# kluonj/HelFEM

Measured on AMD Instinct MI355X. Metric: scf_iteration_wall_time_fock_plus_geneig_nbf4230, lower is better.
Workload: dtype f64; 1 GPU; diatomic Z1=7 Z2=7 R=2.068 PBE, nelem=5 nnodes=15 nquad=75 lmmax=[20,20] (Nbf=4230, Nang=61, Nrad=70), XC grid 92x13, symmetry blocks [1380, 1470, 1380]: J+XC Fock build + eig_gsym_sub + density per step; parallelism=shard1, density=occupied orbitals of the core Hamiltonian

## Files before the change

### helfem_amd/__init__.py

```python
import ctypes
import os

import numpy as np

_HERE = os.path.dirname(os.path.abspath(__file__))
_LIB_PATH = os.environ.get("HELFEM_AMD_LIB") or os.path.join(_HERE, "lib", "libhelfem_amd.so")
_lib = None

c_double_p = ctypes.POINTER(ctypes.c_double)
c_int_p = ctypes.POINTER(ctypes.c_int)
c_i64_p = ctypes.POINTER(ctypes.c_int64)


class hfg_diatomic_desc(ctypes.Structure):
    _fields_ = [("Z1", ctypes.c_int), ("Z2", ctypes.c_int), ("Rhalf", ctypes.c_double), ("primbas", ctypes.c_int),
                ("nnodes", ctypes.c_int), ("nquad", ctypes.c_int), ("bval", c_double_p), ("nbval", ctypes.c_int),
                ("lval", c_int_p), ("mval", c_int_p), ("nang", ctypes.c_int), ("lpad", ctypes.c_int)]


class hfg_model_pot(ctypes.Structure):
    _fields_ = [("kind", ctypes.c_int), ("Z", ctypes.c_int), ("d", ctypes.c_double), ("H", ctypes.c_double)]


class hfg_atomic_desc(ctypes.Structure):
# ... 34 lines not shown
class hfg_scf_atomic_extras(ctypes.Structure):
    _fields_ = [("Rrms", ctypes.c_double), ("conf_N", ctypes.c_int), ("conf_R", ctypes.c_double),
                ("conf_barrier", ctypes.c_double), ("shift_conf", ctypes.c_double), ("add_conf", ctypes.c_int),
                ("Zl", ctypes.c_int), ("Zr", ctypes.c_int), ("Rmid", ctypes.c_double), ("nelem0", ctypes.c_int),
                ("grid0", ctypes.c_int), ("zexp0", ctypes.c_double), ("Econf", ctypes.c_double)]


def lib():
    global _lib
    if _lib is None:
        if not os.path.exists(_LIB_PATH):
            raise RuntimeError("%s is missing: run `python -m helfem_amd.build` (or __graft_entry__.build()) first; "
                               "there is no Python/CPU fallback for the hot path" % _LIB_PATH)
        if os.environ.get("HELFEM_NO_TORCH", "0") != "1":
            try:
                import torch
            except Exception:
                pass
        L = ctypes.CDLL(_LIB_PATH)
        L.hfg_last_error.restype = ctypes.c_char_p
        L.hfg_version.restype = ctypes.c_char_p
        L.hfg_gaunt_coefficient.restype = ctypes.c_double
        L.hfg_gaunt_coefficient.argtypes = [ctypes.c_int] * 6
        L.hfg_modified_gaunt_coefficient.restype = ctypes.c_double
        L.hfg_modified_gaunt_coefficient.argtypes = [ctypes.c_int] * 6
        L.hfg_theta_lm.restype = ctypes.c_double
        L.hfg_theta_lm.argtypes = [ctypes.c_int, ctypes.c_int, ctypes.c_double]
        L.hfg_legendre_PQ.restype = None
        L.hfg_legendre_PQ.argtypes = [ctypes.c_int, ctypes.c_int, ctypes.c_double, c_double_p, c_double_p]
        for nm in ("hfg_bessel_il", "hfg_bessel_kl"):
            getattr(L, nm).restype = ctypes.c_double
            getattr(L, nm).argtypes = [ctypes.c_double, ctypes.c_int]
        L.hfg_erfc_phi.restype = ctypes.c_double
        L.hfg_erfc_phi.argtypes = [ctypes.c_int, ctypes.c_double, ctypes.c_double]
        L.hfg_compute_rs_tei.argtypes = [ctypes.c_void_p, ctypes.c_int, ctypes.c_double]
        L.hfg_compute_rs_tei_dev.argtypes = [ctypes.c_void_p, ctypes.c_void_p, ctypes.c_int, ctypes.c_double]
        L.hfg_rs_special_dev.argtypes = [ctypes.c_void_p, ctypes.c_int, ctypes.c_int, c_double_p, c_double_p, ctypes.c_int64, c_double_p]
        L.hfg_set_erfc_binomial_mode.restype = None
        L.hfg_set_erfc_binomial_mode.argtypes = [ctypes.c_int]
        L.hfg_model_potential.argtypes = [ctypes.c_void_p, ctypes.c_void_p, ctypes.POINTER(hfg_model_pot),
                                          ctypes.POINTER(hfg_model_pot), c_double_p]
        L.hfg_chebyshev_rule.restype = None
        L.hfg_chebyshev_rule.argtypes = [ctypes.c_int, c_double_p, c_double_p]
        L.hfg_lobatto_nodes.restype = None
        L.hfg_lobatto_nodes.argtypes = [ctypes.c_int, c_double_p]
        L.hfg_radial_grid.argtypes = [ctypes.c_double, ctypes.c_int, ctypes.c_int, ctypes.c_double, c_double_p]
        L.hfg_basis_confinement.argtypes = [ctypes.c_void_p, ctypes.c_int, ctypes.c_int, ctypes.c_double, ctypes.c_double,
                                            ctypes.c_double, c_double_p]
        L.hfg_atomic_grid.argtypes = [ctypes.c_int, ctypes.c_double, ctypes.c_int, ctypes.c_double, ctypes.c_int, ctypes.c_double,
                                      ctypes.c_int, ctypes.c_int, ctypes.c_double, ctypes.c_int, ctypes.c_int, ctypes.c_int,
                                      ctypes.c_double, ctypes.c_int, ctypes.c_double, c_double_p, c_int_p]
        L.hfg_scf_options_check_ex.argtypes = [ctypes.POINTER(hfg_scf_options), ctypes.POINTER(hfg_scf_atomic_extras)]
        L.hfg_scf_run_ex.argtypes = [ctypes.c_void_p, ctypes.POINTER(hfg_scf_options), ctypes.POINTER(hfg_scf_atomic_extras),
                                     ctypes.POINTER(hfg_scf_result), c_double_p, c_double_p]
        L.hfg_ctx_create.argtypes = [ctypes.POINTER(ctypes.c_void_p), ctypes.c_int, ctypes.c_void_p]
        L.hfg_xc_fock.argtypes = [ctypes.c_void_p, ctypes.c_void_p, ctypes.c_int, ctypes.c_int, c_double_p, c_double_p,
                                  c_double_p, c_double_p, c_double_p, ctypes.c_double]
        L.hfg_xc_fock_pol.argtypes = [ctypes.c_void_p, ctypes.c_void_p, ctypes.c_int, ctypes.c_int, c_double_p, c_double_p,
                                      c_double_p, c_double_p, c_double_p, c_double_p, c_double_p, ctypes.c_double]
        L.hfg_xc_fock_dev.argtypes = [ctypes.c_void_p, ctypes.c_void_p, ctypes.c_int, ctypes.c_int, ctypes.c_void_p,
                                      ctypes.c_void_p, ctypes.c_void_p, ctypes.c_double]
        L.hfg_coulomb_batch.argtypes = [ctypes.c_void_p, ctypes.c_void_p, ctypes.c_int64, c_double_p, c_double_p]
        L.hfg_coulomb_energy_matrix.argtypes = [ctypes.c_void_p, ctypes.c_void_p, ctypes.c_int64, c_double_p, c_double_p]
        L.hfg_coulomb_batch_devptr.argtypes = [ctypes.c_void_p, ctypes.c_void_p, ctypes.c_int64, ctypes.c_void_p, ctypes.c_void_p]
        for name in ("hfg_exchange_batch", "hfg_rs_exchange_batch"):
            getattr(L, name).argtypes = [ctypes.c_void_p, ctypes.c_void_p, ctypes.c_int64, c_double_p, c_double_p]
        for name in ("hfg_exchange_batch_devptr", "hfg_rs_exchange_batch_devptr"):
            getattr(L, name).argtypes = [ctypes.c_void_p, ctypes.c_void_p, ctypes.c_int64, ctypes.c_void_p, ctypes.c_void_p]
        L.hfg_exchange_occ_batch_devptr.argtypes = [ctypes.c_void_p, ctypes.c_void_p, ctypes.c_int64, ctypes.c_void_p, ctypes.c_void_p,
                                                    c_i64_p, ctypes.c_int64, ctypes.c_void_p]
        L.hfg_exchange_batch_plan.argtypes = [ctypes.c_int64, c_int_p, ctypes.c_int, c_int_p, c_int_p]
        L.hfg_fock_compact_pol_size.restype = ctypes.c_int64
        L.hfg_fock_compact_pol_size.argtypes = [ctypes.c_void_p]
        L.hfg_fock_compact_pol_devptr.argtypes = [ctypes.c_void_p, ctypes.c_void_p, ctypes.c_int, ctypes.c_int, ctypes.c_void_p,
                                                  ctypes.c_void_p, ctypes.c_void_p, ctypes.c_void_p, ctypes.c_double]
        L.hfg_fock_finish_pol_devptr.argtypes = [ctypes.c_void_p] * 7
        L.hfg_eig_gsym_sub_pair_devptr.argtypes = [ctypes.c_void_p, ctypes.c_int64, ctypes.c_void_p, ctypes.c_void_p, ctypes.c_void_p,
                                                   ctypes.c_int, c_i64_p, c_i64_p] + [ctypes.c_void_p] * 4
        L.hfg_profile_get.argtypes = [ctypes.c_void_p, ctypes.c_char_p, c_double_p, c_i64_p]
        L.hfg_measure_kernel.argtypes = [ctypes.c_void_p, ctypes.c_char_p, c_double_p, c_i64_p]
        L.hfg_profile_names.argtypes = [ctypes.c_void_p, ctypes.c_char_p, ctypes.c_size_t]
        L.hfg_diis_create.argtypes = [ctypes.c_void_p, ctypes.c_int64, ctypes.c_int, ctypes.c_int, ctypes.c_double, ctypes.c_double,
                                      ctypes.c_int, ctypes.POINTER(ctypes.c_void_p)]
        L.hfg_diis_destroy.argtypes = [ctypes.c_void_p]
        L.hfg_diis_set_metric_devptr.argtypes = [ctypes.c_void_p, ctypes.c_void_p, ctypes.c_void_p, ctypes.c_int64]
        L.hfg_diis_set_blocks.argtypes = [ctypes.c_void_p, ctypes.c_int, c_i64_p, c_i64_p]
        L.hfg_diis_update_devptr.argtypes = [ctypes.c_void_p, ctypes.c_double, ctypes.c_void_p, ctypes.c_void_p, ctypes.c_void_p,
                                             ctypes.c_int64, ctypes.c_void_p, ctypes.c_void_p, ctypes.c_void_p, ctypes.c_int64,
                                             c_double_p]
        L.hfg_diis_solve_devptr.argtypes = [ctypes.c_void_p, ctypes.c_void_p, ctypes.c_void_p, c_int_p]
        L.hfg_diis_size.argtypes = [ctypes.c_void_p]
        L.hfg_diis_get.argtypes = [ctypes.c_void_p, ctypes.c_int, c_double_p, ctypes.c_int64]
        L.hfg_coulomb_dev.argtypes = [ctypes.c_void_p] * 4
        _lib = L
    return _lib


def _check(rc):
    if rc != 0:
        raise RuntimeError(lib().hfg_last_error().decode())


def _f(a):
    return np.asfortranarray(a, dtype=np.float64)


def _p(a):
    return a.ctypes.data_as(c_double_p)


def device_count():
    return int(lib().hfg_device_count())


class Context(object):

    def __init__(self, device=0, stream=None):
        h = ctypes.c_void_p()
        if stream is None:
            sp = None
        elif int(stream) == 0:
            sp = ctypes.c_void_p(-1)
        else:
            sp = ctypes.c_void_p(int(stream))
        _check(lib().hfg_ctx_create(ctypes.byref(h), int(device), sp))
        self.h = h
        self.device = device

    def close(self):
        if self.h:
            lib().hfg_ctx_destroy(self.h)
            self.h = None

    def __del__(self):
        try:
            self.close()
        except Exception:
            pass

    def synchronize(self):
        _check(lib().hfg_ctx_synchronize(self.h))

    def set_shard(self, rank, nranks):
        _check(lib().hfg_ctx_set_shard(self.h, int(rank), int(nranks)))

    def set_fock_blocks(self, basis, blockid_ptr):
        f = lib().hfg_ctx_set_fock_blocks
        f.argtypes = [ctypes.c_void_p, ctypes.c_void_p, ctypes.c_void_p]
        _check(f(self.h, basis.h, ctypes.c_void_p(blockid_ptr or 0)))

    def fix_sinvh(self, device_ptr):
        _check(lib().hfg_ctx_fix_sinvh(self.h, ctypes.c_void_p(device_ptr or 0)))

    def profile(self, on=True):
        _check(lib().hfg_profile_enable(self.h, 1 if on else 0))

    def profile_reset(self):
        _check(lib().hfg_profile_reset(self.h))

    def measure_kernel(self, name):
        ms = ctypes.c_double()
        n = ctypes.c_int64()
        _check(lib().hfg_measure_kernel(self.h, name.encode(), ctypes.byref(ms), ctypes.byref(n)))
        return ms.value, n.value

    def profile_names(self):
        buf = ctypes.create_string_buffer(1 << 16)
        _check(lib().hfg_profile_names(self.h, buf, len(buf)))
        return [x for x in buf.value.decode().split("\n") if x]

    def profile_get(self, name):
        ms = ctypes.c_double()
        n = ctypes.c_int64()
        _check(lib().hfg_profile_get(self.h, name.encode(), ctypes.byref(ms), ctypes.byref(n)))
        return ms.value, n.value

    def cuhf_update(self, S, Ca, na, Cb, nb, Fa, Fb):
        N = int(round(Fa.numel() ** 0.5))
        na, nb = int(na), int(nb)
        for t, count, what in ((S, N * N, "S"), (Ca, N * na, "Ca"), (Cb, N * nb, "Cb"), (Fa, N * N, "Fa"), (Fb, N * N, "Fb")):
            if t is None or not (t.is_cuda and t.is_contiguous() and str(t.dtype) == "torch.float64" and t.numel() >= count):
                raise ValueError("Context.cuhf_update: %s must be a contiguous float64 tensor on the device with at least %d elements"
                                 % (what, count))
        if N * N != Fa.numel() or Fb.numel() != Fa.numel():
            raise ValueError("Context.cuhf_update: Fa and Fb are N x N")
        f = lib().hfg_cuhf_update_devptr
        f.argtypes = [ctypes.c_void_p, ctypes.c_int64, ctypes.c_void_p, ctypes.c_void_p, ctypes.c_int64, ctypes.c_void_p, ctypes.c_int64,
                      ctypes.c_void_p, ctypes.c_void_p]
        _check(f(self.h, N, S.data_ptr(), Ca.data_ptr(), na, Cb.data_ptr(), nb, Fa.data_ptr(), Fb.data_ptr()))


_default_ctx = None


def default_context():
    global _default_ctx
    if _default_ctx is None:
        _default_ctx = Context(0)
    return _default_ctx


def tuning_table():
    buf = ctypes.create_string_buffer(1 << 16)
    _check(lib().hfg_tuning_table(buf, ctypes.c_size_t(len(buf))))
    keys = ("name", "kind", "default", "value", "read", "meaning")
    return [dict(zip(keys, line.split("\t"))) for line in buf.value.decode().split("\n") if line]


def lm_to_l_m(lmmax):
    lmmax = list(lmmax)
    cap = sum(2 * (l + 1) for l in lmmax) + 4
    lv = (ctypes.c_int * cap)()
    mv = (ctypes.c_int * cap)()
    n = ctypes.c_int(cap)
    arr = (ctypes.c_int * len(lmmax))(*lmmax)
    _check(lib().hfg_lm_list(arr, len(lmmax), lv, mv, ctypes.byref(n)))
    return list(lv[:n.value]), list(mv[:n.value])


def get_grid(mumax, nelem, igrid=4, zexp=1.0):
    b = np.zeros(nelem + 1)
    _check(lib().hfg_radial_grid(float(mumax), int(nelem), int(igrid), float(zexp), _p(b)))
    return b


class TwoDBasis(object):

    def __init__(self, Z1, Z2, Rhalf, nnodes, nquad, bval, lval, mval, lpad=10, ctx=None):
        self._bval = np.ascontiguousarray(bval, dtype=np.float64)
        self._lval = (ctypes.c_int * len(lval))(*lval)
        self._mval = (ctypes.c_int * len(mval))(*mval)
        d = hfg_diatomic_desc(int(Z1), int(Z2), float(Rhalf), 4, int(nnodes), int(nquad), _p(self._bval),
                              len(self._bval), self._lval, self._mval, len(lval), int(lpad))
        h = ctypes.c_void_p()
        _check(lib().hfg_diatomic_basis_create(ctypes.byref(d), ctypes.byref(h)))
        self.h = h
        self.ctx = ctx
        self.lval, self.mval = list(lval), list(mval)
        self._uploaded = None
        dims = [ctypes.c_int64() for _ in range(5)]
        _check(lib().hfg_basis_dims(self.h, *[ctypes.byref(x) for x in dims]))
        self._Nbf, self._Ndummy, self._Nrad, self._Nang, self._Nel = [x.value for x in dims]

    def __del__(self):
        try:
            if self.h:
                lib().hfg_basis_destroy(self.h)
                self.h = None
        except Exception:
            pass

    def Nbf(self):
        return self._Nbf

    def Ndummy(self):
        return self._Ndummy

    def Nrad(self):
        return self._Nrad

    def Nang(self):
        return self._Nang

    def Nel(self):
        return self._Nel

    def _mat(self, fn):
        M = np.zeros((self._Nbf, self._Nbf), order="F")
        _check(fn(self.h, _p(M)))
        return M

    def overlap(self):
        return self._mat(lib().hfg_basis_overlap)

    def kinetic(self):
        return self._mat(lib().hfg_basis_kinetic)

    def nuclear(self):
        return self._mat(lib().hfg_basis_nuclear)

    def get_sym_idx(self, symm):
        n = ctypes.c_int()
        _check(lib().hfg_basis_sym_blocks(self.h, int(symm), ctypes.byref(n), None, None))
        ptr = np.zeros(n.value + 1, dtype=np.int64)
        idx = np.zeros(self._Nbf, dtype=np.int64)
        _check(lib().hfg_basis_sym_blocks(self.h, int(symm), ctypes.byref(n), ptr.ctypes.data_as(c_i64_p),
                                          idx.ctypes.data_as(c_i64_p)))
        return [idx[ptr[i]:ptr[i + 1]].copy() for i in range(n.value)]

    def compute_tei(self, exchange=True, device=False, ctx=None):
        if device:
            ctx = ctx or self.ctx or default_context()
            self.ctx = ctx
            _check(lib().hfg_compute_tei_dev(ctx.h, self.h, 1 if exchange else 0))
        else:
            _check(lib().hfg_compute_tei(self.h, 1 if exchange else 0))
        self._uploaded = None

    def overlap_with(self, other):
        out = np.zeros((self.Nbf(), other.Nbf()), order="F")
        f = lib().hfg_basis_interbasis_overlap
        f.argtypes = [ctypes.c_void_p, ctypes.c_void_p, c_double_p]
        _check(f(self.h, other.h, _p(out)))
        return out

    def lm_map(self):
# ... 139 lines not shown
class AtomicTwoDBasis(TwoDBasis):

    def __init__(self, Z, nnodes, nquad, bval, lval, mval, ctx=None, finitenuc=0, Rrms=0.0, zeroder=False, Zl=0, Zr=0, Rmid=0.0):
        self._bval = np.ascontiguousarray(bval, dtype=np.float64)
        self._lval = (ctypes.c_int * len(lval))(*lval)
        self._mval = (ctypes.c_int * len(mval))(*mval)
        d = hfg_atomic_desc(int(Z), 4, int(nnodes), int(nquad), _p(self._bval), len(self._bval), self._lval,
                            self._mval, len(lval))
        h = ctypes.c_void_p()
        if finitenuc or zeroder or Zl or Zr:
            dx = hfg_atomic_desc_ex(d, int(finitenuc), float(Rrms), 1 if zeroder else 0, int(Zl), int(Zr), float(Rmid))
            _check(lib().hfg_atomic_basis_create_ex(ctypes.byref(dx), ctypes.byref(h)))
        else:
            _check(lib().hfg_atomic_basis_create(ctypes.byref(d), ctypes.byref(h)))
        self.h = h
        self.ctx = ctx
        self.lval, self.mval = list(lval), list(mval)
        self._uploaded = None
        dims = [ctypes.c_int64() for _ in range(5)]
        _check(lib().hfg_basis_dims(self.h, *[ctypes.byref(x) for x in dims]))
        self._Nbf, self._Ndummy, self._Nrad, self._Nang, self._Nel = [x.value for x in dims]

    def confinement(self, iconf, N=0, R=0.0, V=0.0, shift=0.0):
        out = np.zeros((self._Nbf, self._Nbf), order="F")
        _check(lib().hfg_basis_confinement(self.h, int(iconf), int(N), float(R), float(V), float(shift), _p(out)))
        return out

    ATOMIC_TABLES = {"prim_tei": 0, "prim_ktei": 4, "disjoint_L": 8, "disjoint_m1L": 10, "disjoint_iL": 12, "disjoint_kL": 13,
                     "rs_tei": 14, "rs_ktei": 15}

    def atomic_table(self, name, L, iel, kel=None):
        which = self.ATOMIC_TABLES[name]
        idx = int(iel) if kel is None else int(iel) * self._Nel + int(kel)
        r, c = ctypes.c_int64(), ctypes.c_int64()
        ctxh = self.ctx.h if self.ctx is not None else None
        f = lib().hfg_basis_get_prim
        f.argtypes = [ctypes.c_void_p, ctypes.c_void_p, ctypes.c_int, ctypes.c_int, ctypes.c_int, c_double_p,
                      ctypes.POINTER(ctypes.c_int64), ctypes.POINTER(ctypes.c_int64)]
        _check(f(ctxh, self.h, which, int(L), idx, None, ctypes.byref(r), ctypes.byref(c)))
        out = np.zeros((r.value, c.value), order="F")
        _check(f(ctxh, self.h, which, int(L), idx, _p(out), ctypes.byref(r), ctypes.byref(c)))
        return out

    RADIAL_TABLES = {"bf": 0, "df": 1, "lf": 2, "r": 3}

    def radial_table(self, name, iel):
        f = lib().hfg_basis_radial_table
        f.argtypes = [ctypes.c_void_p, ctypes.c_int, ctypes.c_int, c_double_p, ctypes.POINTER(ctypes.c_int64),
                      ctypes.POINTER(ctypes.c_int64)]
        r, c = ctypes.c_int64(), ctypes.c_int64()
        _check(f(self.h, self.RADIAL_TABLES[name], int(iel), None, ctypes.byref(r), ctypes.byref(c)))
        out = np.zeros((r.value, c.value), order="F")
        _check(f(self.h, self.RADIAL_TABLES[name], int(iel), _p(out), ctypes.byref(r), ctypes.byref(c)))
        return out[:, 0] if name == "r" else out

    def _compute_rs(self, kind, omega, device, ctx):
        if device:
            ctx = ctx or self.ctx
            if ctx is None:
                raise ValueError("device=True needs a context (ctx=... here or at construction)")
            self.ctx = ctx
            _check(lib().hfg_compute_rs_tei_dev(ctx.h, self.h, kind, float(omega)))
        else:
            _check(lib().hfg_compute_rs_tei(self.h, kind, float(omega)))
        self._uploaded = None

    def compute_yukawa(self, lam, device=False, ctx=None):
        self._compute_rs(1, lam, device, ctx)

    def compute_erfc(self, mu, device=False, ctx=None):
        self._compute_rs(2, mu, device, ctx)

    def rs_exchange_batch(self, Ps, ctx=None):
        return self.exchange_batch(Ps, ctx=ctx, _entry="hfg_rs_exchange_batch")

    def rs_exchange(self, P):
        ctx = self._ensure()
        P = _f(P)
        K = np.zeros_like(P, order="F")
        _check(lib().hfg_rs_exchange(ctx.h, self.h, _p(P), _p(K)))
        return K

    def mix_exchange_tables(self, alpha, beta, ctx=None):
        if ctx is not None and self._uploaded is None:
            self.upload(ctx=ctx)
        ctx = ctx or self._ensure()
        f = lib().hfg_mix_exchange_tables
        f.argtypes = [ctypes.c_void_p, ctypes.c_void_p, ctypes.c_double, ctypes.c_double]
        rc = f(ctx.h, self.h, float(alpha), float(beta))
        if rc == 4:
            return False
        _check(rc)
        return True

    def mix_exchange(self, P):
        if self.ctx is None:
            raise RuntimeError("The mixed exchange tables have not been built (mix_exchange_tables)!")
        P = _f(P)
        K = np.zeros_like(P, order="F")
        f = lib().hfg_mix_exchange
        f.argtypes = [ctypes.c_void_p, ctypes.c_void_p, c_double_p, c_double_p]
        _check(f(self.ctx.h, self.h, _p(P), _p(K)))
        return K

    def mix_exchange_torch(self, dP, dC=None, nocc=None, out=None, ctx=None):
        import torch
        ctx = ctx or self.ctx
        N = self.Nbf()
        N2 = N * N
        if out is None:
            out = torch.empty_like(dP)
        for t in (dP, out) + ((dC,) if dC is not None else ()):
            if t.dtype != torch.float64 or not t.is_cuda or not t.is_contiguous() or t.numel() % N2 or t.numel() != dP.numel():
                raise ValueError("mix_exchange_torch: contiguous float64 device tensors of nP * Nbf * Nbf elements")
        nP = dP.numel() // N2
        L = lib()
        ptr = lambda t: ctypes.c_void_p(t.data_ptr())
        if dC is not None:
            counts = np.ascontiguousarray(np.atleast_1d(nocc), dtype=np.int64)
            if len(counts) != nP:
                raise ValueError("mix_exchange_torch: one count of occupied orbitals per density")
        if nP == 1 and dC is None:
            L.hfg_mix_exchange_devptr.argtypes = [ctypes.c_void_p] * 4
            _check(L.hfg_mix_exchange_devptr(ctx.h, self.h, ptr(dP), ptr(out)))
        elif nP == 1:
            L.hfg_mix_exchange_occ_devptr.argtypes = [ctypes.c_void_p] * 4 + [ctypes.c_int64, ctypes.c_void_p]
            _check(L.hfg_mix_exchange_occ_devptr(ctx.h, self.h, ptr(dP), ptr(dC), int(counts[0]), ptr(out)))
        else:
            L.hfg_mix_exchange_occ_batch_devptr.argtypes = [ctypes.c_void_p, ctypes.c_void_p, ctypes.c_int64, ctypes.c_void_p, ctypes.c_void_p,
                                                            c_i64_p, ctypes.c_int64, ctypes.c_void_p]
            _check(L.hfg_mix_exchange_occ_batch_devptr(ctx.h, self.h, nP, ptr(dP), ptr(dC) if dC is not None else None,
                                                       counts.ctypes.data_as(c_i64_p) if dC is not None else None, N, ptr(out)))
        return out

    def mixed_table(self, L, iel, kel):
        f = lib().hfg_basis_get_prim
        f.argtypes = [ctypes.c_void_p, ctypes.c_void_p, ctypes.c_int, ctypes.c_int, ctypes.c_int, c_double_p,
                      ctypes.POINTER(ctypes.c_int64), ctypes.POINTER(ctypes.c_int64)]
        r, c = ctypes.c_int64(), ctypes.c_int64()
        ctxh = self.ctx.h if self.ctx is not None else None
        idx = int(iel) * self._Nel + int(kel)
        _check(f(ctxh, self.h, 16, int(L), idx, None, ctypes.byref(r), ctypes.byref(c)))
        out = np.zeros((r.value, c.value), order="F")
        _check(f(ctxh, self.h, 16, int(L), idx, _p(out), ctypes.byref(r), ctypes.byref(c)))
        return out


def exchange_batch_plan(ranks, max_members=0):
    r = np.ascontiguousarray(ranks, dtype=np.int32)
    out = np.full(len(r), -2, dtype=np.int32)
    n = ctypes.c_int(0)
    _check(lib().hfg_exchange_batch_plan(len(r), r.ctypes.data_as(c_int_p), int(max_members), out.ctypes.data_as(c_int_p), ctypes.byref(n)))
    return out.tolist(), n.value


class DFTGrid(object):

    def __init__(self, basis, ldft, mdft):
        self.basis, self.ldft, self.mdft = basis, int(ldft), int(mdft)

    def eval_Fxc(self, x_func, c_func, P, thr=1e-12):
        b = self.basis
        if b._uploaded != (self.ldft, self.mdft):
            b.upload(self.ldft, self.mdft)
        P = _f(P)
        H = np.zeros_like(P, order="F")
        exc, nel, ekin = ctypes.c_double(), ctypes.c_double(), ctypes.c_double()
        _check(lib().hfg_xc_fock(b.ctx.h, b.h, int(x_func), int(c_func), _p(P), _p(H), ctypes.byref(exc),
                                 ctypes.byref(nel), ctypes.byref(ekin), float(thr)))
        return H, exc.value, nel.value, ekin.value

    def eval_Fxc_pol(self, x_func, c_func, Pa, Pb, thr=1e-12):
        b = self.basis
        if b._uploaded != (self.ldft, self.mdft):
            b.upload(self.ldft, self.mdft)
        Pa, Pb = _f(Pa), _f(Pb)
        Ha, Hb = np.zeros_like(Pa, order="F"), np.zeros_like(Pb, order="F")
        exc, nel, ekin = ctypes.c_double(), ctypes.c_double(), ctypes.c_double()
        _check(lib().hfg_xc_fock_pol(b.ctx.h, b.h, int(x_func), int(c_func), _p(Pa), _p(Pb), _p(Ha), _p(Hb),
                                     ctypes.byref(exc), ctypes.byref(nel), ctypes.byref(ekin), float(thr)))
        return Ha, Hb, exc.value, nel.value, ekin.value


    def eval_Fxc_dev(self, x_func, c_func, P, Pb=None, thr=1e-12):
        import torch
        b = self.basis
        if b._uploaded != (self.ldft, self.mdft):
            b.upload(self.ldft, self.mdft)
        dev = torch.device("cuda", b.ctx.device)
        N = b.Nbf()

        def up(M):
            return torch.from_numpy(np.asfortranarray(M, dtype=np.float64).ravel(order="F").copy()).to(dev)

        def ptr(t):
            return ctypes.c_void_p(t.data_ptr())
        scal = torch.zeros(3, dtype=torch.float64, device=dev)
        dP = up(P)
        dH = torch.zeros(N * N, dtype=torch.float64, device=dev)
        torch.cuda.synchronize(dev)
        L = lib()
        if Pb is None:
            L.hfg_xc_fock_dev.argtypes = [ctypes.c_void_p, ctypes.c_void_p, ctypes.c_int, ctypes.c_int, ctypes.c_void_p,
                                          ctypes.c_void_p, ctypes.c_void_p, ctypes.c_double]
            _check(L.hfg_xc_fock_dev(b.ctx.h, b.h, int(x_func), int(c_func), ptr(dP), ptr(dH), ptr(scal), float(thr)))
            b.ctx.synchronize()
            sc = scal.cpu().numpy()
            return dH.cpu().numpy().reshape((N, N), order="F"), sc[0], sc[1], sc[2]
        dPb = up(Pb)
        dHb = torch.zeros(N * N, dtype=torch.float64, device=dev)
        torch.cuda.synchronize(dev)
        L.hfg_xc_fock_pol_dev.argtypes = [ctypes.c_void_p, ctypes.c_void_p, ctypes.c_int, ctypes.c_int, ctypes.c_void_p,
                                          ctypes.c_void_p, ctypes.c_void_p, ctypes.c_void_p, ctypes.c_void_p,
                                          ctypes.c_double]
        _check(L.hfg_xc_fock_pol_dev(b.ctx.h, b.h, int(x_func), int(c_func), ptr(dP), ptr(dPb), ptr(dH), ptr(dHb), ptr(scal),
                                     float(thr)))
        b.ctx.synchronize()
        sc = scal.cpu().numpy()
        return (dH.cpu().numpy().reshape((N, N), order="F"), dHb.cpu().numpy().reshape((N, N), order="F"), sc[0], sc[1],
                sc[2])


class scf(object):

    @staticmethod
    def _blocks(m_idx):
        ptr = np.zeros(len(m_idx) + 1, dtype=np.int64)
        for i, b in enumerate(m_idx):
            ptr[i + 1] = ptr[i] + len(b)
        idx = np.concatenate([np.asarray(b, dtype=np.int64) for b in m_idx]) if len(m_idx) else np.zeros(0, np.int64)
        return ptr, np.ascontiguousarray(idx)

    @staticmethod
    def eig_gsym(F, Sinvh, ctx=None):
        ctx = ctx or default_context()
        F, Sinvh = _f(F), _f(Sinvh)
        N, n = Sinvh.shape
        E = np.zeros(n)
        C = np.zeros((N, n), order="F")
        _check(lib().hfg_eig_gsym(ctx.h, ctypes.c_int64(N), ctypes.c_int64(n), _p(F), _p(Sinvh), _p(E), _p(C)))
        return E, C

    @staticmethod
    def eig_gsym_sub(F, Sinvh, m_idx, ctx=None):
        ctx = ctx or default_context()
        F, Sinvh = _f(F), _f(Sinvh)
        N = F.shape[0]
        ptr, idx = scf._blocks(m_idx)
        E = np.zeros(N)
        C = np.zeros((N, N), order="F")
        _check(lib().hfg_eig_gsym_sub(ctx.h, ctypes.c_int64(N), _p(F), _p(Sinvh), len(m_idx),
                                      ptr.ctypes.data_as(c_i64_p), idx.ctypes.data_as(c_i64_p), _p(E), _p(C)))
        return E, C

    @staticmethod
    def eig_gsym_sub_pair(Fa, Fb, Sinvh, m_idx, ctx=None):
        ctx = ctx or default_context()
        Fa, Fb, Sinvh = _f(Fa), _f(Fb), _f(Sinvh)
        N = Fa.shape[0]
        ptr, idx = scf._blocks(m_idx)
        Ea, Eb = np.zeros(N), np.zeros(N)
        Ca, Cb = np.zeros((N, N), order="F"), np.zeros((N, N), order="F")
        f = lib().hfg_eig_gsym_sub_pair
        f.argtypes = [ctypes.c_void_p, ctypes.c_int64, c_double_p, c_double_p, c_double_p, ctypes.c_int, c_i64_p, c_i64_p, c_double_p,
                      c_double_p, c_double_p, c_double_p]
        _check(f(ctx.h, N, _p(Fa), _p(Fb), _p(Sinvh), len(m_idx), ptr.ctypes.data_as(c_i64_p), idx.ctypes.data_as(c_i64_p), _p(Ea), _p(Ca),
                 _p(Eb), _p(Cb)))
        return Ea, Ca, Eb, Cb

    @staticmethod
    def eig_sym(A, ctx=None):
        ctx = ctx or default_context()
        A = _f(A)
        n = A.shape[0]
        E = np.zeros(n)
        C = np.zeros((n, n), order="F")
        _check(lib().hfg_eig_sym(ctx.h, ctypes.c_int64(n), _p(A), _p(E), _p(C)))
        return E, C

    @staticmethod
    def eig_sel_count(m_idx, nev):
        ptr, _ = scf._blocks(m_idx)
        f = lib().hfg_eig_sel_count
        f.restype = ctypes.c_int64
        f.argtypes = [ctypes.c_int, c_i64_p, ctypes.c_int64]
        return int(f(len(m_idx), ptr.ctypes.data_as(c_i64_p), int(nev)))

    @staticmethod
    def eig_sym_sel(A, nev, ctx=None):
        ctx = ctx or default_context()
        A = _f(A)
        n = A.shape[0]
        K = max(0, min(int(nev), n))
        E = np.zeros(K)
        C = np.zeros((n, K), order="F")
        f = lib().hfg_eig_sym_sel
        f.argtypes = [ctypes.c_void_p, ctypes.c_int64, c_double_p, ctypes.c_int64, c_double_p, c_double_p]
        _check(f(ctx.h, n, _p(A), int(nev), _p(E), _p(C)))
        return E, C

    @staticmethod
    def eig_gsym_sub_sel(F, Sinvh, m_idx, nev, ctx=None):
        ctx = ctx or default_context()
        F, Sinvh = _f(F), _f(Sinvh)
        N = F.shape[0]
        ptr, idx = scf._blocks(m_idx)
# ... 311 lines not shown
            raise ValueError("DeviceDIIS.update: nspin = 1 takes one spin")
        err = ctypes.c_double()
        _check(lib().hfg_diis_update_devptr(self.h, float(E), self._dp(self._mat(Fa, self.N, "Fa")), self._dp(self._mat(Pa, self.N, "Pa")),
                                            self._dp(self._mat(Ca, int(nocca), "Ca")), int(nocca) if Ca is not None else 0,
                                            self._dp(self._mat(Fb, self.N, "Fb")), self._dp(self._mat(Pb, self.N, "Pb")),
                                            self._dp(self._mat(Cb, int(noccb), "Cb")), int(noccb) if Cb is not None else 0,
                                            ctypes.byref(err)))
        return err.value

    def solve(self, Fa, Fb=None):
        if self.nspin == 2 and Fb is None:
            raise ValueError("DeviceDIIS.solve: nspin = 2 needs Fb")
        dropped = ctypes.c_int()
        _check(lib().hfg_diis_solve_devptr(self.h, self._dp(self._mat(Fa, self.N, "Fa")), self._dp(self._mat(Fb, self.N, "Fb")),
                                           ctypes.byref(dropped)))
        return dropped.value

    @property
    def size(self):
        return int(lib().hfg_diis_size(self.h))

    def _get(self, which, count):
        out = np.zeros(max(count, 1))
        _check(lib().hfg_diis_get(self.h, which, _p(out), count))
        return out[:count]

    @property
    def B(self):
        k = self.size
        return self._get(0, k * k).reshape(k, k)

    @property
    def T(self):
        k = self.size
        return self._get(1, k * k).reshape(k, k)

    @property
    def weights(self):
        return self._get(2, self.size)

    @property
    def error(self):
        n = self.n
        return self._get(3, self.nspin * n * n).reshape(self.nspin, n, n).transpose(0, 2, 1)


MIX_BY_DEFAULT = {1: True, 2: True}


def _refuse_out_of_scope(who, rohf, cuhf, readocc, maverage, dampfock):
    bad = [name for name, on in (("ROHF", rohf), ("CUHF", cuhf), ("readocc", readocc is not None and int(readocc) >= 0),
                                 ("maverage", maverage), ("dampfock", float(dampfock) != 1.0)) if on]
    if bad:
        raise NotImplementedError("%s.run: %s not supported by the step objects; use the SCF drivers (scf_diatomic, scf_atomic, "
                                  "scf_run_atomic)" % (who, ", ".join(bad)))


class DeviceSCFStep(object):

    def __init__(self, basis, x_func, c_func, ldft, mdft, nocc, symmetry=1, device=0, rank=0, nranks=1,
                 dens_thr=1e-12, kfrac=0.0, device_tei=False, fock_shard="auto", kshort=0.0, omega=0.0, rs_kind=None):
        self.nocc = int(nocc)
        self._setup(basis, x_func, c_func, ldft, mdft, symmetry, device, rank, nranks, dens_thr, kfrac, device_tei, fock_shard,
                    kshort, omega, rs_kind)
        f64 = dict(dtype=self.torch.float64, device=self.dev)
        L, N = lib(), self.N
        self.Fc = self.torch.zeros(int(L.hfg_fock_compact_size(basis.h)), **f64)
        self.scal = self.torch.zeros(3, **f64)
        self.F = self.torch.zeros(N * N, **f64)
        self.E = self.torch.zeros(N, **f64)
        self.C = self.torch.zeros(N * N, **f64)
        self.P = self.torch.zeros(N * N, **f64)
        nb = int(L.hfg_eig_block_buf_size(len(self.blocks), self.blk_ptr.ctypes.data_as(c_i64_p)))
        self.blockbuf = self.torch.zeros(nb, **f64)
        if self.anyK:
            self.K = self.torch.zeros(N * N, **f64)
            self.Pa = self.torch.zeros(N * N, **f64)

    def _setup(self, basis, x_func, c_func, ldft, mdft, symmetry, device, rank, nranks, dens_thr, kfrac, device_tei, fock_shard,
               kshort=0.0, omega=0.0, rs_kind=None):
        self.kshort, self.omega = float(kshort), float(omega)
        self.rs_kind = 0
        self.mix = False
        self.Krs = None
        if self.kshort != 0.0:
            if not isinstance(basis, AtomicTwoDBasis):
                raise RuntimeError("Range separated functionals are not supported.")
            self.rs_kind = xc_rs_kind(x_func) if rs_kind is None else int(rs_kind)
            if self.rs_kind not in (1, 2) or self.omega == 0.0:
                raise ValueError("kshort != 0 needs a screened kernel (rs_kind 1 Yukawa or 2 erfc, from the exchange functional "
                                 "when None) and its range omega != 0")
        import torch
        self.torch = torch
        self.basis = basis
        self.x_func, self.c_func, self.thr = int(x_func), int(c_func), float(dens_thr)
        self.dev = torch.device("cuda", device)
        torch.cuda.set_device(self.dev)
        self.ctx = Context(device, stream=torch.cuda.current_stream(self.dev).cuda_stream)
        self.ctx.set_shard(rank, nranks)
        self.rank, self.nranks = int(rank), int(nranks)
        self.fock_shard = os.environ.get("HELFEM_FOCK_SHARD", fock_shard)
        if device_tei:
            basis.compute_tei(float(kfrac) != 0.0 or self.kshort != 0.0, device=True, ctx=self.ctx)
        if self.kshort != 0.0:
            switches = {r["name"]: r["value"] for r in tuning_table()}
            on_device = bool(device_tei) or switches["HELFEM_RS_TEI"] == "dev"
            basis._compute_rs(self.rs_kind, self.omega, on_device, self.ctx)
        basis.upload(ldft, mdft, ctx=self.ctx)
        if self.kshort != 0.0:
            want = int(switches["HELFEM_EXL_MIX"])
            if want > 0 or (want < 0 and MIX_BY_DEFAULT[self.rs_kind]):
                self.mix = basis.mix_exchange_tables(float(kfrac), self.kshort, ctx=self.ctx)
        L = lib()
        L.hfg_fock_compact_size.restype = ctypes.c_int64
        L.hfg_eig_block_buf_size.restype = ctypes.c_int64
        L.hfg_fock_compact_dev.argtypes = [ctypes.c_void_p, ctypes.c_void_p, ctypes.c_int, ctypes.c_int, ctypes.c_void_p,
                                           ctypes.c_void_p, ctypes.c_void_p, ctypes.c_double]
        N = basis.Nbf()
        self.N = N
        self.blocks = basis.get_sym_idx(symmetry)
        self.blk_ptr, self.blk_idx = scf._blocks(self.blocks)
        blockid = np.zeros(N, dtype=np.int32)
        for ib, b in enumerate(self.blocks):
            blockid[b] = ib
        self.blockid = torch.from_numpy(blockid).to(self.dev)
        self.ctx.set_fock_blocks(basis, self.blockid.data_ptr())
        self.H0 = None
        self.Sinvh = None
        self.kfrac = float(kfrac)
        self.anyK = self.kfrac != 0.0 or self.kshort != 0.0
        self.kscale = self.kfrac if self.kshort == 0.0 else 1.0
        self.have_C = False
        self.have_density = False
        if self.kshort != 0.0:
            self.Krs = None if self.mix else torch.zeros(N * N, dtype=torch.float64, device=self.dev)
            for name in ("hfg_rs_exchange_dev", "hfg_mix_exchange_devptr"):
                getattr(L, name).argtypes = [ctypes.c_void_p] * 4
            L.hfg_mix_exchange_occ_devptr.argtypes = [ctypes.c_void_p] * 4 + [ctypes.c_int64, ctypes.c_void_p]
            L.hfg_mix_exchange_occ_batch_devptr.argtypes = L.hfg_exchange_occ_batch_devptr.argtypes
        if self.anyK:
            L.hfg_exchange_occ_dev.argtypes = [ctypes.c_void_p, ctypes.c_void_p, ctypes.c_void_p, ctypes.c_void_p, ctypes.c_int64,
                                               ctypes.c_void_p]
            L.hfg_exchange_dev.argtypes = [ctypes.c_void_p, ctypes.c_void_p, ctypes.c_void_p, ctypes.c_void_p]

    def _ptr(self, t):
        return ctypes.c_void_p(t.data_ptr())

    def set_matrices(self, H0, Sinvh):
        t = self.torch
        self.H0 = t.from_numpy(np.asfortranarray(H0).ravel(order="F").copy()).to(self.dev)
        self.ctx.fix_sinvh(None)
        self.Sinvh = t.from_numpy(np.asfortranarray(Sinvh).ravel(order="F").copy()).to(self.dev)
        self.ctx.fix_sinvh(self.Sinvh.data_ptr())

    def set_density(self, P, C=None):
        self.P.copy_(self.torch.from_numpy(np.asfortranarray(P).ravel(order="F").copy()))
        self.have_density = True
        self.have_C = C is not None
        if C is not None:
            self.C[:self.N * self.nocc].copy_(self.torch.from_numpy(np.asfortranarray(C[:, :self.nocc]).ravel(order="F").copy()))

    def exchange(self):
        self.torch.mul(self.P, 0.5, out=self.Pa)
        self._build_K(self.Pa, self.C, self.nocc, self.K)

    def _build_K(self, P, C, nocc, K):
        L, h, b = lib(), self.ctx.h, self.basis.h
        if self.mix:
            if self.have_C:
                _check(L.hfg_mix_exchange_occ_devptr(h, b, self._ptr(P), self._ptr(C), ctypes.c_int64(nocc), self._ptr(K)))
            else:
                _check(L.hfg_mix_exchange_devptr(h, b, self._ptr(P), self._ptr(K)))
            return
        if self.kfrac != 0.0:
            if self.have_C:
                _check(L.hfg_exchange_occ_dev(h, b, self._ptr(P), self._ptr(C), ctypes.c_int64(nocc), self._ptr(K)))
            else:
                _check(L.hfg_exchange_dev(h, b, self._ptr(P), self._ptr(K)))
        if self.kshort != 0.0:
            _check(L.hfg_rs_exchange_dev(h, b, self._ptr(P), self._ptr(self.Krs)))
            if self.kfrac != 0.0:
                K.mul_(self.kfrac).add_(self.Krs, alpha=self.kshort)
            else:
                self.torch.mul(self.Krs, self.kshort, out=K)

    def fock_partial(self):
        _check(lib().hfg_fock_compact_dev(self.ctx.h, self.basis.h, self.x_func, self.c_func, self._ptr(self.P),
                                          self._ptr(self.Fc), self._ptr(self.scal), self.thr))

    def fock_finish(self):
        _check(lib().hfg_fock_finish_dev(self.ctx.h, self.basis.h, self._ptr(self.Fc), self._ptr(self.H0),
                                         self._ptr(self.blockid), self._ptr(self.F)))

    def eig_partial(self):
        _check(lib().hfg_eig_blocks_dev(self.ctx.h, ctypes.c_int64(self.N), self._ptr(self.F), self._ptr(self.Sinvh),
                                        len(self.blocks), self.blk_ptr.ctypes.data_as(c_i64_p),
                                        self.blk_idx.ctypes.data_as(c_i64_p), self._ptr(self.blockbuf)))

    def eig_finish(self):
        _check(lib().hfg_eig_assemble_dev(self.ctx.h, ctypes.c_int64(self.N), len(self.blocks),
                                          self.blk_ptr.ctypes.data_as(c_i64_p), self.blk_idx.ctypes.data_as(c_i64_p),
                                          self._ptr(self.blockbuf), self._ptr(self.E), self._ptr(self.C)))

    def eig_whole(self):
        _check(lib().hfg_eig_gsym_sub_dev(self.ctx.h, ctypes.c_int64(self.N), self._ptr(self.F), self._ptr(self.Sinvh),
                                          len(self.blocks), self.blk_ptr.ctypes.data_as(c_i64_p),
                                          self.blk_idx.ctypes.data_as(c_i64_p), self._ptr(self.E), self._ptr(self.C)))

    def density(self):
        _check(lib().hfg_form_density_dev(self.ctx.h, ctypes.c_int64(self.N), ctypes.c_int64(self.N), self._ptr(self.C),
                                          ctypes.c_int64(self.nocc), self._ptr(self.P)))
        self.have_density = True

    def step(self, allreduce=None, exchange_blocks=None):
        shard_fock = self.nranks > 1 and self.fock_shard == "always"
        if self.nranks > 1 and not shard_fock:
            self.ctx.set_shard(0, 1)
        self.fock_partial()
        if self.nranks > 1 and not shard_fock:
            self.ctx.set_shard(self.rank, self.nranks)
        if allreduce is not None and (shard_fock or self.nranks == 1):
            allreduce(self.Fc)
            allreduce(self.scal)
        self.fock_finish()
        if self.anyK:
            self.exchange()
            if allreduce is not None:
                allreduce(self.K)
            self.F.add_(self.K, alpha=self.kscale)
        self._eig_stage(allreduce, exchange_blocks)
        self.density()
        self.have_C = True

    def _whole_shard(self, fn):
        if self.nranks > 1:
            self.ctx.set_shard(0, 1)
        try:
            fn()
        finally:
            if self.nranks > 1:
                self.ctx.set_shard(self.rank, self.nranks)

    def _fock_stage(self, allreduce):
        shard_fock = self.nranks > 1 and self.fock_shard == "always"
        if shard_fock or self.nranks == 1:
            self.fock_partial()
            if allreduce is not None:
                allreduce(self.Fc)
                allreduce(self.scal)
        else:
            self._whole_shard(self.fock_partial)
        self.fock_finish()
        if self.anyK:
            self.exchange()
            if allreduce is not None:
                allreduce(self.K)
            self._add_exchange()

    def _add_exchange(self):
        self.F.add_(self.K, alpha=self.kscale)

    def _eig_stage(self, allreduce, exchange_blocks):
        if self.nranks == 1 and allreduce is None and exchange_blocks is None:
            self.eig_whole()
            return
        self.eig_partial()
        if exchange_blocks is not None:
            exchange_blocks(self.blockbuf, len(self.blocks))
        elif allreduce is not None:
            allreduce(self.blockbuf)
        self.eig_finish()

    def _coulomb_energy_matrix(self, P):
        if getattr(self, "J", None) is None:
            self.J = self.torch.zeros(self.N * self.N, dtype=self.torch.float64, device=self.dev)
        self._whole_shard(lambda: _check(lib().hfg_coulomb_dev(self.ctx.h, self.basis.h, self._ptr(P), self._ptr(self.J))))
        return self.J

    def _energy_terms(self):
        t = self.torch
        J = self._coulomb_energy_matrix(self.P)
        terms = [t.dot(self.P, self.H0), t.dot(self.P, J)]
        terms.append(t.dot(self.Pa, self.K) if self.anyK else t.zeros((), dtype=t.float64, device=self.dev))
        return terms

    def energy(self, Enucr=0.0):
        t = self.torch
        v = t.stack(self._energy_terms() + [self.scal[0]]).cpu().numpy()
        r = dict(E1=float(v[0]), Ecoul=0.5 * float(v[1]), Exx=self._exx_factor() * float(v[2]), Exc=float(v[3]), Enucr=float(Enucr))
        r["Etot"] = r["E1"] + r["Ecoul"] + r["Exx"] + r["Exc"] + r["Enucr"]
        return r

    def _exx_factor(self):
        return self.kscale

    def _nspin(self):
        return 1

    def _density_stage(self):
        self.density()
        self.P.mul_(2.0)
        self.have_C = True

    def _core_guess(self, allreduce, exchange_blocks):
        self.F.copy_(self.H0)
        self._eig_stage(allreduce, exchange_blocks)
# ... 288 lines not shown
```

### helfem_amd/csrc/hip/capi.cpp

```cpp
#include "internal.h"
#include "../host/checkpoint.h"
#include "../host/diis.h"
#include "../host/dftfuncs.h"
#include "../host/exchange_batch_plan.h"
#include "../host/fock_need.h"
#include <cstring>
#include <memory>
#include <mutex>

namespace hfg {
static thread_local std::string g_err;
void set_error(const std::string &msg) { g_err = msg; }

}

using namespace hfg;

#define HFG_TRY try {
#define HFG_CATCH                       \
  }                                     \
  catch (const std::logic_error &e) {   \
    hfg::set_error(e.what());           \
    return 1;                           \
  }                                     \
  catch (const std::runtime_error &e) { \
    hfg::set_error(e.what());           \
    return 2;                           \
  }                                     \
  catch (const std::exception &e) {     \
    hfg::set_error(e.what());           \
    return 3;                           \
  }                                     \
  return 0;

hipStream_t hfg_ctx::side() {
  if (!side_stream) {
    HFG_HIP_CHECK(hipStreamCreateWithFlags(&side_stream, hipStreamNonBlocking));
    HFG_HIP_CHECK(hipEventCreateWithFlags(&side_ev[0], hipEventDisableTiming));
    HFG_HIP_CHECK(hipEventCreateWithFlags(&side_ev[1], hipEventDisableTiming));
  }
  return side_stream;
}
void hfg_ctx::drop_side() {
  if (!side_stream) return;
  (void)hipStreamSynchronize(side_stream);
  (void)hipStreamDestroy(side_stream);
  (void)hipEventDestroy(side_ev[0]);
  (void)hipEventDestroy(side_ev[1]);
  side_stream = nullptr;
  side_ev[0] = side_ev[1] = nullptr;
}
void *hfg_ctx::pinned_buf(size_t bytes) {
  if (bytes > pinned_bytes) {
    if (pinned) (void)hipHostFree(pinned);
    pinned = nullptr;
    HFG_HIP_CHECK(hipHostMalloc((void **)&pinned, bytes, hipHostMallocDefault));
    pinned_bytes = bytes;
  }
  return pinned;
}
hipEvent_t hfg_ctx::get_event() {
  if (!event_pool.empty()) {
    hipEvent_t e = event_pool.back();
    event_pool.pop_back();
    return e;
  }
  hipEvent_t e;
  HFG_HIP_CHECK(hipEventCreate(&e));
  return e;
}
void hfg_ctx::prof_begin(const char *name) {
  hipEvent_t a = get_event(), b = get_event();
  HFG_HIP_CHECK(hipEventRecord(a, stream));
  prof[name].pending.push_back(std::make_pair(a, b));
}
void hfg_ctx::prof_end(const char *name) {
  ProfEntry &p = prof[name];
  HFG_HIP_CHECK(hipEventRecord(p.pending.back().second, stream));
  p.launches++;
}
void hfg_ctx::prof_collect() {
  for (auto &kv : prof) {
    for (auto &ev : kv.second.pending) {
      float ms = 0.f;
      HFG_HIP_CHECK(hipEventSynchronize(ev.second));
      HFG_HIP_CHECK(hipEventElapsedTime(&ms, ev.first, ev.second));
      kv.second.ms += ms;
      event_pool.push_back(ev.first);
      event_pool.push_back(ev.second);
    }
    kv.second.pending.clear();
  }
}

namespace {
struct Stage {
  hfg_ctx *ctx;
  std::vector<double *> bufs;
  explicit Stage(hfg_ctx *c) : ctx(c) { HFG_HIP_CHECK(hipSetDevice(c->device)); }
  ~Stage() {
    for (double *p : bufs) (void)hipFree(p);
  }
  double *alloc(size_t n) {
    double *p = nullptr;
    HFG_HIP_CHECK(hipMalloc((void **)&p, std::max<size_t>(n, 1) * sizeof(double)));
    bufs.push_back(p);
    return p;
  }
  double *up(const double *h, size_t n) {
    double *p = alloc(n);
    HFG_HIP_CHECK(hipMemcpyAsync(p, h, n * sizeof(double), hipMemcpyHostToDevice, ctx->stream));
    return p;
  }
  void down(double *h, const double *d, size_t n) {
    HFG_HIP_CHECK(hipMemcpyAsync(h, d, n * sizeof(double), hipMemcpyDeviceToHost, ctx->stream));
  }
  void sync() { HFG_HIP_CHECK(hipStreamSynchronize(ctx->stream)); }
};

void require_gpu() {
  int n = 0;
  hipError_t e = hipGetDeviceCount(&n);
  if (e != hipSuccess || n <= 0)
    throw std::runtime_error("no usable HIP device: the helfem_amd hot path has no CPU fallback");
}
}

extern "C" {

const char *hfg_last_error(void) { return g_err.c_str(); }
const char *hfg_version(void) { return "helfem_amd 0.1 (gfx950)"; }

int hfg_device_count(void) {
  int n = 0;
  if (hipGetDeviceCount(&n) != hipSuccess) return 0;
  return n;
}

int hfg_ctx_create(hfg_ctx **out, int device, void *stream) {
  HFG_TRY
  require_gpu();
  HFG_HIP_CHECK(hipSetDevice(device));
  hfg_ctx *c = new hfg_ctx();
  c->device = device;
  if (stream == HFG_NULL_STREAM) {
    c->stream = nullptr;
    c->own_stream = false;
  } else if (stream) {
    c->stream = (hipStream_t)stream;
    c->own_stream = false;
  } else {
    HFG_HIP_CHECK(hipStreamCreateWithFlags(&c->stream, hipStreamNonBlocking));
    c->own_stream = true;
  }
  *out = c;
  HFG_CATCH
}

int hfg_ctx_destroy(hfg_ctx *c) {
  HFG_TRY
  if (!c) return 0;
  (void)hipSetDevice(c->device);
  (void)hipStreamSynchronize(c->stream);
  c->work.drop_all();
  for (auto &kv : c->prof)
    for (auto &ev : kv.second.pending) {
      (void)hipEventDestroy(ev.first);
      (void)hipEventDestroy(ev.second);
    }
  for (hipEvent_t e : c->event_pool) (void)hipEventDestroy(e);
  if (c->pinned) (void)hipHostFree(c->pinned);
  if (c->side_stream) {
    (void)hipStreamSynchronize(c->side_stream);
    (void)hipStreamDestroy(c->side_stream);
    (void)hipEventDestroy(c->side_ev[0]);
    (void)hipEventDestroy(c->side_ev[1]);
  }
  if (c->own_stream) (void)hipStreamDestroy(c->stream);
  delete c;
  HFG_CATCH
}

int hfg_ctx_synchronize(hfg_ctx *c) {
  HFG_TRY
  HFG_HIP_CHECK(hipStreamSynchronize(c->stream));
  trdp_check_status(c);
  HFG_CATCH
}

int hfg_ctx_fix_sinvh(hfg_ctx *c, const double *dSinvh) {
  HFG_TRY
  c->fix_sinvh(dSinvh);
  HFG_CATCH
}

int hfg_ctx_set_shard(hfg_ctx *c, int rank, int nranks) {
  HFG_TRY
  if (nranks < 1 || rank < 0 || rank >= nranks) throw std::logic_error("invalid shard");
  c->shard_rank = rank;
  c->shard_n = nranks;
  HFG_CATCH
}

int hfg_diatomic_basis_create(const hfg_diatomic_desc *d, hfg_basis **out) {
  HFG_TRY
  if (d->primbas != 4) throw std::logic_error("Unsupported primitive basis.\n");
  hfg_basis *b = new hfg_basis();
  b->b = helfem::diatomic::TwoDBasis(d->Z1, d->Z2, d->Rhalf, d->nnodes, d->nquad,
                                     helfem::Vec(d->bval, d->bval + d->nbval),
                                     helfem::IVec(d->lval, d->lval + d->nang),
                                     helfem::IVec(d->mval, d->mval + d->nang), d->lpad);
  *out = b;
  HFG_CATCH
}

int hfg_atomic_basis_create(const hfg_atomic_desc *d, hfg_basis **out) {
  HFG_TRY
  if (d->primbas != 4) throw std::logic_error("Unsupported primitive basis.\n");
  hfg_basis *b = new hfg_basis();
  b->kind = 1;
  b->ab = helfem::atomic::TwoDBasis(d->Z, d->nnodes, d->nquad, helfem::Vec(d->bval, d->bval + d->nbval),
                                    helfem::IVec(d->lval, d->lval + d->nang), helfem::IVec(d->mval, d->mval + d->nang));
  *out = b;
  HFG_CATCH
}

static int copy_out(const helfem::Mat &M, double *out);

int hfg_atomic_basis_create_ex(const hfg_atomic_desc_ex *dx, hfg_basis **out) {
  HFG_TRY
  const hfg_atomic_desc *d = &dx->base;
  if (d->primbas != 4) throw std::logic_error("Unsupported primitive basis.\n");
  if (dx->finitenuc != 0 && (dx->Zl != 0 || dx->Zr != 0))
    throw std::logic_error("Off-center nuclei not supported in finite nucleus mode!\n");
  std::unique_ptr<hfg_basis> b(new hfg_basis());
  b->kind = 1;
  b->ab = helfem::atomic::TwoDBasis(d->Z, dx->finitenuc, dx->Rrms, dx->zeroder != 0, d->nnodes, d->nquad,
                                    helfem::Vec(d->bval, d->bval + d->nbval), helfem::IVec(d->lval, d->lval + d->nang),
                                    helfem::IVec(d->mval, d->mval + d->nang), dx->Zl, dx->Zr, dx->Rmid);
  *out = b.release();
  HFG_CATCH
}

int hfg_basis_confinement(const hfg_basis *b, int iconf, int N, double R, double V, double shift, double *out) {
  HFG_TRY
  if (!b->kind) throw std::logic_error("Confinement potentials belong to the atomic program.\n");
  copy_out(b->ab.confinement(N, R, iconf, V, shift), out);
  HFG_CATCH
}

int hfg_atomic_grid(int finitenuc, double Rrms, int nelem, double Rmax, int grid, double zexp, int nelem0, int grid0,
                    double zexp0, int Z, int Zl, int Zr, double Rmid, int add_conf, double shift_conf, double *bval, int *n) {
  HFG_TRY
  helfem::Vec g = helfem::atomic::form_grid(finitenuc, Rrms, nelem, Rmax, grid, zexp, nelem0, grid0, zexp0, Z, Zl, Zr, Rmid,
                                            add_conf != 0, shift_conf, false);
  const int cap = *n;
  *n = (int)g.size();
  if ((int)g.size() > cap) throw std::logic_error("hfg_atomic_grid: output capacity too small");
  for (size_t i = 0; i < g.size(); i++) bval[i] = g[i];
  HFG_CATCH
}

int hfg_angular_basis(int lmax, int mmax, int *lval, int *mval, int *nang) {
  HFG_TRY
  helfem::IVec l, m;
  helfem::atomic::angular_basis(lmax, mmax, l, m);
  if ((int)l.size() > *nang) {
    *nang = (int)l.size();
    throw std::logic_error("hfg_angular_basis: output capacity too small");
  }
  *nang = (int)l.size();
  for (size_t i = 0; i < l.size(); i++) {
    lval[i] = l[i];
    mval[i] = m[i];
  }
  HFG_CATCH
}

int hfg_basis_destroy(hfg_basis *b) {
  HFG_TRY
  if (!b) return 0;
  delete b->dev_mix;
  delete b->dev;
  delete b->dev_rs;
  delete b;
  HFG_CATCH
}

int hfg_basis_dims(const hfg_basis *b, int64_t *Nbf, int64_t *Ndummy, int64_t *Nrad, int64_t *Nang, int64_t *Nel) {
  if (Nbf) *Nbf = b->Nbf();
  if (Ndummy) *Ndummy = b->Ndummy();
  if (Nrad) *Nrad = b->Nrad();
  if (Nang) *Nang = b->Nang();
  if (Nel) *Nel = b->Nel();
  return 0;
}

static int copy_out(const helfem::Mat &M, double *out) {
  memcpy(out, M.memptr(), sizeof(double) * M.n_elem());
  return 0;
}
int hfg_basis_overlap(const hfg_basis *b, double *S) {
  HFG_TRY copy_out(b->kind ? b->ab.overlap() : b->b.overlap(), S);
  HFG_CATCH
}
int hfg_basis_kinetic(const hfg_basis *b, double *T) {
  HFG_TRY copy_out(b->kind ? b->ab.kinetic() : b->b.kinetic(), T);
  HFG_CATCH
}
int hfg_basis_nuclear(const hfg_basis *b, double *V) {
  HFG_TRY copy_out(b->kind ? b->ab.nuclear() : b->b.nuclear(), V);
  HFG_CATCH
}

int hfg_basis_sym_blocks(const hfg_basis *b, int symm, int *nblk, int64_t *blk_ptr, int64_t *blk_idx) {
  HFG_TRY
  auto idx = b->kind ? b->ab.get_sym_idx(symm) : b->b.get_sym_idx(symm);
  *nblk = (int)idx.size();
  if (blk_ptr) {
    int64_t off = 0;
    for (size_t i = 0; i < idx.size(); i++) {
      blk_ptr[i] = off;
      for (size_t k = 0; k < idx[i].size(); k++) blk_idx[off + k] = (int64_t)idx[i][k];
      off += idx[i].size();
    }
    blk_ptr[idx.size()] = off;
  }
  HFG_CATCH
}

int hfg_compute_tei(hfg_basis *b, int exchange) {
  HFG_TRY
  if (b->kind) b->ab.compute_tei(exchange != 0);
  else b->b.compute_tei(exchange != 0);
  HFG_CATCH
}

int hfg_compute_rs_tei(hfg_basis *b, int rs_kind, double omega) {
  HFG_TRY
  if (b->kind == 0) throw std::logic_error("Range separated functionals are not supported.\n");
  if (rs_kind == 1) b->ab.compute_yukawa(omega);
  else if (rs_kind == 2) b->ab.compute_erfc(omega);
  else throw std::logic_error("unknown range-separation kernel (1 = Yukawa, 2 = erfc)\n");
  b->rs_on_device = false;
  drop_mix_tables(b);
// ... 971 lines not shown
```

### helfem_amd/csrc/hip/common.h

```cpp
#pragma once
#include <hip/hip_runtime.h>
#include <cstdint>
#include <cstring>
#include <map>
#include <stdexcept>
#include <string>
#include <vector>

#include "../../../include/helfem_gpu.h"
#include "../host/atomic_basis.h"
#include "../host/diatomic_basis.h"
#include "../host/tuning.h"
#include "workspace_owner.h"

namespace hfg {
using helfem::TrdMode, helfem::tuning;

void set_error(const std::string &msg);

#define HFG_HIP_CHECK(expr)                                                                          \
  do {                                                                                               \
    hipError_t _e = (expr);                                                                          \
    if (_e != hipSuccess)                                                                            \
      throw std::runtime_error(std::string("HIP error: ") + hipGetErrorString(_e) + " in " + #expr + \
                               " (" + __FILE__ + ":" + std::to_string(__LINE__) + ")");              \
  } while (0)

template <typename T>
struct DevBuf {
  T *p = nullptr;
  size_t n = 0;
  DevBuf() {}
  DevBuf(const DevBuf &) = delete;
  DevBuf &operator=(const DevBuf &) = delete;
  ~DevBuf() { release(); }
  void release() {
    if (p) (void)hipFree(p);
    p = nullptr;
    n = 0;
  }
  void resize(size_t count) {
    if (count <= n) return;
    release();
    HFG_HIP_CHECK(hipMalloc((void **)&p, count * sizeof(T)));
    n = count;
  }
  void upload(const std::vector<T> &h, hipStream_t s) {
    resize(h.size() ? h.size() : 1);
    if (h.size()) HFG_HIP_CHECK(hipMemcpyAsync(p, h.data(), h.size() * sizeof(T), hipMemcpyHostToDevice, s));
  }
};

template <typename T>
bool upload_cached(DevBuf<T> &buf, std::vector<T> &cache, const std::vector<T> &h, hipStream_t s) {
  if (buf.p && cache.size() == h.size() && buf.n >= h.size() &&
      (h.empty() || memcmp((const void *)cache.data(), (const void *)h.data(), h.size() * sizeof(T)) == 0))
    return false;
  HFG_HIP_CHECK(hipStreamSynchronize(s));
  cache = h;
  buf.upload(cache, s);
  return true;
}

struct ProfEntry {
  double ms = 0.0;
  int64_t launches = 0;
  std::vector<std::pair<hipEvent_t, hipEvent_t> > pending;
};

}

struct hfg_dev_tables;

struct hfg_ctx {
  int device = 0;
  hipStream_t stream = nullptr;
  bool own_stream = false;
  hipStream_t side_stream = nullptr;
  hipEvent_t side_ev[2] = {nullptr, nullptr};
  hipStream_t side();
  bool avoid_side = false;
  void drop_side();
  int shard_rank = 0, shard_n = 1;
  const double *fixed_sinvh = nullptr;
  unsigned long fixed_gen = 0;
  void fix_sinvh(const double *p) {
    fixed_sinvh = p;
    fixed_gen++;
  }
  hfg::DevBuf<int> fock_need, fock_gneed;
  const hfg_dev_tables *fock_need_tables = nullptr;
  int fock_need_A = 0, fock_need_G = 0;
  bool profiling = false;
  std::map<std::string, hfg::ProfEntry> prof;
  std::vector<hipEvent_t> event_pool;
  hfg::DevBuf<double> ws[8];
  double *pinned = nullptr;
  size_t pinned_bytes = 0;
  hfg::WorkspaceOwner<hfg::WS_CTX_SLOTS> work;

  void *pinned_buf(size_t bytes);
  hipEvent_t get_event();
  void prof_begin(const char *name);
  void prof_end(const char *name);
  void prof_collect();
};

struct hfg_basis {
  int kind = 0;
  helfem::diatomic::TwoDBasis b;
  helfem::atomic::TwoDBasis ab;
  hfg_dev_tables *dev = nullptr;
  hfg_dev_tables *dev_rs = nullptr;
  hfg_dev_tables *dev_mix = nullptr;
  double mix_alpha = 0.0, mix_beta = 0.0, mix_omega = 0.0;
  int mix_kind = 0;
  int dev_device = -1;
  hfg::DevBuf<double> dev_tei;
  bool tei_on_device = false;
  hfg::DevBuf<double> dev_rs_tei, dev_rs_disj;
  bool rs_on_device = false;

  size_t Nbf() const { return kind ? ab.Nbf() : b.Nbf(); }
  size_t Ndummy() const { return kind ? ab.Nbf() : b.Ndummy(); }
  size_t Nrad() const { return kind ? ab.Nrad() : b.Nrad(); }
  size_t Nang() const { return kind ? ab.Nang() : b.Nang(); }
  size_t Nel() const { return kind ? ab.Nel() : b.Nel(); }
  size_t max_Nprim() const { return kind ? ab.max_Nprim() : b.max_Nprim(); }
  bool have_tei() const { return tei_on_device || (kind ? ab.have_tei : b.have_tei); }
};

namespace hfg {
struct GemmTask {
  const double *A;
  const double *B;
  double *C;
  int M, N, K, lda, ldb, ldc;
  int tA = 0, tB = 0;
  double alpha = 1.0, beta = 0.0;
  int sym = 0;
  int over = 0;
  const int *amap = nullptr, *cmap = nullptr;
  const int64_t *rmap = nullptr;
};
static_assert(sizeof(GemmTask) == 104, "GemmTask is compared bytewise: keep it free of padding");

struct ProfScope {
  hfg_ctx *c;
  const char *n;
  ProfScope(hfg_ctx *ctx, const char *name) : c(ctx), n(name) {
    if (c->profiling) c->prof_begin(n);
  }
  ~ProfScope() {
    if (c->profiling) c->prof_end(n);
  }
};
}
```

### helfem_amd/csrc/hip/eig.hip

```cpp
#include "internal.h"
#include "wave.h"
#include "../host/eigsel_count.h"
#include <cstdlib>
#include <cstring>
#include <functional>

namespace hfg {

constexpr int MAXB = 8;
struct EigBatch {
  int nblk;
  int n[MAXB];
  double *A[MAXB];
  double *d[MAXB];
  double *e[MAXB];
  double *tau[MAXB];
  double *v[MAXB];
  double *pp[MAXB];
  double *dots[MAXB];
  double *Z[MAXB];
  int nz[MAXB];
  double *rot[MAXB];
  int *sweeps[MAXB];
  long rotcap[MAXB];
};

constexpr int TRD_NCS = 8;

__global__ void k_gather_block(const double *__restrict__ F, const double *__restrict__ S, int N,
                               const int64_t *__restrict__ rows, const int64_t *__restrict__ cols, int n,
                               double *__restrict__ Fb, double *__restrict__ Xb) {
  int i = blockIdx.x * blockDim.x + threadIdx.x;
  int j = blockIdx.y;
  if (i >= n) return;
  Fb[(size_t)j * n + i] = F[(size_t)rows[j] * N + rows[i]];
  Xb[(size_t)j * n + i] = S[(size_t)cols[j] * N + rows[i]];
}

__global__ void k_gather_f(const double *__restrict__ F, int N, const int64_t *__restrict__ rows, int n, double *__restrict__ Fb) {
  int i = blockIdx.x * blockDim.x + threadIdx.x;
  int j = blockIdx.y;
  if (i >= n) return;
  Fb[(size_t)j * n + i] = F[(size_t)rows[j] * N + rows[i]];
}

__global__ void k_col_support(const double *__restrict__ S, int N, const int64_t *__restrict__ rows, int n,
                              int *__restrict__ flag) {
  int c = blockIdx.x;
  int any = 0;
  for (int i = threadIdx.x; i < n; i += blockDim.x)
    if (S[(size_t)c * N + rows[i]] != 0.0) any = 1;
  any = __syncthreads_or(any);
  if (threadIdx.x == 0) flag[c] = any;
}

__device__ inline void householder_of_column(const double *__restrict__ A, int n, int k, double *vsh, double *red,
                                             double &tau, double &beta) {
  const int m = n - k - 1;
  const double *x = A + (size_t)k * n + k + 1;
  double s = 0.0;
  for (int i = 1 + threadIdx.x; i < m; i += blockDim.x) s += x[i] * x[i];
  s = wave_sum(s);
  int nwave = blockDim.x / 64;
  if ((threadIdx.x & 63) == 0) red[threadIdx.x >> 6] = s;
  __syncthreads();
  double xn2 = 0.0;
  for (int w = 0; w < nwave; w++) xn2 += red[w];
  double alpha = x[0];
  double scale;
  if (xn2 == 0.0) {
    tau = 0.0;
    beta = alpha;
    scale = 0.0;
  } else {
    double nrm = sqrt(alpha * alpha + xn2);
    beta = (alpha >= 0.0) ? -nrm : nrm;
    tau = (beta - alpha) / beta;
    scale = 1.0 / (alpha - beta);
  }
  for (int i = threadIdx.x; i < m; i += blockDim.x) vsh[i] = (i == 0) ? 1.0 : x[i] * scale;
  __syncthreads();
}

__global__ __launch_bounds__(256) void k_trd_gemv(EigBatch b, int k) {
  extern __shared__ double sh[];
  const int blk = blockIdx.y;
  const int n = b.n[blk];
  if (k > n - 3) return;
  const int m = n - k - 1;
  const int nrs = (m + 63) / 64;
  const int rs = blockIdx.x / TRD_NCS, cs = blockIdx.x % TRD_NCS;
  if (rs >= nrs) return;
  double *A = b.A[blk];
  double *vsh = sh;
  double *red = sh + n;
  double tau, beta;
  householder_of_column(A, n, k, vsh, red, tau, beta);
  if (blockIdx.x == 0) {
    for (int i = threadIdx.x; i < m; i += blockDim.x) b.v[blk][i] = vsh[i];
    if (threadIdx.x == 0) {
      b.tau[blk][k] = tau;
      b.e[blk][k] = beta;
      b.d[blk][k] = A[(size_t)k * n + k];
    }
  }
  const int cchunk = (m + TRD_NCS - 1) / TRD_NCS;
  const int c0 = cs * cchunk, c1 = min(m, c0 + cchunk);
  const int wave = threadIdx.x >> 6, lane = threadIdx.x & 63;
  const int row = rs * 64 + lane;
  double acc = 0.0;
  if (row < m) {
    const double *a = A + (size_t)(k + 1) * n + (k + 1) + row;
    for (int c = c0 + wave; c < c1; c += 4) acc += a[(size_t)c * n] * vsh[c];
  }
  __syncthreads();
  red[wave * 64 + lane] = acc;
  __syncthreads();
  if (wave == 0) {
    double p = red[lane] + red[64 + lane] + red[128 + lane] + red[192 + lane];
    if (row < m) b.pp[blk][(size_t)cs * n + row] = p;
    double dv = (row < m) ? p * vsh[row] : 0.0;
    dv = wave_sum(dv);
    if (lane == 0) b.dots[blk][blockIdx.x] = dv;
  }
}

__global__ __launch_bounds__(256) void k_trd_update(EigBatch b, int k) {
  __shared__ double vr[64], vc[64], wr[64], wc[64];
  __shared__ double Ksh;
  const int blk = blockIdx.y;
  const int n = b.n[blk];
  if (k > n - 3) return;
  const int m = n - k - 1;
  const int nt = (m + 63) / 64;
  if ((int)blockIdx.x >= nt * nt) return;
  const int tr = blockIdx.x % nt, tc = blockIdx.x / nt;
  double *A = b.A[blk];
  const double tau = b.tau[blk][k];
  if (threadIdx.x == 0) {
    const int nrs = (m + 63) / 64;
    double s = 0.0;
    for (int i = 0; i < nrs * TRD_NCS; i++) s += b.dots[blk][i];
    Ksh = 0.5 * tau * tau * s;
  }
  __syncthreads();
  if (threadIdx.x < 128) {
    int which = threadIdx.x >> 6, l = threadIdx.x & 63;
    int idx = (which ? tc : tr) * 64 + l;
    double v = 0.0, w = 0.0;
    if (idx < m) {
      v = b.v[blk][idx];
      double p = 0.0;
      for (int cs = 0; cs < TRD_NCS; cs++) p += b.pp[blk][(size_t)cs * n + idx];
      w = tau * p - Ksh * v;
    }
    if (which) {
      vc[l] = v;
      wc[l] = w;
    } else {
      vr[l] = v;
      wr[l] = w;
    }
  }
  __syncthreads();
  const int lane = threadIdx.x & 63, wave = threadIdx.x >> 6;
  const int row = tr * 64 + lane;
  if (row < m) {
    double *a = A + (size_t)(k + 1) * n + (k + 1) + row;
    for (int c = wave; c < 64; c += 4) {
      int col = tc * 64 + c;
      if (col < m) a[(size_t)col * n] -= vr[lane] * wc[c] + wr[lane] * vc[c];
    }
  }
  if (blockIdx.x == 0) {
    for (int i = 1 + threadIdx.x; i < m; i += blockDim.x) A[(size_t)k * n + k + 1 + i] = b.v[blk][i];
  }
}

__global__ void k_trd_finish(EigBatch b) {
  int blk = blockIdx.x;
  if (threadIdx.x != 0) return;
  int n = b.n[blk];
  double *A = b.A[blk];
  if (n >= 2) {
    b.d[blk][n - 2] = A[(size_t)(n - 2) * n + (n - 2)];
    b.e[blk][n - 2] = A[(size_t)(n - 2) * n + (n - 1)];
    b.tau[blk][n - 2] = 0.0;
  }
  b.d[blk][n - 1] = A[(size_t)(n - 1) * n + (n - 1)];
  b.e[blk][n - 1] = 0.0;
}

__global__ void k_tql_values(EigBatch b) {
  int blk = blockIdx.x;
  if (threadIdx.x != 0) return;
  const int n = b.n[blk];
// ... 254 lines not shown
  const int j0 = pair * BT_PW;
  if (j0 > n - 3) return;
  const int kb1 = min(BT_KB, n - 2 - (j0 + BT_KB));
  const int tid = threadIdx.x, cl = tid >> 6, i = tid & 63;
  if (kb1 > 0) {
    constexpr int NE = BT_KB * BT_KB / 256;
    double c[NE];
#pragma unroll
    for (int u = 0; u < NE; u++) c[u] = 0.0;
    for (int sl = 0; sl < GS; sl++) {
      const double *src = Cc[blk] + ((size_t)sl * npair + pair) * BT_KB * BT_KB + tid;
#pragma unroll
      for (int u = 0; u < NE; u++) c[u] += src[256 * u];
    }
#pragma unroll
    for (int u = 0; u < NE; u++) {
      const int t = tid + 256 * u;
      sC[t % BT_KB][t / BT_KB] = c[u];
    }
  }
  const size_t tot = (size_t)BT_PW * n;
  double a0[BT_WREP], a1[BT_WREP];
#pragma unroll
  for (int rep = 0; rep < BT_WREP; rep++) {
    const int col = (blockIdx.x * BT_WREP + rep) * 4 + cl;
    a0[rep] = 0.0;
    a1[rep] = 0.0;
    if (col < n) {
      for (int sl = 0; sl < S; sl++) {
        a0[rep] += Wpart[blk][(size_t)sl * tot + (size_t)col * BT_PW + i];
        a1[rep] += Wpart[blk][(size_t)sl * tot + (size_t)col * BT_PW + BT_KB + i];
      }
    }
  }
  if (mirror) {
    const int kb0 = min(BT_KB, n - 2 - j0);
#pragma unroll
    for (int rep = 0; rep < BT_WREP; rep++) {
      const int col = (blockIdx.x * BT_WREP + rep) * 4 + cl;
      __syncthreads();
      s1[cl][i] = (i < kb0) ? a0[rep] : 0.0;
      __syncthreads();
      if (col < n) {
        double r1 = 0.0;
        if (kb1 > 0 && i < kb1) {
          double corr = 0.0;
          for (int j = 0; j < kb0; j++) corr += sC[j][i] * s1[cl][j];
          r1 = a1[rep] - corr;
        }
        W[blk][(size_t)col * BT_PW + i] = a0[rep];
        W[blk][(size_t)col * BT_PW + BT_KB + i] = r1;
      }
    }
    return;
  }
#pragma unroll
  for (int rep = 0; rep < BT_WREP; rep++) {
    const int col = (blockIdx.x * BT_WREP + rep) * 4 + cl;
    __syncthreads();
    s1[cl][i] = (kb1 > 0 && i < kb1) ? a1[rep] : 0.0;
    __syncthreads();
    if (col < n) {
      double r0 = a0[rep];
      if (kb1 > 0) {
        double corr = 0.0;
        for (int j = 0; j < kb1; j++) corr += sC[i][j] * s1[cl][j];
        r0 -= corr;
      }
      W[blk][(size_t)col * BT_PW + i] = r0;
      W[blk][(size_t)col * BT_PW + BT_KB + i] = (kb1 > 0 && i < kb1) ? a1[rep] : 0.0;
    }
  }
}

constexpr int BT_GS = 4;
__global__ __launch_bounds__(64) void k_bt_T(EigBatch b, double *const *__restrict__ G, double *const *__restrict__ T,
                                             int P) {
  __shared__ double sT[BT_KB][BT_KB + 1];
  __shared__ double sG[BT_KB][BT_KB + 1];
  __shared__ double sg[BT_KB];
  const int blk = blockIdx.y, p = blockIdx.x;
  const int n = b.n[blk];
  const int j0 = p * BT_KB;
  if (j0 > n - 3) return;
  const int kb = min(BT_KB, n - 2 - j0);
  double *Tp = T[blk] + (size_t)p * BT_KB * BT_KB;
  const int t = threadIdx.x;
  for (int c0 = 0; c0 < BT_KB; c0 += 16) {
    double g[16];
#pragma unroll
    for (int u = 0; u < 16; u++) g[u] = 0.0;
#pragma unroll
    for (int sl = 0; sl < BT_GS; sl++) {
      const double *src = G[blk] + ((size_t)sl * P + p) * BT_KB * BT_KB + (size_t)c0 * BT_KB + t;
#pragma unroll
      for (int u = 0; u < 16; u++) g[u] += src[(size_t)u * BT_KB];
    }
#pragma unroll
    for (int u = 0; u < 16; u++) {
      sG[c0 + u][t] = g[u];
      sT[t][c0 + u] = 0.0;
    }
  }
  __shared__ double stau[BT_KB];
  stau[t] = (t < kb) ? b.tau[blk][j0 + t] : 0.0;
  __syncthreads();
  for (int i = 0; i < kb; i++) {
    const double ti = stau[i];
    sg[t] = (t < i) ? sG[i][t] : 0.0;
    __syncthreads();
    if (t < i) {
      double acc0 = 0.0, acc1 = 0.0, acc2 = 0.0, acc3 = 0.0;
#pragma unroll
      for (int k = 0; k < BT_KB; k += 4) {
        acc0 += sT[t][k] * sg[k];
        acc1 += sT[t][k + 1] * sg[k + 1];
        acc2 += sT[t][k + 2] * sg[k + 2];
        acc3 += sT[t][k + 3] * sg[k + 3];
      }
      sT[t][i] = -ti * ((acc0 + acc1) + (acc2 + acc3));
    }
    if (t == i) sT[i][i] = ti;
    __syncthreads();
  }
  for (int c = 0; c < BT_KB; c++) Tp[(size_t)c * BT_KB + t] = sT[t][c];
}

struct EigWork : Workspace {
  GemmHow full_how;
  std::vector<int64_t> asm_rows;
  DevBuf<long long> asm_rows_dev;
  bool folded = false;
  DevBuf<double> Y[MAXB];
  DevBuf<GemmTask> btslabR, btupdR;
  std::vector<GemmTask> h_btslabR, h_btupdR;
  DevBuf<double> A[MAXB], d[MAXB], e[MAXB], tau[MAXB], v[MAXB], pp[MAXB], dots[MAXB], Z[MAXB], rot[MAXB];
  DevBuf<double> Zs[MAXB], Ws[MAXB];
  DevBuf<int> selrank;
  DevBuf<int> sweeps[MAXB];
  DevBuf<int> ibuf1, ibuf2;
  DevBuf<GemmTask> gtasks, bttasks, btslab, btgram, btcpl, btupd;
  std::vector<GemmTask> h_gtasks, h_bttasks, h_btslab, h_btgram, h_btcpl, h_btupd;
  std::vector<double *> h_btptr;
  DevBuf<double> Vx[MAXB], G[MAXB], T[MAXB], VT[MAXB], Wb[MAXB], Wp[MAXB], Cc[MAXB];
  DevBuf<double *> btptr;
  bool used_dc = true;
  DevBuf<double> idx;
  const double *sup_S = nullptr;
  unsigned long sup_gen = 0;
  int sup_N = 0;
  std::vector<int64_t> sup_ptr, sup_idx;
  DevBuf<double> Xc;
  std::vector<char> xc_have;
  int *h_status = nullptr;
  hipEvent_t status_ev = nullptr;
  ~EigWork() {
    if (h_status) (void)hipHostFree(h_status);
    if (status_ev) (void)hipEventDestroy(status_ev);
  }
};
static EigWork &work_for(hfg_ctx *ctx) { return ctx->work.get<EigWork>(WS_EIG); }

struct CopySlices {
  const double *src[16];
  double *dst[16];
  int n[16];
};
__global__ void k_copy_slices(CopySlices c) {
  const int q = blockIdx.y;
  for (int i = blockIdx.x * blockDim.x + threadIdx.x; i < c.n[q]; i += gridDim.x * blockDim.x) c.dst[q][i] = c.src[q][i];
}
static void copy_slices(hipStream_t s, const std::vector<const double *> &src, const std::vector<double *> &dst, const std::vector<int> &n) {
  for (size_t q0 = 0; q0 < src.size(); q0 += 16) {
    CopySlices c{};
    const int m = (int)std::min<size_t>(16, src.size() - q0);
    int nmax = 0;
    for (int q = 0; q < m; q++) {
      c.src[q] = src[q0 + q];
      c.dst[q] = dst[q0 + q];
      c.n[q] = n[q0 + q];
      nmax = std::max(nmax, n[q0 + q]);
    }
    if (nmax > 0) hipLaunchKernelGGL(k_copy_slices, dim3((nmax + 255) / 256, m), dim3(256), 0, s, c);
  }
}

struct TrPtrs {
  const double *src[MAXB];
  double *dst[MAXB];
  int n[MAXB];
};
__global__ __launch_bounds__(256) void k_transpose_batch(TrPtrs t) {
  __shared__ double tile[64][65];
  const int blk = blockIdx.z, n = t.n[blk];
  const int bi = blockIdx.x * 64, bj = blockIdx.y * 64;
  if (bi >= n || bj >= n) return;
  const int tx = threadIdx.x & 63, ty = threadIdx.x >> 6;
  for (int c = ty; c < 64; c += 4) {
    const int gm = bi + tx, gn = bj + c;
    tile[c][tx] = (gm < n && gn < n) ? t.src[blk][(size_t)gn * n + gm] : 0.0;
  }
  __syncthreads();
  for (int c = ty; c < 64; c += 4) {
    const int gm = bj + tx, gn = bi + c;
    if (gm < n && gn < n) t.dst[blk][(size_t)gn * n + gm] = tile[tx][c];
  }
}

static void bt_wy_setup(hfg_ctx *ctx, EigWork &w, const EigBatch &b, int nblk, const int *ns, int nmax, bool fold = false) {
  hipStream_t s = ctx->stream;
  const int P = (nmax - 3) / BT_KB + 1;
  const int NP = (P + 1) / 2;
  constexpr int BT_S = 6;
  std::vector<double *> ptrs(6 * (size_t)nblk);
  for (int k = 0; k < nblk; k++) {
    const int n = ns[k];
    w.Vx[k].resize((size_t)n * n);
    w.G[k].resize((size_t)BT_GS * P * BT_KB * BT_KB);
    w.T[k].resize((size_t)P * BT_KB * BT_KB);
    w.VT[k].resize((size_t)n * P * BT_KB);
    w.Wb[k].resize((size_t)BT_PW * n);
    w.Wp[k].resize((size_t)BT_S * BT_PW * n);
    w.Cc[k].resize((size_t)BT_GS * NP * BT_KB * BT_KB);
    ptrs[k] = w.Vx[k].p;
    ptrs[nblk + k] = w.G[k].p;
    ptrs[2 * nblk + k] = w.T[k].p;
    ptrs[3 * nblk + k] = w.Wp[k].p;
    ptrs[4 * nblk + k] = w.Wb[k].p;
    ptrs[5 * nblk + k] = w.Cc[k].p;
  }
  upload_cached(w.btptr, w.h_btptr, ptrs, s);
  GemmTask none;
  none.A = none.B = nullptr;
  none.C = nullptr;
  none.M = none.N = none.K = 0;
  none.lda = none.ldb = none.ldc = 1;
  auto kb_of = [&](int k, int p) { return std::max(0, std::min(BT_KB, ns[k] - 2 - p * BT_KB)); };
  auto chunk_of = [](int len, int parts) { return ((len + parts - 1) / parts + 15) / 16 * 16; };

  std::vector<GemmTask> gram((size_t)BT_GS * P * nblk, none), vt((size_t)P * nblk, none);
  for (int p = 0; p < P; p++)
    for (int k = 0; k < nblk; k++) {
      const int n = ns[k], j0 = p * BT_KB, kb = kb_of(k, p);
      if (kb <= 0) continue;
      const int r0 = j0 + 1, mr = n - r0;
      const double *Vp = w.Vx[k].p + (size_t)j0 * n + r0;
      const int chunk = chunk_of(mr, BT_GS);
      for (int sl = 0; sl < BT_GS; sl++) {
        GemmTask g = none;
        const int k0 = sl * chunk, kk = std::max(0, std::min(chunk, mr - k0));
        g.A = g.B = Vp + (kk > 0 ? k0 : 0);
        g.C = w.G[k].p + ((size_t)sl * P + p) * BT_KB * BT_KB;
        g.tA = 1;
        g.M = g.N = kb;
        g.K = kk;
        g.lda = g.ldb = n;
        g.ldc = BT_KB;
        gram[((size_t)sl * P + p) * nblk + k] = g;
      }
      const int rp = (p & ~1) * BT_KB + 1;
      GemmTask g = none;
      g.A = w.Vx[k].p + (size_t)j0 * n + rp;
      g.B = w.T[k].p + (size_t)p * BT_KB * BT_KB;
      g.C = w.VT[k].p + (size_t)j0 * n + rp;
      g.M = n - rp;
      g.N = g.K = kb;
      g.lda = n;
      g.ldb = BT_KB;
      g.ldc = n;
      vt[(size_t)p * nblk + k] = g;
    }
  upload_cached(w.btgram, w.h_btgram, gram, s);
  upload_cached(w.bttasks, w.h_bttasks, vt, s);

  std::vector<GemmTask> cpl((size_t)BT_GS * NP * nblk, none), slab((size_t)NP * BT_S * nblk, none), upd((size_t)NP * nblk, none);
  for (int g2 = 0; g2 < NP; g2++)
    for (int k = 0; k < nblk; k++) {
      const int n = ns[k], p0 = 2 * g2, j0 = p0 * BT_KB;
      const int kb0 = kb_of(k, p0), kb1 = (p0 + 1 < P) ? kb_of(k, p0 + 1) : 0;
      if (kb0 <= 0) continue;
      const int r0 = j0 + 1, mr = n - r0, kbp = kb0 + kb1;
      if (kb1 > 0) {
        const int r1 = j0 + BT_KB + 1, m1 = n - r1;
        const int chunk = chunk_of(m1, BT_GS);
        for (int sl = 0; sl < BT_GS; sl++) {
          GemmTask c = none;
          const int k0 = sl * chunk, kk = std::max(0, std::min(chunk, m1 - k0));
          c.A = w.Vx[k].p + (size_t)j0 * n + r1 + (kk > 0 ? k0 : 0);
          c.B = w.VT[k].p + (size_t)(j0 + BT_KB) * n + r1 + (kk > 0 ? k0 : 0);
          c.C = w.Cc[k].p + ((size_t)sl * NP + g2) * BT_KB * BT_KB;
          c.tA = 1;
          c.M = kb0;
          c.N = kb1;
          c.K = kk;
          c.lda = c.ldb = n;
          c.ldc = BT_KB;
          cpl[((size_t)sl * NP + g2) * nblk + k] = c;
        }
      }
      const int chunk = chunk_of(mr, BT_S);
      for (int sl = 0; sl < BT_S; sl++) {
        GemmTask q = none;
        const int k0 = sl * chunk, kk = std::max(0, std::min(chunk, mr - k0));
        q.A = w.Vx[k].p + (size_t)j0 * n + r0 + (kk > 0 ? k0 : 0);
        q.B = b.Z[k] + r0 + (kk > 0 ? k0 : 0);
        q.C = w.Wp[k].p + (size_t)sl * BT_PW * n;
// ... 244 lines not shown
    tridiag_sel_batch(ctx, nblk, ns, nev, dp, ep, wp, zp);
  } else {
    ProfScope ps(ctx, "eig_tridiag_solve");
    w.used_dc = !tuning().tridiag_ql;
    if (!w.used_dc) {
      hipLaunchKernelGGL(k_set_identity, dim3((nmax + 255) / 256, nmax, nblk), dim3(256), 0, s, b);
      hipLaunchKernelGGL(k_tql_values, dim3(nblk), dim3(64), 0, s, b);
      hipLaunchKernelGGL(k_tql_apply, dim3((nmax + 63) / 64, nblk), dim3(64), 0, s, b);
    } else {
      double *dp[MAXB], *ep[MAXB], *zp[MAXB];
      for (int i = 0; i < nblk; i++) {
        dp[i] = w.d[i].p;
        ep[i] = w.e[i].p;
        zp[i] = w.Z[i].p;
      }
      tridiag_dc_batch(ctx, nblk, ns, dp, ep, zp);
    }
    if (nev) {
      size_t off = 0;
      for (int i = 0; i < nblk; i++) off += ns[i] + 8;
      w.selrank.resize(off);
      off = 0;
      for (int i = 0; i < nblk; i++) {
        launch_rank(ctx, w.d[i].p, ns[i], w.selrank.p + off);
        hipLaunchKernelGGL(k_take_lowest, dim3((ns[i] + 255) / 256, ns[i]), dim3(256), 0, s, w.Z[i].p, w.d[i].p, ns[i], nev[i],
                           w.selrank.p + off, w.Zs[i].p, w.Ws[i].p);
        off += ns[i] + 8;
      }
    }
  }
  if (after_solve) after_solve();
  {
    ProfScope ps(ctx, "eig_backtransform");
    if (fold) {
      HFG_HIP_CHECK(hipStreamWaitEvent(s, ctx->side_ev[1], 0));
    } else if (bt_wy) {
      bt_wy_apply(ctx, w, bz, nblk, nmax);
    } else {
    dim3 grid((nzmax + 3) / 4, nblk);
    if (nmax <= 64 * 8)
      hipLaunchKernelGGL(k_backtransform<8>, grid, dim3(256), 0, s, bz);
    else if (nmax <= 64 * 24)
      hipLaunchKernelGGL(k_backtransform<24>, grid, dim3(256), 0, s, bz);
    else {
      size_t shb = (size_t)4 * nmax * sizeof(double);
      if (shb > 64 * 1024)
        HFG_HIP_CHECK(
            hipFuncSetAttribute((const void *)k_backtransform_lds, hipFuncAttributeMaxDynamicSharedMemorySize, (int)shb));
      hipLaunchKernelGGL(k_backtransform_lds, grid, dim3(256), shb, s, bz);
    }
    }
  }
  HFG_HIP_CHECK(hipGetLastError());
}

static void check_status(hfg_ctx *ctx, EigWork &w, int nblk) {
  if (w.used_dc) {
    if (dc_status(ctx) != 0) throw std::logic_error("Eigendecomposition failed!\n");
    trdp_check_status(ctx);
    return;
  }
  for (int i = 0; i < nblk; i++) {
    int st[2];
    HFG_HIP_CHECK(hipMemcpyAsync(st, w.sweeps[i].p, 2 * sizeof(int), hipMemcpyDeviceToHost, ctx->stream));
    HFG_HIP_CHECK(hipStreamSynchronize(ctx->stream));
    if (st[1] != 0) throw std::logic_error("Eigendecomposition failed!\n");
  }
}

void eig_sym_dev(hfg_ctx *ctx, int n, const double *dA, double *dE, double *dC) {
  EigWork &w = work_for(ctx);
  w.A[0].resize((size_t)n * n + 2);
  HFG_HIP_CHECK(hipMemcpyAsync(w.A[0].p, dA, sizeof(double) * n * n, hipMemcpyDeviceToDevice, ctx->stream));
  eig_sym_batch(ctx, w, 1, &n);
  DevBuf<int> &rank = w.ibuf1;
  rank.resize(n + 8);
  launch_rank(ctx, w.d[0].p, n, rank.p);
  hipLaunchKernelGGL(k_scatter_cols, dim3((n + 255) / 256, n), dim3(256), 0, ctx->stream, w.Z[0].p, n, n,
                     (const int64_t *)nullptr, rank.p, 0, w.d[0].p, n, dC, dE);
  check_status(ctx, w, 1);
}

void eig_sym_sel_dev(hfg_ctx *ctx, int n, const double *dA, int nev, double *dE, double *dC) {
  if (nev < 1) throw std::logic_error("eig_sym_sel: nev must be at least 1\n");
  if (n < 1) throw std::logic_error("eig_sym_sel: empty matrix\n");
  nev = std::min(nev, n);
  EigWork &w = work_for(ctx);
  w.A[0].resize((size_t)n * n + 2);
  HFG_HIP_CHECK(hipMemcpyAsync(w.A[0].p, dA, sizeof(double) * n * n, hipMemcpyDeviceToDevice, ctx->stream));
  eig_sym_batch(ctx, w, 1, &n, nullptr, &nev);
  HFG_HIP_CHECK(hipMemcpyAsync(dC, w.Zs[0].p, sizeof(double) * (size_t)n * nev, hipMemcpyDeviceToDevice, ctx->stream));
  HFG_HIP_CHECK(hipMemcpyAsync(dE, w.Ws[0].p, sizeof(double) * nev, hipMemcpyDeviceToDevice, ctx->stream));
  check_status(ctx, w, 1);
}

void eig_gsym_dev(hfg_ctx *ctx, int N, int n, const double *dF, const double *dS, double *dE, double *dC) {
  EigWork &w = work_for(ctx);
  w.A[0].resize((size_t)n * n + 2);
  DevBuf<double> &T1 = ctx->ws[0];
  DevBuf<double> &Ctmp = ctx->ws[1];
  T1.resize((size_t)N * n);
  Ctmp.resize((size_t)N * n);
  {
    ProfScope ps(ctx, "eig_reduce");
    gemm_dev(ctx, false, false, N, n, N, 1.0, dF, N, dS, N, 0.0, T1.p, N);
    gemm_dev(ctx, true, false, n, n, N, 1.0, dS, N, T1.p, N, 0.0, w.A[0].p, n);
  }
  eig_sym_batch(ctx, w, 1, &n);
  {
    ProfScope ps(ctx, "eig_backtransform");
    gemm_dev(ctx, false, false, N, n, n, 1.0, dS, N, w.Z[0].p, n, 0.0, Ctmp.p, N);
  }
  DevBuf<int> &rank = w.ibuf1;
  rank.resize(n + 8);
  launch_rank(ctx, w.d[0].p, n, rank.p);
  hipLaunchKernelGGL(k_scatter_cols, dim3((N + 255) / 256, n), dim3(256), 0, ctx->stream, Ctmp.p, N, n,
                     (const int64_t *)nullptr, rank.p, 0, w.d[0].p, N, dC, dE);
  check_status(ctx, w, 1);
}

size_t eig_block_buf_size(int nblk, const int64_t *blk_ptr) {
  size_t nmax = 0;
  for (int ib = 0; ib < nblk; ib++) nmax = std::max<size_t>(nmax, blk_ptr[ib + 1] - blk_ptr[ib]);
  return (size_t)nblk * (nmax * nmax + nmax);
}

static void eig_blocks_multi_dev(hfg_ctx *ctx, int N, int nF, const double *const *dFs, const double *dS, int nblk, const int64_t *blk_ptr,
                                 const int64_t *blk_idx, double *const *dBlockBufs, int nev = 0, double *const *dEs = nullptr,
                                 double *const *dCs = nullptr);
static int eig_num_cus(hfg_ctx *ctx) {
  static const int ncu = [&] {
    hipDeviceProp_t prop;
    return (hipGetDeviceProperties(&prop, ctx->device) == hipSuccess && prop.multiProcessorCount > 0) ? prop.multiProcessorCount : 256;
  }();
  return ncu;
}
void eig_blocks_dev(hfg_ctx *ctx, int N, const double *dF, const double *dS, int nblk, const int64_t *blk_ptr,
                    const int64_t *blk_idx, double *dBlockBuf) {
  eig_blocks_multi_dev(ctx, N, 1, &dF, dS, nblk, blk_ptr, blk_idx, &dBlockBuf);
}
static void eig_blocks_multi_dev(hfg_ctx *ctx, int N, int nF, const double *const *dFs, const double *dS, int nblk, const int64_t *blk_ptr,
                                 const int64_t *blk_idx, double *const *dBlockBufs, int nev, double *const *dEs, double *const *dCs) {
  EigWork &w = work_for(ctx);
  hipStream_t s = ctx->stream;
  const bool direct = dEs != nullptr;
  if (direct && (ctx->shard_n != 1 || nF * nblk > MAXB)) throw std::logic_error("eig_blocks_multi_dev: direct path needs one rank and one batch\n");
  if (blk_ptr[nblk] != N) throw std::logic_error("Symmetry mismatch in eig_gsym_sub\n");
  DevBuf<double> &idxbuf = w.idx;
  idxbuf.resize(2 * (size_t)N + 16);
  int64_t *drows = (int64_t *)idxbuf.p;
  int64_t *dcols = drows + N;
  for (int ib = 0; ib < nblk; ib++)
    if (blk_ptr[ib + 1] == blk_ptr[ib]) throw std::logic_error("eig_gsym_sub: empty symmetry block\n");
  const bool cached = ctx->fixed_sinvh && ctx->fixed_sinvh == dS && w.sup_S == dS && w.sup_gen == ctx->fixed_gen &&
                      w.sup_N == N &&
                      w.sup_ptr.size() == (size_t)nblk + 1 && std::equal(w.sup_ptr.begin(), w.sup_ptr.end(), blk_ptr) &&
                      w.sup_idx.size() == (size_t)N && std::equal(w.sup_idx.begin(), w.sup_idx.end(), blk_idx);
  if (!cached) {
    w.sup_S = nullptr;
    w.xc_have.clear();
    HFG_HIP_CHECK(hipMemcpyAsync(drows, blk_idx, sizeof(int64_t) * N, hipMemcpyHostToDevice, s));
    DevBuf<int> &flag = w.ibuf2;
    flag.resize((size_t)N * nblk + 8);
    for (int ib = 0; ib < nblk; ib++) {
      int n = (int)(blk_ptr[ib + 1] - blk_ptr[ib]);
      hipLaunchKernelGGL(k_col_support, dim3(N), dim3(256), 0, s, dS, N, drows + blk_ptr[ib], n, flag.p + (size_t)ib * N);
    }
    std::vector<int> hflag((size_t)N * nblk);
    HFG_HIP_CHECK(hipMemcpyAsync(hflag.data(), flag.p, sizeof(int) * hflag.size(), hipMemcpyDeviceToHost, s));
    HFG_HIP_CHECK(hipStreamSynchronize(s));
    std::vector<int64_t> allcols;
    for (int ib = 0; ib < nblk; ib++) {
      int cnt = 0;
      for (int c = 0; c < N; c++)
        if (hflag[(size_t)ib * N + c]) {
          allcols.push_back(c);
          cnt++;
        }
      if (cnt != (int)(blk_ptr[ib + 1] - blk_ptr[ib]))
        throw std::logic_error("eig_gsym_sub: Sinvh is not block structured (columns with support != block size)\n");
    }
    HFG_HIP_CHECK(hipMemcpyAsync(dcols, allcols.data(), sizeof(int64_t) * N, hipMemcpyHostToDevice, s));
    HFG_HIP_CHECK(hipStreamSynchronize(s));
    if (ctx->fixed_sinvh == dS) {
      w.sup_S = dS;
      w.sup_gen = ctx->fixed_gen;
      w.sup_N = N;
      w.sup_ptr.assign(blk_ptr, blk_ptr + nblk + 1);
      w.sup_idx.assign(blk_idx, blk_idx + N);
    }
  }

  size_t nmax = 0;
  for (int ib = 0; ib < nblk; ib++) nmax = std::max<size_t>(nmax, blk_ptr[ib + 1] - blk_ptr[ib]);
  const size_t slot = nmax * nmax + nmax;
  if (!direct && ctx->shard_n > 1)
    for (int f = 0; f < nF; f++) HFG_HIP_CHECK(hipMemsetAsync(dBlockBufs[f], 0, sizeof(double) * slot * nblk, s));
  const bool keep_x = w.sup_S == dS && w.sup_S != nullptr;
  std::vector<size_t> xoff(nblk + 1, 0);
  for (int ib = 0; ib < nblk; ib++) xoff[ib + 1] = xoff[ib] + (size_t)(blk_ptr[ib + 1] - blk_ptr[ib]) * (size_t)(blk_ptr[ib + 1] - blk_ptr[ib]);
  if (keep_x) {
    if (w.xc_have.size() != (size_t)nblk || w.Xc.n < xoff[nblk]) {
      w.Xc.resize(xoff[nblk]);
      w.xc_have.assign(nblk, 0);
    }
  }
  std::vector<int64_t> koff(nblk + 1, 0);
  for (int ib = 0; ib < nblk; ib++) {
    const int64_t n = blk_ptr[ib + 1] - blk_ptr[ib];
    koff[ib + 1] = koff[ib] + (nev > 0 ? std::min<int64_t>(nev, n) : n);
  }
  const int K = (int)koff[nblk];
  DevBuf<int> &rank = w.ibuf1;
  DevBuf<double> &Etmp = ctx->ws[3];
  if (direct) {
    rank.resize((size_t)nF * (N + 8));
    Etmp.resize((size_t)nF * N);
  }

  std::vector<int> mine;
  for (int f = 0; f < nF; f++)
    for (int ib = 0; ib < nblk; ib++)
      if (ib % ctx->shard_n == ctx->shard_rank) mine.push_back(f * nblk + ib);
  DevBuf<double> &Fb = ctx->ws[5];
  DevBuf<double> &T1 = ctx->ws[0];
  DevBuf<double> &Xall = ctx->ws[4];
  Fb.resize(nmax * nmax * MAXB);
  T1.resize(nmax * nmax * MAXB);
  Xall.resize(nmax * nmax * MAXB);
  for (size_t c0 = 0; c0 < mine.size(); c0 += MAXB) {
    int nb = (int)std::min<size_t>(MAXB, mine.size() - c0);
    std::vector<int> ns(nb), nevs(nb);
    std::vector<GemmTask> gt(4 * (size_t)nb);
    const double *Xptr[MAXB];
    int nm = 0;
    for (int k = 0; k < nb; k++) {
      const int ib = mine[c0 + k] % nblk;
      double *dBlockBuf = direct ? nullptr : dBlockBufs[mine[c0 + k] / nblk];
      int n = (int)(blk_ptr[ib + 1] - blk_ptr[ib]);
      ns[k] = n;
      nevs[k] = nev > 0 ? std::min(nev, n) : n;
      nm = std::max(nm, n);
      w.A[k].resize((size_t)n * n + 2);
      if (nev > 0) w.Zs[k].resize((size_t)n * nevs[k]);
      else w.Z[k].resize((size_t)n * n);
      w.Y[k].resize((size_t)n * n);
      double *Xb = keep_x ? w.Xc.p + xoff[ib] : Xall.p + (size_t)k * nmax * nmax;
      double *Fk = Fb.p + (size_t)k * nmax * nmax, *Tk = T1.p + (size_t)k * nmax * nmax;
      Xptr[k] = Xb;
      GemmTask g;
      g.M = g.N = g.K = n;
      g.lda = g.ldb = g.ldc = n;
      g.A = Fk;
      g.B = Xb;
      g.C = Tk;
      gt[k] = g;
      g.A = Xb;
      g.tA = 1;
      g.B = Tk;
      g.C = w.A[k].p;
      g.sym = 1;
      gt[nb + k] = g;
      g.sym = 0;
      g.tA = 0;
      g.A = Xb;
      g.B = nev > 0 ? w.Zs[k].p : w.Z[k].p;
      g.N = nevs[k];
      if (direct) {
        const int f = mine[c0 + k] / nblk;
        g.C = dCs[f];
        g.ldc = N;
        g.rmap = drows + blk_ptr[ib];
        g.cmap = rank.p + (size_t)f * (N + 8) + koff[ib];
      } else
        g.C = dBlockBuf + (size_t)ib * slot;
      gt[2 * nb + k] = g;
      g.A = w.Y[k].p;
      g.tA = 1;
      gt[3 * nb + k] = g;
    }
    upload_cached(w.gtasks, w.h_gtasks, gt, s);
    {
      ProfScope ps(ctx, "eig_reduce");
      for (int k = 0; k < nb; k++) {
        const int ib = mine[c0 + k] % nblk;
        const double *dF = dFs[mine[c0 + k] / nblk];
        int n = ns[k];
        if (keep_x && w.xc_have[ib])
          hipLaunchKernelGGL(k_gather_f, dim3((n + 255) / 256, n), dim3(256), 0, s, dF, N, drows + blk_ptr[ib], n, Fb.p + (size_t)k * nmax * nmax);
        else
          hipLaunchKernelGGL(k_gather_block, dim3((n + 255) / 256, n), dim3(256), 0, s, dF, dS, N, drows + blk_ptr[ib],
                             dcols + blk_ptr[ib], n, Fb.p + (size_t)k * nmax * nmax, const_cast<double *>(Xptr[k]));
        if (keep_x) w.xc_have[ib] = 1;
      }
      const int force_split = tuning().gemm_splitk;
      long full_tiles = 0, low_tiles = 0;
      for (int k = 0; k < nb; k++) {
        const long t1 = (ns[k] + 127) / 128;
        full_tiles += t1 * t1;
        low_tiles += t1 * (t1 + 1) / 2;
      }
      const int slots = 2 * eig_num_cus(ctx);
      const bool split_full = force_split >= 0 ? force_split != 0 : (full_tiles < slots && nm >= 256);
      const bool split_low = force_split >= 0 ? force_split != 0 : (low_tiles < slots && nm >= 256);
      ProfScope pp3(ctx, "eig_products");
      const bool tile64 = force_split < 0 && !gemm_prefers_128(ctx, full_tiles);
      GemmHow full, low;
      if (tile64) full.tile = low.tile = GemmTile::T64;
      else {
        if (split_full) full.tile = GemmTile::T128, full.split2 = true;
        else if (tuning().gemm_rect) full.tile = GemmTile::T128x64;
        if (split_low) low.tile = GemmTile::T128, low.split2 = true;
      }
      w.full_how = full;
      if (full.split2)
        for (int k = 0; k < nb; k++) HFG_HIP_CHECK(hipMemsetAsync(T1.p + (size_t)k * nmax * nmax, 0, sizeof(double) * (size_t)ns[k] * ns[k], s));
      gemm_tasklist_dev(ctx, w.gtasks.p, nb, nm, nm, full);
      if (low.split2)
        for (int k = 0; k < nb; k++) HFG_HIP_CHECK(hipMemsetAsync(w.A[k].p, 0, sizeof(double) * (size_t)ns[k] * ns[k], s));
      gemm_tasklist_dev(ctx, w.gtasks.p + nb, nb, nm, nm, low);
      gemm_mirror_lower_dev(ctx, w.gtasks.p + nb, nb, nm);
    }
    std::function<void()> after_solve;
    if (direct)
      after_solve = [&] {
        if (w.used_dc) {
          if (!w.h_status) HFG_HIP_CHECK(hipHostMalloc((void **)&w.h_status, sizeof(int), hipHostMallocDefault));
          if (!w.status_ev) HFG_HIP_CHECK(hipEventCreateWithFlags(&w.status_ev, hipEventDisableTiming));
          HFG_HIP_CHECK(hipMemcpyAsync(w.h_status, dc_status_word(ctx), sizeof(int), hipMemcpyDeviceToHost, s));
          HFG_HIP_CHECK(hipEventRecord(w.status_ev, s));
        }
        ProfScope ps(ctx, "scatter");
        std::vector<const double *> csrc;
        std::vector<double *> cdst;
        std::vector<int> cn;
        for (int k = 0; k < nb; k++) {
          const int ib = mine[c0 + k] % nblk, f = mine[c0 + k] / nblk;
          csrc.push_back(nev > 0 ? w.Ws[k].p : w.d[k].p);
          cdst.push_back(Etmp.p + (size_t)f * N + koff[ib]);
          cn.push_back(nevs[k]);
        }
        copy_slices(s, csrc, cdst, cn);
        for (int f = 0; f < nF; f++) {
          int *rk = rank.p + (size_t)f * (N + 8);
          launch_rank(ctx, Etmp.p + (size_t)f * N, K, rk);
          hipLaunchKernelGGL(k_place_values, dim3((K + 255) / 256), dim3(256), 0, s, Etmp.p + (size_t)f * N, K, rk, dEs[f]);
          HFG_HIP_CHECK(hipMemsetAsync(dCs[f], 0, sizeof(double) * (size_t)N * K, s));
        }
      };
    eig_sym_batch(ctx, w, nb, ns.data(), Xptr, nev > 0 ? nevs.data() : nullptr, after_solve);
    {
      ProfScope ps(ctx, "eig_backtransform");
      if (!direct) {
        std::vector<const double *> csrc;
        std::vector<double *> cdst;
        std::vector<int> cn;
        for (int k = 0; k < nb; k++) {
          const int ib = mine[c0 + k] % nblk;
          double *slotp = dBlockBufs[mine[c0 + k] / nblk] + (size_t)ib * slot;
          csrc.push_back(nev > 0 ? w.Ws[k].p : w.d[k].p);
          cdst.push_back(slotp + nmax * nmax);
          cn.push_back(nevs[k]);
          if (nev <= 0 && w.full_how.split2 && ctx->shard_n == 1)
            HFG_HIP_CHECK(hipMemsetAsync(slotp, 0, sizeof(double) * (size_t)ns[k] * ns[k], s));
        }
        copy_slices(s, csrc, cdst, cn);
      }
      {
        ProfScope pp3(ctx, "eig_products");
        const GemmTask *last = w.gtasks.p + (w.folded ? 3 : 2) * (size_t)nb;
        GemmHow how = nev > 0 ? GemmHow{GemmTile::T64} : w.full_how;
        how.scatter = direct;
        gemm_tasklist_dev(ctx, last, nb, nm, nev > 0 ? *std::max_element(nevs.begin(), nevs.end()) : nm, how);
      }
    }
    if (direct && w.used_dc) {
      HFG_HIP_CHECK(hipEventSynchronize(w.status_ev));
      if (*w.h_status != 0) throw std::logic_error("Eigendecomposition failed!\n");
      trdp_check_status(ctx);
    } else
    check_status(ctx, w, nb);
  }
  HFG_HIP_CHECK(hipGetLastError());
}

static void eig_assemble_sel_dev(hfg_ctx *ctx, int N, int nblk, const int64_t *blk_ptr, const int64_t *blk_idx, const double *dBlockBuf,
                                 double *dE, double *dC, int nev);
void eig_assemble_dev(hfg_ctx *ctx, int N, int nblk, const int64_t *blk_ptr, const int64_t *blk_idx,
                      const double *dBlockBuf, double *dE, double *dC) {
  eig_assemble_sel_dev(ctx, N, nblk, blk_ptr, blk_idx, dBlockBuf, dE, dC, 0);
}
int64_t eig_sel_count(int nblk, const int64_t *blk_ptr, int64_t nev) { return helfem::eig_sel_count(nblk, blk_ptr, nev); }
static void eig_assemble_sel_dev(hfg_ctx *ctx, int N, int nblk, const int64_t *blk_ptr, const int64_t *blk_idx, const double *dBlockBuf,
                                 double *dE, double *dC, int nev) {
  EigWork &w = work_for(ctx);
  hipStream_t s = ctx->stream;
  ProfScope ps(ctx, "scatter");
  if (w.asm_rows.size() != (size_t)N || !std::equal(w.asm_rows.begin(), w.asm_rows.end(), blk_idx)) {
    w.asm_rows.assign(blk_idx, blk_idx + N);
    w.asm_rows_dev.resize((size_t)N + 2);
    HFG_HIP_CHECK(hipMemcpyAsync(w.asm_rows_dev.p, w.asm_rows.data(), sizeof(int64_t) * N, hipMemcpyHostToDevice, s));
  }
  int64_t *drows = (int64_t *)w.asm_rows_dev.p;
  size_t nmax = 0;
  for (int ib = 0; ib < nblk; ib++) nmax = std::max<size_t>(nmax, blk_ptr[ib + 1] - blk_ptr[ib]);
  const size_t slot = nmax * nmax + nmax;
  DevBuf<double> &Etmp = ctx->ws[3];
  Etmp.resize(N);
  std::vector<int64_t> koff(nblk + 1, 0);
  for (int ib = 0; ib < nblk; ib++) {
    const int64_t n = blk_ptr[ib + 1] - blk_ptr[ib];
    koff[ib + 1] = koff[ib] + (nev > 0 ? std::min<int64_t>(nev, n) : n);
  }
  const int K = (int)koff[nblk];
  {
    std::vector<const double *> csrc;
    std::vector<double *> cdst;
    std::vector<int> cn;
    for (int ib = 0; ib < nblk; ib++) {
      csrc.push_back(dBlockBuf + (size_t)ib * slot + nmax * nmax);
      cdst.push_back(Etmp.p + koff[ib]);
      cn.push_back((int)(koff[ib + 1] - koff[ib]));
    }
    copy_slices(s, csrc, cdst, cn);
  }
  DevBuf<int> &rank = w.ibuf1;
  rank.resize(N + 8);
  HFG_HIP_CHECK(hipMemsetAsync(dC, 0, sizeof(double) * (size_t)N * K, s));
  launch_rank(ctx, Etmp.p, K, rank.p);
  for (int ib = 0; ib < nblk; ib++) {
    int n = (int)(blk_ptr[ib + 1] - blk_ptr[ib]), nc = (int)(koff[ib + 1] - koff[ib]);
    hipLaunchKernelGGL(k_scatter_cols, dim3((n + 255) / 256, nc), dim3(256), 0, s, dBlockBuf + (size_t)ib * slot, n, nc,
                       drows + blk_ptr[ib], rank.p, (int)koff[ib], Etmp.p + koff[ib], N, dC, dE);
  }
  HFG_HIP_CHECK(hipGetLastError());
}

static void eig_gsym_sub_multi_dev(hfg_ctx *ctx, int N, int nF, const double *const *dFs, const double *dS, int nblk, const int64_t *blk_ptr,
                                   const int64_t *blk_idx, int nev, double *const *dEs, double *const *dCs) {
  int save_rank = ctx->shard_rank, save_n = ctx->shard_n;
  ctx->shard_rank = 0;
  ctx->shard_n = 1;
  try {
    if (helfem::tuning_live().eig_direct && nF * nblk <= MAXB) {
      eig_blocks_multi_dev(ctx, N, nF, dFs, dS, nblk, blk_ptr, blk_idx, nullptr, nev, dEs, dCs);
    } else {
      const size_t sz = eig_block_buf_size(nblk, blk_ptr);
      DevBuf<double> &buf = ctx->ws[6];
      buf.resize(nF * sz);
      double *bufs[MAXB];
      if (nF > MAXB) throw std::logic_error("eig_gsym_sub: too many matrices in one call\n");
      for (int f = 0; f < nF; f++) bufs[f] = buf.p + f * sz;
      eig_blocks_multi_dev(ctx, N, nF, dFs, dS, nblk, blk_ptr, blk_idx, bufs, nev);
      for (int f = 0; f < nF; f++) eig_assemble_sel_dev(ctx, N, nblk, blk_ptr, blk_idx, bufs[f], dEs[f], dCs[f], nev);
    }
  } catch (...) {
    ctx->shard_rank = save_rank;
    ctx->shard_n = save_n;
    throw;
  }
  ctx->shard_rank = save_rank;
  ctx->shard_n = save_n;
}

void eig_gsym_sub_dev(hfg_ctx *ctx, int N, const double *dF, const double *dS, int nblk, const int64_t *blk_ptr,
                      const int64_t *blk_idx, double *dE, double *dC) {
  eig_gsym_sub_multi_dev(ctx, N, 1, &dF, dS, nblk, blk_ptr, blk_idx, 0, &dE, &dC);
}

void eig_gsym_sub_sel_dev(hfg_ctx *ctx, int N, const double *dF, const double *dS, int nblk, const int64_t *blk_ptr,
                          const int64_t *blk_idx, int nev, double *dE, double *dC) {
  if (nev < 1) throw std::logic_error("eig_gsym_sub_sel: nev must be at least 1\n");
  eig_gsym_sub_multi_dev(ctx, N, 1, &dF, dS, nblk, blk_ptr, blk_idx, nev, &dE, &dC);
}

void eig_block_supports(hfg_ctx *ctx, int N, const double *dS, int nblk, const int64_t *blk_ptr, const int64_t *blk_idx,
                        std::vector<int64_t> &cols) {
  hipStream_t s = ctx->stream;
  DevBuf<int64_t> drows;
  DevBuf<int> flag;
  drows.resize(N);
  flag.resize((size_t)N * nblk + 8);
  HFG_HIP_CHECK(hipMemcpyAsync(drows.p, blk_idx, sizeof(int64_t) * N, hipMemcpyHostToDevice, s));
  for (int ib = 0; ib < nblk; ib++) {
    const int n = (int)(blk_ptr[ib + 1] - blk_ptr[ib]);
    hipLaunchKernelGGL(k_col_support, dim3(N), dim3(256), 0, s, dS, N, drows.p + blk_ptr[ib], n, flag.p + (size_t)ib * N);
  }
  std::vector<int> hflag((size_t)N * nblk);
  HFG_HIP_CHECK(hipMemcpyAsync(hflag.data(), flag.p, sizeof(int) * hflag.size(), hipMemcpyDeviceToHost, s));
  HFG_HIP_CHECK(hipStreamSynchronize(s));
  cols.clear();
  for (int ib = 0; ib < nblk; ib++) {
    int cnt = 0;
    for (int c = 0; c < N; c++)
      if (hflag[(size_t)ib * N + c]) {
        cols.push_back(c);
        cnt++;
      }
    if (cnt != (int)(blk_ptr[ib + 1] - blk_ptr[ib]))
      throw std::logic_error("eig_gsym_sub: Sinvh is not block structured (columns with support != block size)\n");
  }
}

void eig_gsym_sub_pair_dev(hfg_ctx *ctx, int N, const double *dFa, const double *dFb, const double *dS, int nblk, const int64_t *blk_ptr,
                           const int64_t *blk_idx, double *dEa, double *dCa, double *dEb, double *dCb) {
  const double *Fs[2] = {dFa, dFb};
  double *Es[2] = {dEa, dEb}, *Cs[2] = {dCa, dCb};
  eig_gsym_sub_multi_dev(ctx, N, 2, Fs, dS, nblk, blk_ptr, blk_idx, 0, Es, Cs);
}

}
```

### helfem_amd/csrc/hip/gemm.hip

```cpp
#include "internal.h"
#include <algorithm>
#include <cstdint>
#include <cstdlib>
#include <cstring>

namespace hfg {

typedef double double4_t __attribute__((ext_vector_type(4)));
typedef double d2_t __attribute__((ext_vector_type(2)));

template <int BM, int BN, bool ACC = false, int MF = 1, bool MAP = false, bool RMAP = false>
__device__ __forceinline__ void dgemm_tile(int id, int transA, int transB, int M, int N, int K, double alpha,
                                           const double *__restrict__ A, int lda, const double *__restrict__ B, int ldb,
                                           double beta, double *__restrict__ C, int ldc, double (*As)[16][BM + 16],
                                           double (*Bs)[16][BN + 16], int sym = 0, int kbeg = 0, int kend = -1, int over = 0,
                                           const int *__restrict__ amap = nullptr, const int *__restrict__ cmap = nullptr,
                                           const int64_t *__restrict__ rmap = nullptr) {
  constexpr int BK = 16;
  constexpr int PAD = 16;
  constexpr int WM = BM / 2, WN = BN / 2;
  constexpr int TM = WM / 16, TN = WN / 16;
  static_assert(PAD == 16, "LDS row padding is part of the tile types");

  int nbm = (M + BM - 1) / BM, nbn = (N + BN - 1) / BN;
  const bool lower = !ACC && sym == 1;
  int nwg = lower ? nbm * (nbm + 1) / 2 : nbm * nbn;
  if (!(over & 4)) {
    int q = nwg / 8, r = nwg % 8, xcd = id % 8;
    id = (xcd < r ? xcd * (q + 1) : r * (q + 1) + (xcd - r) * q) + id / 8;
  }
  int bm = (id % nbm) * BM, bn = (id / nbm) * BN;
  if (lower) {
    int ti = (int)((sqrt(8.0 * (double)id + 1.0) - 1.0) * 0.5);
    while (ti * (ti + 1) / 2 > id) ti--;
    while ((ti + 1) * (ti + 2) / 2 <= id) ti++;
    const int tj = id - ti * (ti + 1) / 2;
    if (ti >= nbm) return;
    bm = ti * BM;
    bn = tj * BN;
  }

  if constexpr (ACC) {
    if (sym == 2 && bm / BM + 3 < bn / BN) return;
  }
  const int tid = threadIdx.x, wave = tid >> 6, lane = tid & 63;
  const int wm = (wave & 1) * WM, wn = (wave >> 1) * WN;
  const int l15 = lane & 15, l4 = lane >> 4;

  constexpr bool V4 = (MF == 1);
  double4_t accv[V4 ? TM : 1][V4 ? TN : 1];
  double accs[V4 ? 1 : TM][V4 ? 1 : TN][4];
  if constexpr (V4) {
#pragma unroll
    for (int i = 0; i < TM; i++)
#pragma unroll
      for (int j = 0; j < TN; j++) accv[i][j] = (double4_t){0.0, 0.0, 0.0, 0.0};
  } else {
#pragma unroll
    for (int i = 0; i < TM; i++)
#pragma unroll
      for (int j = 0; j < TN; j++)
#pragma unroll
        for (int c = 0; c < 4; c++) accs[i][j][c] = 0.0;
  }
  auto acc = [&](int i, int j, int r) -> double {
    if constexpr (V4) return accv[i][j][r];
    else return accs[i][j][r];
  };

  constexpr bool PRE = ACC && (TM * TN <= 4);
  double cpre[PRE ? TM : 1][PRE ? TN : 1][4];
  if constexpr (PRE) {
#pragma unroll
    for (int i = 0; i < TM; i++)
#pragma unroll
      for (int j = 0; j < TN; j++)
#pragma unroll
        for (int r = 0; r < 4; r++) {
          int gm = min(bm + wm + i * 16 + l15, M - 1), gn = min(bn + wn + j * 16 + l4 + 4 * r, N - 1);
          cpre[i][j][r] = C[(size_t)gn * ldc + gm];
        }
  }

  constexpr int VA = BM * BK / 2 / 256, VB = BN * BK / 2 / 256;
  const bool fastA = ((reinterpret_cast<uintptr_t>(A) & 15) == 0) && ((lda & 1) == 0) && (bm + BM <= M || (over & 1));
  const bool fastB = ((reinterpret_cast<uintptr_t>(B) & 15) == 0) && ((ldb & 1) == 0) && (bn + BN <= N || (over & 2));
  const int a_mv = tid % (BM / 2), a_kc = tid / (BM / 2);
  const int a_m = tid % BM, a_kv = tid / BM;
  const int b_nv = tid % (BN / 2), b_kc = tid / (BN / 2);
  const int b_n = tid % BN, b_kv = tid / BN;
  const double *pA = MAP ? A + bm + 2 * a_mv : transA ? A + (size_t)(bm + a_m) * lda + 2 * a_kv : A + (size_t)a_kc * lda + bm + 2 * a_mv;
  const double *pB = transB ? B + (size_t)b_kc * ldb + bn + 2 * b_nv : B + (size_t)(bn + b_n) * ldb + 2 * b_kv;
  d2_t va[VA], vb[VB];
  auto load_tiles = [&](int k0) {
    const bool fullk = (k0 + BK <= K);
    if constexpr (MAP) {
      if (fastA && fullk) {
#pragma unroll
        for (int r = 0; r < VA; r++) va[r] = *reinterpret_cast<const d2_t *>(pA + (size_t)amap[k0 + a_kc + r * (512 / BM)] * lda);
      } else {
#pragma unroll
        for (int r = 0; r < VA; r++) {
          const int gm0 = bm + 2 * a_mv, gk = k0 + a_kc + r * (512 / BM);
          d2_t v = (d2_t){0.0, 0.0};
          if (gk < K) {
            const double *col = A + (size_t)amap[gk] * lda;
            if (gm0 < M) v.x = col[gm0];
            if (gm0 + 1 < M) v.y = col[gm0 + 1];
          }
          va[r] = v;
        }
      }
    } else if (fastA && fullk) {
      if (!transA) {
#pragma unroll
        for (int r = 0; r < VA; r++) va[r] = *reinterpret_cast<const d2_t *>(pA + (size_t)(k0 + r * (512 / BM)) * lda);
      } else {
#pragma unroll
        for (int r = 0; r < VA; r++) va[r] = *reinterpret_cast<const d2_t *>(pA + k0 + 2 * r * (256 / BM));
      }
    } else {
#pragma unroll
      for (int r = 0; r < VA; r++) {
        int gm0, gk0, gm1, gk1;
        if (!transA) {
          gm0 = bm + 2 * a_mv;
          gm1 = gm0 + 1;
          gk0 = gk1 = k0 + a_kc + r * (512 / BM);
        } else {
          gm0 = gm1 = bm + a_m;
          gk0 = k0 + 2 * (a_kv + r * (256 / BM));
          gk1 = gk0 + 1;
        }
        d2_t v;
        v.x = (gm0 < M && gk0 < K) ? (transA ? A[(size_t)gm0 * lda + gk0] : A[(size_t)gk0 * lda + gm0]) : 0.0;
        v.y = (gm1 < M && gk1 < K) ? (transA ? A[(size_t)gm1 * lda + gk1] : A[(size_t)gk1 * lda + gm1]) : 0.0;
        va[r] = v;
      }
    }
    if (fastB && fullk) {
      if (transB) {
#pragma unroll
        for (int r = 0; r < VB; r++) vb[r] = *reinterpret_cast<const d2_t *>(pB + (size_t)(k0 + r * (512 / BN)) * ldb);
      } else {
#pragma unroll
        for (int r = 0; r < VB; r++) vb[r] = *reinterpret_cast<const d2_t *>(pB + k0 + 2 * r * (256 / BN));
      }
    } else {
#pragma unroll
      for (int r = 0; r < VB; r++) {
        int gn0, gk0, gn1, gk1;
        if (transB) {
          gn0 = bn + 2 * b_nv;
          gn1 = gn0 + 1;
          gk0 = gk1 = k0 + b_kc + r * (512 / BN);
        } else {
          gn0 = gn1 = bn + b_n;
          gk0 = k0 + 2 * (b_kv + r * (256 / BN));
          gk1 = gk0 + 1;
        }
        d2_t v;
        v.x = (gn0 < N && gk0 < K) ? (transB ? B[(size_t)gk0 * ldb + gn0] : B[(size_t)gn0 * ldb + gk0]) : 0.0;
        v.y = (gn1 < N && gk1 < K) ? (transB ? B[(size_t)gk1 * ldb + gn1] : B[(size_t)gn1 * ldb + gk1]) : 0.0;
        vb[r] = v;
      }
    }
  };
  auto store_tiles = [&](int buf) {
    if (!transA) {
#pragma unroll
      for (int r = 0; r < VA; r++) *reinterpret_cast<d2_t *>(&As[buf][a_kc + r * (512 / BM)][2 * a_mv]) = va[r];
    } else {
#pragma unroll
      for (int r = 0; r < VA; r++) {
        As[buf][2 * (a_kv + r * (256 / BM))][a_m] = va[r].x;
        As[buf][2 * (a_kv + r * (256 / BM)) + 1][a_m] = va[r].y;
      }
    }
    if (transB) {
#pragma unroll
      for (int r = 0; r < VB; r++) *reinterpret_cast<d2_t *>(&Bs[buf][b_kc + r * (512 / BN)][2 * b_nv]) = vb[r];
    } else {
#pragma unroll
      for (int r = 0; r < VB; r++) {
        Bs[buf][2 * (b_kv + r * (256 / BN))][b_n] = vb[r].x;
        Bs[buf][2 * (b_kv + r * (256 / BN)) + 1][b_n] = vb[r].y;
      }
    }
  };

  const bool splitk = kend >= 0;
  const int kstop = splitk ? min(kend, K) : K;
  load_tiles(kbeg);
  store_tiles(0);
  __syncthreads();
  int buf = 0;
  for (int k0 = kbeg; k0 < kstop; k0 += BK) {
    const bool more = (k0 + BK < kstop);
    if (more) load_tiles(k0 + BK);
#pragma unroll
    for (int kk = 0; kk < BK; kk += 4) {
      double fa[TM];
#pragma unroll
      for (int i = 0; i < TM; i++) fa[i] = As[buf][kk + l4][wm + i * 16 + l15];
      if constexpr (MF == 1) {
        double fb[TN];
#pragma unroll
        for (int j = 0; j < TN; j++) fb[j] = Bs[buf][kk + l4][wn + j * 16 + l15];
#pragma unroll
        for (int i = 0; i < TM; i++)
#pragma unroll
          for (int j = 0; j < TN; j++)
            accv[i][j] = __builtin_amdgcn_mfma_f64_16x16x4f64(fb[j], fa[i], accv[i][j], 0, 0, 0);
      } else {
#pragma unroll
        for (int j = 0; j < TN; j++) {
          double fb[4];
#pragma unroll
          for (int c = 0; c < 4; c++) fb[c] = Bs[buf][kk + l4][wn + j * 16 + 4 * c + (lane & 3)];
#pragma unroll
          for (int i = 0; i < TM; i++)
#pragma unroll
            for (int c = 0; c < 4; c++)
              accs[i][j][c] = __builtin_amdgcn_mfma_f64_4x4x4f64(fb[c], fa[i], accs[i][j][c], 0, 0, 0);
        }
      }
    }
    if (more) store_tiles(buf ^ 1);
    __syncthreads();
    buf ^= 1;
  }
  if constexpr (PRE) {
#pragma unroll
    for (int i = 0; i < TM; i++)
#pragma unroll
      for (int j = 0; j < TN; j++)
#pragma unroll
        for (int r = 0; r < 4; r++) {
          int gm = bm + wm + i * 16 + l15, gn = bn + wn + j * 16 + l4 + 4 * r;
          if (gm < M && gn < N) C[(size_t)gn * ldc + gm] = alpha * acc(i, j, r) + beta * cpre[i][j][r];
        }
    return;
  } else if constexpr (ACC) {
    constexpr int HI = (TM > 2) ? TM / 2 : TM;
#pragma unroll
    for (int i0 = 0; i0 < TM; i0 += HI) {
      double cv[HI][TN][4];
#pragma unroll
      for (int i = 0; i < HI; i++)
#pragma unroll
        for (int j = 0; j < TN; j++)
#pragma unroll
          for (int r = 0; r < 4; r++) {
            int gm = min(bm + wm + (i0 + i) * 16 + l15, M - 1), gn = min(bn + wn + j * 16 + l4 + 4 * r, N - 1);
            cv[i][j][r] = C[(size_t)gn * ldc + gm];
          }
#pragma unroll
      for (int i = 0; i < HI; i++)
#pragma unroll
        for (int j = 0; j < TN; j++)
#pragma unroll
          for (int r = 0; r < 4; r++) {
            int gm = bm + wm + (i0 + i) * 16 + l15, gn = bn + wn + j * 16 + l4 + 4 * r;
            if (gm < M && gn < N) C[(size_t)gn * ldc + gm] = alpha * acc(i0 + i, j, r) + beta * cv[i][j][r];
          }
    }
    return;
  }
#pragma unroll
  for (int i = 0; i < TM; i++)
#pragma unroll
    for (int j = 0; j < TN; j++)
#pragma unroll
      for (int r = 0; r < 4; r++) {
        int gm = bm + wm + i * 16 + l15, gn = bn + wn + j * 16 + l4 + 4 * r;
        if (gm < M && gn < N) {
          size_t o;
          if constexpr (RMAP) o = (size_t)cmap[gn] * ldc + (size_t)rmap[gm];
          else if constexpr (MAP) o = (size_t)cmap[gn] * ldc + gm;
          else o = (size_t)gn * ldc + gm;
          double v = alpha * acc(i, j, r);
          if (splitk) {
            unsafeAtomicAdd(&C[o], v);
            continue;
          }
          if (beta != 0.0) v += beta * C[o];
          C[o] = v;
        }
      }
}

template <int BM, int BN, int MF = 1>
__global__ __launch_bounds__(256, 2) void k_dgemm(int transA, int transB, int M, int N, int K, double alpha,
                                               const double *__restrict__ A, int lda, const double *__restrict__ B,
                                               int ldb, double beta, double *__restrict__ C, int ldc) {
  __shared__ __attribute__((aligned(16))) double As[2][16][BM + 16];
  __shared__ __attribute__((aligned(16))) double Bs[2][16][BN + 16];
  dgemm_tile<BM, BN, false, MF>(blockIdx.x, transA, transB, M, N, K, alpha, A, lda, B, ldb, beta, C, ldc, As, Bs);
}

template <int BM, int BN, bool ACC = false, int MF = 1>
__global__ __launch_bounds__(256, 2) void k_dgemm_tasklist(const GemmTask *__restrict__ tasks) {
  __shared__ __attribute__((aligned(16))) double As[2][16][BM + 16];
  __shared__ __attribute__((aligned(16))) double Bs[2][16][BN + 16];
  const GemmTask t = tasks[blockIdx.y];
  if (t.M <= 0 || t.N <= 0) return;
  const int sym = (!ACC && BM == BN && t.M == t.N && t.beta == 0.0) ? (t.sym == 1) : ((ACC && t.sym == 2) ? 2 : 0);
  const int nbm = (t.M + BM - 1) / BM;
  const int nt = (sym == 1) ? nbm * (nbm + 1) / 2 : nbm * ((t.N + BN - 1) / BN);
  if ((int)blockIdx.x >= nt) return;
  dgemm_tile<BM, BN, ACC, MF>(blockIdx.x, t.tA, t.tB, t.M, t.N, t.K, t.alpha, t.A, t.lda, t.B, t.ldb, t.beta, t.C, t.ldc,
                              As, Bs, sym, 0, -1, t.over);
}

template <int MF = 1>
__global__ __launch_bounds__(256, 2) void k_dgemm_tasklist_map(const GemmTask *__restrict__ tasks) {
  __shared__ __attribute__((aligned(16))) double As[2][16][64 + 16];
  __shared__ __attribute__((aligned(16))) double Bs[2][16][64 + 16];
  const GemmTask t = tasks[blockIdx.y];
  if (t.M <= 0 || t.N <= 0) return;
  const int nt = ((t.M + 63) / 64) * ((t.N + 63) / 64);
  if ((int)blockIdx.x >= nt) return;
  dgemm_tile<64, 64, false, MF, true>(blockIdx.x, 0, 0, t.M, t.N, t.K, t.alpha, t.A, t.lda, t.B, t.ldb, 0.0, t.C, t.ldc, As, Bs, 0,
                                      0, -1, 0, t.amap, t.cmap);
}

template <int BM, int BN, int MF = 1>
__global__ __launch_bounds__(256, 2) void k_dgemm_tasklist_scatter(const GemmTask *__restrict__ tasks) {
  __shared__ __attribute__((aligned(16))) double As[2][16][BM + 16];
  __shared__ __attribute__((aligned(16))) double Bs[2][16][BN + 16];
  const GemmTask t = tasks[blockIdx.y];
  if (t.M <= 0 || t.N <= 0) return;
  const int nt = ((t.M + BM - 1) / BM) * ((t.N + BN - 1) / BN);
  if ((int)blockIdx.x >= nt) return;
  dgemm_tile<BM, BN, false, MF, false, true>(blockIdx.x, t.tA, t.tB, t.M, t.N, t.K, t.alpha, t.A, t.lda, t.B, t.ldb, 0.0, t.C, t.ldc,
                                             As, Bs, 0, 0, -1, t.over, nullptr, t.cmap, t.rmap);
}

template <int BM, int BN, bool SPLIT = false>
__global__ __launch_bounds__(256, 2) void k_dgemm_tasklist_wl(const GemmTask *__restrict__ tasks, const int2 *__restrict__ wl, int nwg) {
  __shared__ __attribute__((aligned(16))) double As[2][16][BM + 16];
  __shared__ __attribute__((aligned(16))) double Bs[2][16][BN + 16];
  const int xcd = blockIdx.x % 8, slot = blockIdx.x / 8;
  const int q8 = nwg / 8, r8 = nwg % 8;
  if (slot >= q8 + (xcd < r8 ? 1 : 0)) return;
  const int2 w = wl[(xcd < r8 ? xcd * (q8 + 1) : r8 * (q8 + 1) + (xcd - r8) * q8) + slot];
  const GemmTask t = tasks[w.x];
  if constexpr (SPLIT) {
    const int half = w.y & 1;
    const int Kh = ((t.K / 2 + 15) / 16) * 16;
    const int kbeg = half ? Kh : 0, kend = half ? t.K : Kh;
    if (kbeg >= kend) return;
    dgemm_tile<BM, BN, false, 1>(w.y >> 1, t.tA, t.tB, t.M, t.N, t.K, t.alpha, t.A, t.lda, t.B, t.ldb, 0.0, t.C, t.ldc, As, Bs, 0, kbeg,
                                 kend, t.over | 4);
  } else {
    dgemm_tile<BM, BN, false, 1>(w.y, t.tA, t.tB, t.M, t.N, t.K, t.alpha, t.A, t.lda, t.B, t.ldb, t.beta, t.C, t.ldc, As, Bs, 0, 0, -1,
                                 t.over | 4);
  }
}

template <int BM, int BN>
__global__ __launch_bounds__(256, 2) void k_dgemm_tasklist_split2(const GemmTask *__restrict__ tasks) {
  __shared__ __attribute__((aligned(16))) double As[2][16][BM + 16];
  __shared__ __attribute__((aligned(16))) double Bs[2][16][BN + 16];
  const GemmTask t = tasks[blockIdx.y];
  if (t.M <= 0 || t.N <= 0) return;
  const int sym = (BM == BN && t.M == t.N) ? (t.sym == 1) : 0;
  const int nbm = (t.M + BM - 1) / BM;
  const int nt = (sym == 1) ? nbm * (nbm + 1) / 2 : nbm * ((t.N + BN - 1) / BN);
  const int tile = blockIdx.x >> 1, half = blockIdx.x & 1;
  if (tile >= nt) return;
  const int Kh = ((t.K / 2 + 15) / 16) * 16;
  const int kbeg = half ? Kh : 0, kend = half ? t.K : Kh;
  if (kbeg >= kend) return;
  dgemm_tile<BM, BN, false, 1>(tile, t.tA, t.tB, t.M, t.N, t.K, t.alpha, t.A, t.lda, t.B, t.ldb, 0.0, t.C, t.ldc, As, Bs, sym, kbeg, kend);
}
template <int BM, int BN>
__global__ __launch_bounds__(256, 2) void k_dgemm_tasklist_split2_scatter(const GemmTask *__restrict__ tasks) {
  __shared__ __attribute__((aligned(16))) double As[2][16][BM + 16];
  __shared__ __attribute__((aligned(16))) double Bs[2][16][BN + 16];
  const GemmTask t = tasks[blockIdx.y];
  if (t.M <= 0 || t.N <= 0) return;
  const int nt = ((t.M + BM - 1) / BM) * ((t.N + BN - 1) / BN);
  const int tile = blockIdx.x >> 1, half = blockIdx.x & 1;
  if (tile >= nt) return;
  const int Kh = ((t.K / 2 + 15) / 16) * 16;
  const int kbeg = half ? Kh : 0, kend = half ? t.K : Kh;
  if (kbeg >= kend) return;
  dgemm_tile<BM, BN, false, 1, false, true>(tile, t.tA, t.tB, t.M, t.N, t.K, t.alpha, t.A, t.lda, t.B, t.ldb, 0.0, t.C, t.ldc, As, Bs, 0,
                                            kbeg, kend, 0, nullptr, t.cmap, t.rmap);
}

__global__ __launch_bounds__(256) void k_mirror_lower(const GemmTask *__restrict__ tasks) {
  __shared__ double tile[64][65];
  const GemmTask t = tasks[blockIdx.y];
  if (t.sym != 1 || t.M <= 0 || t.M != t.N) return;
  const int nb = (t.M + 63) / 64;
  int bi = (int)((1.0 + sqrt(1.0 + 8.0 * (double)blockIdx.x)) * 0.5);
  while (bi * (bi - 1) / 2 > (int)blockIdx.x) bi--;
  while ((bi + 1) * bi / 2 <= (int)blockIdx.x) bi++;
  const int bj = blockIdx.x - bi * (bi - 1) / 2;
  if (bi >= nb) return;
  const int tx = threadIdx.x & 63, ty = threadIdx.x >> 6;
  for (int c = ty; c < 64; c += 4) {
    int gm = bi * 64 + tx, gn = bj * 64 + c;
    tile[c][tx] = (gm < t.M && gn < t.N) ? t.C[(size_t)gn * t.ldc + gm] : 0.0;
  }
  __syncthreads();
  for (int c = ty; c < 64; c += 4) {
    int gm = bj * 64 + tx, gn = bi * 64 + c;
    if (gm < t.M && gn < t.N) t.C[(size_t)gn * t.ldc + gm] = tile[tx][c];
  }
}

void gemm_mirror_lower_dev(hfg_ctx *ctx, const GemmTask *dtasks, int ntasks, int maxN) {
  if (ntasks <= 0 || maxN <= 64) return;
  const int nb = (maxN + 63) / 64;
  hipLaunchKernelGGL(k_mirror_lower, dim3(nb * (nb - 1) / 2, ntasks), dim3(256), 0, ctx->stream, dtasks);
  HFG_HIP_CHECK(hipGetLastError());
}

static bool mfma4() { return tuning().mfma_4x4x4; }

namespace {
struct TileShape {
  int bm, bn;
};
TileShape tile_shape(GemmTile tile) {
  switch (tile) {
    case GemmTile::T64: return {64, 64};
    case GemmTile::T128: return {128, 128};
    case GemmTile::T128x64: return {128, 64};
    default: throw std::logic_error("GEMM tile engine: GemmTile::Auto names no tile shape");
  }
}
int tile_count(TileShape s, int M, int N) { return ((M + s.bm - 1) / s.bm) * ((N + s.bn - 1) / s.bn); }
const char *tile_name(GemmTile tile) {
  const char *names[] = {"Auto", "T64", "T128", "T128x64"};
  return (unsigned)tile < 4u ? names[(int)tile] : "(unknown)";
}

typedef void (*TaskKernel)(const GemmTask *);
constexpr int ACC = 1, SPLIT2 = 2, MAP = 4, SCATTER = 8;
constexpr int variant(GemmTile tile, int flags) { return 16 * (int)tile + flags; }
TaskKernel tasklist_kernel(GemmTile tile, const GemmHow &how) {
  const bool m4 = mfma4();
  switch (variant(tile, how.acc * ACC + how.split2 * SPLIT2 + how.map * MAP + how.scatter * SCATTER)) {
    case variant(GemmTile::T64, 0): return m4 ? k_dgemm_tasklist<64, 64, false, 0> : k_dgemm_tasklist<64, 64>;
    case variant(GemmTile::T128, 0): return m4 ? k_dgemm_tasklist<128, 128, false, 0> : k_dgemm_tasklist<128, 128>;
    case variant(GemmTile::T128x64, 0): return k_dgemm_tasklist<128, 64>;
    case variant(GemmTile::T64, ACC): return m4 ? k_dgemm_tasklist<64, 64, true, 0> : k_dgemm_tasklist<64, 64, true>;
    case variant(GemmTile::T128, ACC): return m4 ? k_dgemm_tasklist<128, 128, true, 0> : k_dgemm_tasklist<128, 128, true>;
    case variant(GemmTile::T64, MAP): return m4 ? k_dgemm_tasklist_map<0> : k_dgemm_tasklist_map<1>;
    case variant(GemmTile::T128, SPLIT2): return k_dgemm_tasklist_split2<128, 128>;
    case variant(GemmTile::T128x64, SPLIT2): return k_dgemm_tasklist_split2<128, 64>;
    case variant(GemmTile::T64, SCATTER): return m4 ? k_dgemm_tasklist_scatter<64, 64, 0> : k_dgemm_tasklist_scatter<64, 64>;
    case variant(GemmTile::T128, SCATTER): return m4 ? k_dgemm_tasklist_scatter<128, 128, 0> : k_dgemm_tasklist_scatter<128, 128>;
    case variant(GemmTile::T128x64, SCATTER): return k_dgemm_tasklist_scatter<128, 64>;
    case variant(GemmTile::T128, SPLIT2 + SCATTER): return k_dgemm_tasklist_split2_scatter<128, 128>;
    case variant(GemmTile::T128x64, SPLIT2 + SCATTER): return k_dgemm_tasklist_split2_scatter<128, 64>;
    default:
      throw std::logic_error(std::string("gemm_tasklist_dev: no kernel for tile ") + tile_name(tile) + (how.acc ? " acc" : "") +
                             (how.split2 ? " split2" : "") + (how.map ? " map" : "") + (how.scatter ? " scatter" : ""));
  }
}
}

void gemm_tasklist_dev(hfg_ctx *ctx, const GemmTask *dtasks, int ntasks, int maxM, int maxN, GemmHow how) {
  if (ntasks <= 0 || maxM <= 0 || maxN <= 0) return;
  GemmTile tile = how.tile;
  if (tile == GemmTile::Auto)
    tile = (ntasks <= 65535 && !gemm_prefers_128(ctx, (long)ntasks * tile_count({128, 128}, maxM, maxN))) ? GemmTile::T64 : GemmTile::T128;
  const TaskKernel kernel = tasklist_kernel(tile, how);
  const int tiles = tile_count(tile_shape(tile), maxM, maxN) * (how.split2 ? 2 : 1);
  ProfScope ps(ctx, "gemm");
  for (int t0 = 0; t0 < ntasks; t0 += 65535)
    hipLaunchKernelGGL(kernel, dim3(tiles, std::min(65535, ntasks - t0)), dim3(256), 0, ctx->stream, dtasks + t0);
  HFG_HIP_CHECK(hipGetLastError());
}

void gemm_worklist(const std::vector<GemmTask> &tasks, GemmTile tile, bool split2, std::vector<int2> &out) {
  const TileShape shape = tile_shape(tile);
  out.clear();
  for (size_t t = 0; t < tasks.size(); t++) {
    if (tasks[t].M <= 0 || tasks[t].N <= 0) continue;
    const int n = tile_count(shape, tasks[t].M, tasks[t].N) * (split2 ? 2 : 1);
    for (int q = 0; q < n; q++) out.push_back(make_int2((int)t, q));
  }
}

void gemm_worklist_dev(hfg_ctx *ctx, const GemmTask *dtasks, const int2 *dwl, int nwg, GemmTile tile, bool split2) {
  void (*kernel)(const GemmTask *, const int2 *, int) = nullptr;
  if (split2) {
    if (tile == GemmTile::T128x64) kernel = k_dgemm_tasklist_wl<128, 64, true>;
  } else if (tile == GemmTile::T128) kernel = k_dgemm_tasklist_wl<128, 128>;
  else if (tile == GemmTile::T128x64) kernel = k_dgemm_tasklist_wl<128, 64>;
  else if (tile == GemmTile::T64) kernel = k_dgemm_tasklist_wl<64, 64>;
  if (!kernel) throw std::logic_error(std::string("gemm_worklist_dev: no kernel for tile ") + tile_name(tile) + (split2 ? " split2" : ""));
  if (nwg <= 0) return;
  ProfScope ps(ctx, "gemm");
  hipLaunchKernelGGL(kernel, dim3(8u * (unsigned)((nwg + 7) / 8)), dim3(256), 0, ctx->stream, dtasks, dwl, nwg);
  HFG_HIP_CHECK(hipGetLastError());
}

bool gemm_prefers_128(hfg_ctx *ctx, long tiles128) {
  if (tuning().gemm_tile) return tuning().gemm_tile == 128;
  static const int slots = [&] {
    int ncu = 256;
    (void)hipDeviceGetAttribute(&ncu, hipDeviceAttributeMultiprocessorCount, ctx->device);
    return 2 * ncu;
  }();
  const long rounds = (tiles128 + slots - 1) / slots;
  return tiles128 >= slots / 2 && (double)tiles128 >= 0.85 * (double)(rounds * slots);
}

void gemm_dev(hfg_ctx *ctx, bool tA, bool tB, int M, int N, int K, double alpha, const double *A, int lda,
              const double *B, int ldb, double beta, double *C, int ldc) {
  if (M <= 0 || N <= 0) return;
  ProfScope ps(ctx, "gemm");
  const long big_tiles = (long)((M + 127) / 128) * ((N + 127) / 128);
  const bool big = gemm_prefers_128(ctx, big_tiles), m4 = mfma4();
  const long tiles = big ? big_tiles : (long)((M + 63) / 64) * ((N + 63) / 64);
  const auto kernel = big ? (m4 ? k_dgemm<128, 128, 0> : k_dgemm<128, 128>) : (m4 ? k_dgemm<64, 64, 0> : k_dgemm<64, 64>);
  hipLaunchKernelGGL(kernel, dim3((unsigned)tiles), dim3(256), 0, ctx->stream, (int)tA, (int)tB, M, N, K, alpha, A, lda, B, ldb, beta, C,
                     ldc);
  HFG_HIP_CHECK(hipGetLastError());
}

}
```

### helfem_amd/csrc/hip/internal.h

```cpp
#pragma once
#include "common.h"
#include "tables.h"
#include "../host/scf.h"

namespace hfg {

enum class GemmTile { Auto, T64, T128, T128x64 };
struct GemmHow {
  GemmTile tile = GemmTile::Auto;
  bool acc = false, split2 = false, map = false, scatter = false;
};
void gemm_tasklist_dev(hfg_ctx *ctx, const GemmTask *dtasks, int ntasks, int maxM, int maxN, GemmHow how = {});
void gemm_worklist_dev(hfg_ctx *ctx, const GemmTask *dtasks, const int2 *dwl, int nwg, GemmTile tile, bool split2 = false);
void gemm_worklist(const std::vector<GemmTask> &tasks, GemmTile tile, bool split2, std::vector<int2> &out);
void gemm_mirror_lower_dev(hfg_ctx *ctx, const GemmTask *dtasks, int ntasks, int maxN);
bool gemm_prefers_128(hfg_ctx *ctx, long tiles128);
void gemm_dev(hfg_ctx *ctx, bool tA, bool tB, int M, int N, int K, double alpha, const double *A, int lda, const double *B, int ldb,
              double beta, double *C, int ldc);

void coulomb_dev(hfg_ctx *ctx, hfg_basis *basis, const double *dP, double *dJ);
void coulomb_batch_dev(hfg_ctx *ctx, hfg_basis *basis, int64_t nP, const double *dP, double *dJ);
void coulomb_energy_matrix_dev(hfg_ctx *ctx, hfg_basis *basis, int64_t nP, const double *dP, double *dW);
void set_xc_params(hfg_ctx *ctx, int x_func, const double *x_pars, int nx, int c_func, const double *c_pars, int nc);
void xc_eval_host(int id, int nspin, size_t np, const double *rho, const double *sigma, const double *lapl, const double *tau,
                  double *exc, double *vrho, double *vsigma, double *vlapl, double *vtau, double thr);
void xc_eval_host_ext(int id, const double *pars, int npars, int nspin, size_t np, const double *rho, const double *sigma,
                      const double *lapl, const double *tau, double *exc, double *vrho, double *vsigma, double *vlapl, double *vtau,
                      double thr);
void xc_fock_dev(hfg_ctx *ctx, hfg_basis *basis, int x_func, int c_func, const double *dP, double *dH, double *dScal,
                 double thr);
void xc_fock_pol_dev(hfg_ctx *ctx, hfg_basis *basis, int x_func, int c_func, const double *dPa, const double *dPb, double *dHa,
                     double *dHb, double *dScal, double thr);
void model_potential_dev(hfg_ctx *ctx, hfg_basis *basis, int kind1, int Z1, double d1, double H1, int kind2, int Z2, double d2,
                         double H2, double *dH);
void set_fock_blocks(hfg_ctx *ctx, hfg_basis *basis, const int *dBlockId);
size_t fock_compact_size(hfg_basis *basis);
void fock_compact_dev(hfg_ctx *ctx, hfg_basis *basis, int x_func, int c_func, const double *dP, double *dFc, double *dScal,
                      double thr);
void fock_finish_dev(hfg_ctx *ctx, hfg_basis *basis, const double *dFc, const double *dH0, const int *dBlockId,
                     double *dF);
void fock_compact_pol_dev(hfg_ctx *ctx, hfg_basis *basis, int x_func, int c_func, const double *dPa, const double *dPb,
                          double *dFc, double *dScal, double thr);
void fock_finish_pol_dev(hfg_ctx *ctx, hfg_basis *basis, const double *dFc, const double *dH0, const int *dBlockId,
                         double *dFa, double *dFb);

enum class ExTables { coulomb, screened, mix };
hfg_dev_tables *exchange_tables(hfg_basis *basis, ExTables which);
void exchange_dev(hfg_ctx *ctx, hfg_basis *basis, const double *dP, double *dK, ExTables which = ExTables::coulomb,
                  const double *Lknown = nullptr, int rknown = 0);
bool exchange_lowrank_dev(hfg_ctx *ctx, hfg_dev_tables *t, const double *dP, double *dK, const double *Lknown,
                          int rknown);
void exchange_batch_dev(hfg_ctx *ctx, hfg_basis *basis, int64_t nP, const double *dP, double *dK, ExTables which = ExTables::coulomb,
                        const double *dC = nullptr, const int64_t *nocc = nullptr, int64_t ldc = 0);

constexpr double EXL_PAIR_MAX_BYTES = 32e9;
int mix_exchange_tables_dev(hfg_ctx *ctx, hfg_basis *basis, double alpha, double beta);

void compute_tei_dev(hfg_ctx *ctx, hfg_basis *basis);

void compute_rs_tei_dev(hfg_ctx *ctx, hfg_basis *basis, int rs_kind, double omega);
void rs_special_dev(hfg_ctx *ctx, int which, int L, const double *a, const double *b, size_t n, double *out);

void eig_sym_dev(hfg_ctx *ctx, int n, const double *dA, double *dE, double *dC);
void eig_gsym_dev(hfg_ctx *ctx, int N, int n, const double *dF, const double *dS, double *dE, double *dC);
void eig_gsym_sub_dev(hfg_ctx *ctx, int N, const double *dF, const double *dS, int nblk, const int64_t *blk_ptr,
                      const int64_t *blk_idx, double *dE, double *dC);
void eig_gsym_sub_pair_dev(hfg_ctx *ctx, int N, const double *dFa, const double *dFb, const double *dS, int nblk,
                           const int64_t *blk_ptr, const int64_t *blk_idx, double *dEa, double *dCa, double *dEb,
                           double *dCb);
size_t eig_block_buf_size(int nblk, const int64_t *blk_ptr);
void eig_blocks_dev(hfg_ctx *ctx, int N, const double *dF, const double *dS, int nblk, const int64_t *blk_ptr,
                    const int64_t *blk_idx, double *dBlockBuf);
void eig_assemble_dev(hfg_ctx *ctx, int N, int nblk, const int64_t *blk_ptr, const int64_t *blk_idx, const double *dBlockBuf,
                      double *dE, double *dC);
void eig_block_supports(hfg_ctx *ctx, int N, const double *dS, int nblk, const int64_t *blk_ptr, const int64_t *blk_idx,
                        std::vector<int64_t> &cols);
int64_t eig_sel_count(int nblk, const int64_t *blk_ptr, int64_t nev);
void eig_sym_sel_dev(hfg_ctx *ctx, int n, const double *dA, int nev, double *dE, double *dC);
void eig_gsym_sub_sel_dev(hfg_ctx *ctx, int N, const double *dF, const double *dS, int nblk, const int64_t *blk_ptr,
                          const int64_t *blk_idx, int nev, double *dE, double *dC);

void tridiag_dc_batch(hfg_ctx *ctx, int nblk, const int *ns, double *const *d, double *const *e, double *const *Z);
int dc_status(hfg_ctx *ctx);
int *dc_status_word(hfg_ctx *ctx);
void tridiag_sel_batch(hfg_ctx *ctx, int nblk, const int *ns, const int *nev, double *const *d, double *const *e, double *const *W,
                       double *const *Z);
void tridiagonalize_batch(hfg_ctx *ctx, int nblk, const int *ns, double *const *A, double *const *d, double *const *e,
                          double *const *tau);
void trd_measure_gemv(hfg_ctx *ctx, double *ms, int64_t *launches);
bool tridiagonalize_takes_chain(int nblk, const int *ns);
void tridiagonalize_persistent(hfg_ctx *ctx, int nblk, const int *ns, double *const *A, double *const *d, double *const *e,
                               double *const *tau, std::vector<char> &done);
void trdp_check_status(hfg_ctx *ctx);

void form_sinvh_dev(hfg_ctx *ctx, int N, const double *dS, bool chol, int nblk, const int64_t *blk_ptr, const int64_t *blk_idx,
                    double *dSinvh);
void form_density_dev(hfg_ctx *ctx, int N, int ncols, const double *dC, int nocc, double *dP);

constexpr int DIIS_LR_MAXCOLS = 64;
constexpr int DIIS_HIST_CHUNK = 8;
struct DiisErrTask {
  const double *A, *B;
  double *out;
  int n, k, ld, ldo;
};
struct DiisHistory {
  const double *E[DIIS_HIST_CHUNK], *P[DIIS_HIST_CHUNK], *F[DIIS_HIST_CHUNK];
  int n;
};
struct DiisComb {
  const double *F[16];
  double w[16];
  int n;
};
size_t diis_lowrank_partials(int ntasks, int nmax);
void diis_lowrank_error_dev(hfg_ctx *ctx, const DiisErrTask *dtasks, int ntasks, int nmax, double *dPartialMax,
                            double *dMax);
void diis_history_dev(hfg_ctx *ctx, const DiisHistory &h, int j0, int nhtot, const double *dEnew, size_t elen, const double *dPnew,
                      const double *dFnew, size_t flen, bool want_max, double *dPartial, double *dRes);
void diis_extrapolate_dev(hfg_ctx *ctx, const DiisComb &c, size_t NN, int nspin, double *dFa, double *dFb);

constexpr int CUHF_LR_MAXCOLS = 128;
void cuhf_lowrank_dev(hfg_ctx *ctx, int N, const double *dS, const double *dCa, int nocca, const double *dCb, int noccb, double *dFa,
                      double *dFb);
void cuhf_dense_dev(hfg_ctx *ctx, int N, int n, const double *dP, const double *dSh, const double *dSinvh, int nocca, int noccb,
                    double *dFa, double *dFb);

helfem::scf::Result scf_device_loop(hfg_ctx *ctx, hfg_basis *hb, const helfem::scf::Options &opt, int nel, double Enucr, int symm,
                                    const std::vector<std::vector<size_t> > &dsym, int ldft, int mdft,
                                    const std::vector<std::vector<std::vector<size_t> > > &avg_idx =
                                        std::vector<std::vector<std::vector<size_t> > >());

}
```

### helfem_amd/csrc/host/tuning.h

```cpp
#pragma once
#include <string>

namespace helfem {
constexpr int EXL_GMAX = 16;
enum class TrdMode { persistent, chain, twokernel, unblocked };
enum class EigSel { crossover, stein, dc };
enum class RsTei { host, dev };
#define HELFEM_TUNING(X) \
  X(scf_host, bool, false, "HELFEM_SCF", true, "=host", !strcmp(e, "host"), "SCF loop driven from the host through the per-stage entry points (checker of the device-resident loop)") \
  X(tei_host, bool, false, "HELFEM_TEI", false, "=host", !strcmp(e, "host"), "in-element tables built by the threaded host code and uploaded (checker of tei_dev.hip)") \
  X(rs_tei, RsTei, RsTei::host, "HELFEM_RS_TEI", false, "word", !strcmp(e, "dev") ? RsTei::dev : RsTei::host, "range-separated exchange tables of the SCF drivers: dev = built on the device (rs_tei_dev.hip); unset or any other word = built by the threaded host code and uploaded") \
  X(exchange_general, bool, false, "HELFEM_EXCHANGE", true, "=general", !strcmp(e, "general"), "general exchange kernels always, not only where the low-rank fast path declines") \
  X(exl_rb, int, 0, "HELFEM_EXL_RB", false, "int", atoi(e), "RB kernel of the low-rank exchange: 4 the 4 x 4 vector kernel, 1 the one-pair vector kernel (checkers), else the matrix-core kernel k_exl_RBm") \
  X(exl_mgroups, bool, true, "HELFEM_EXL_MGROUPS", false, "off if 0", atoi(e) != 0, "cross-element products by blocks of equal m; off: the full products") \
  X(exl_rect, int, -1, "HELFEM_EXL_RECT", false, "int", atoi(e), "tiles of the element GEMM: 0 / 1 / 2 = 128 x 128 / 128 x 64 / 64 x 64 always; negative: 64 x 64 when the tasks average fewer than 1500 pairs, else 128 x 128") \
  X(exl_wl, bool, true, "HELFEM_EXL_WL", false, "off if 0", atoi(e) != 0, "XCD-contiguous workgroup lists for the element GEMM and the cross products; off: plain task-list grids") \
  X(exl_splitk, bool, true, "HELFEM_EXL_SPLITK", false, "off if 0", atoi(e) != 0, "two half-K workgroups per tile for the cross products; off: one workgroup per tile") \
  X(exl_crect, bool, true, "HELFEM_EXL_CRECT", false, "off if 0", atoi(e) != 0, "128 x 64 tiles for the split cross products; off: 128 x 128") \
  X(exl_groups, int, 4, "HELFEM_EXL_GROUPS", false, "int", std::max(1, std::min(EXL_GMAX, atoi(e))), "groups of 64 factors tried before the general kernels take over, clamped to 1 ... 16") \
  X(exl_hint, bool, true, "HELFEM_EXL_HINT", false, "off if 0", atoi(e) != 0, "the SCF loop's occupied orbitals taken as the factors of P; off: always factorise and verify P (checker)") \
  X(exl_pair, bool, true, "HELFEM_EXL_PAIR", false, "off if 0", atoi(e) != 0, "low-rank fast path for the pair (erfc) tables; off: general kernels") \
  X(exl_mix, int, -1, "HELFEM_EXL_MIX", true, "int", atoi(e), "range-separated hybrids in the step objects: 0 = K from two builds, hfg_exchange_occ_dev and hfg_rs_exchange_dev, added on the device (checker); other non-negative = one build on the mixed-kernel table set (hfg_mix_exchange_tables); negative: by kernel kind as measured, the mixed set for both Yukawa and erfc") \
  X(fock_overlap, bool, true, "HELFEM_FOCK_OVERLAP", false, "off if 0", atoi(e) != 0, "Coulomb kernels on the side stream beside the XC kernels; off: one after the other on the main stream") \
  X(fock_skip, bool, true, "HELFEM_FOCK_SKIP", true, "off if 0", atoi(e) != 0, "Fock build skips shell pairs whose density block is zero and, after hfg_ctx_set_fock_blocks, pairs the caller does not read; off: every pair is computed (checker)") \
  X(xc_lds_limit, size_t, 150 * 1024, "HELFEM_XC_LDS_LIMIT", false, "int", (size_t)atol(e), "bytes of LDS the angular XC kernels plan with; smaller forces the chunked kernels (tests)") \
  X(coulomb_batch_chunk, int, 0, "HELFEM_COULOMB_BATCH_CHUNK", true, "int", std::max(0, atoi(e)), "densities per pass over the tables of the batched Coulomb build forced smaller than the LDS rule allows (tests; 0: the rule's own)") \
  X(exchange_batch_chunk, int, 0, "HELFEM_EXCHANGE_BATCH_CHUNK", true, "int", std::max(0, atoi(e)), "densities per pass over the tables of the batched exchange build at most (tests; 0: as many as fit the 64 factor columns of a pass)") \
  X(uscf_kbatch, bool, false, "HELFEM_USCF_KBATCH", true, "=1", atoi(e) == 1, "DeviceUSCFStep: K[Pa] and K[Pb] through one call of hfg_exchange_occ_batch_devptr; off: one call per spin") \
  X(diis_blocks, bool, true, "HELFEM_DIIS_BLOCKS", false, "off if 0", atoi(e) != 0, "DIIS error per symmetry block; off: the four dense N^3 products (checker)") \
  X(diis_lowrank, bool, true, "HELFEM_DIIS_LOWRANK", false, "off if 0", atoi(e) != 0, "blocked DIIS error from the occupied orbitals; off: per-block n^3 products from F and P (checker)") \
  X(cuhf_lowrank, bool, true, "HELFEM_CUHF_LOWRANK", true, "off if 0", atoi(e) != 0, "hfg_cuhf_update_devptr: the constraint from the occupied orbitals (rank na + nb, up to 128 columns); off: the dense natural-orbital sequence always (checker)") \
  X(eig_pair, bool, true, "HELFEM_EIG_PAIR", false, "off if 0", atoi(e) != 0, "both spins' Fock matrices in one batched eigensolve; off: two calls") \
  X(eig_direct, bool, true, "HELFEM_EIG_DIRECT", true, "off if 0", atoi(e) != 0, "one-call blocked eigensolve (hfg_eig_gsym_sub_dev, _sel_dev, _pair_devptr) ranks before its last product and stores that product straight into C; off: block slots, then hfg_eig_assemble_dev (checker)") \
  X(trd_mode, TrdMode, TrdMode::persistent, "HELFEM_TRD", false, "word", !strcmp(e, "persistent") ? TrdMode::persistent : !strcmp(e, "twokernel") ? TrdMode::twokernel : !strcmp(e, "unblocked") ? TrdMode::unblocked : TrdMode::chain, "tridiagonalisation: persistent = k_trdp where the batch fits, else the chain; chain (and any unknown word) = one k_trdf launch per column always (checker); twokernel = k_trdb_gemv + k_trdb_w; unblocked = the first-generation kernels") \
  X(trdp_min, int, 256, "HELFEM_TRDP_MIN", false, "int", atoi(e), "smallest order the persistent kernel takes") \
  X(trdp_r, int, 0, "HELFEM_TRDP_R", false, "int", atoi(e), "rows per thread of the persistent kernel forced (0: the first that fits)") \
  X(trdp_u, int, 0, "HELFEM_TRDP_U", false, "int", atoi(e), "column chunks per thread of the persistent kernel forced wider than needed (measurement; 0: narrowest)") \
  X(trdp_limit_ms, long long, 200, "HELFEM_TRDP_LIMIT_MS", false, "int", atoll(e), "wall-clock bound of every spin of the persistent kernel, ms") \
  X(trdp_phases, bool, true, "HELFEM_TRDP_PHASES", false, "off if 0", atoi(e) != 0, "one cooperative launch per phase; off: the whole matrix in one launch (checker)") \
  X(trdp_step, int, 96, "HELFEM_TRDP_STEP", false, "int", std::max(1, atoi(e)), "fewest columns of a phase (at least 1)") \
  X(trdp_coop, bool, true, "HELFEM_TRDP_COOP", false, "off if 0", atoi(e) != 0, "hipLaunchCooperativeKernel for the phases; off: plain launches (A/B of the launch overhead)") \
  X(trdp_stamps, int, 0, "HELFEM_TRDP_STAMPS", false, "int", atoi(e), "non-zero: the stamping kernels, one launch per eigensolve, phase summary on stderr; 2 and more: also per-column stamps of one workgroup") \
  X(trdp_stamps_file, std::string, "", "HELFEM_TRDP_STAMPS_FILE", false, "path", e, "with stamps: file for the stamps of every workgroup over 64 columns (tools/trdp_window.py)") \
  X(trd_tail, int, 2, "HELFEM_TRD_TAIL", false, "int", atoi(e), "last columns of the chain in one launch: 0 none, 1 the LDS-resident kernel (order 128), else the register-resident kernel (order 192)") \
  X(trdf_sym, int, -1, "HELFEM_TRDF_SYM", false, "int", atoi(e), "symmetric sweep of k_trdf: 0 never, other non-negative always, negative by HELFEM_TRDF_SYM_MIN") \
  X(trdf_sym_min, int, 0, "HELFEM_TRDF_SYM_MIN", false, "int", atoi(e), "panels whose full grid has more tiles than this sweep one triangle only") \
  X(trd_band_update, bool, true, "HELFEM_TRD_BAND_UPDATE", false, "off if 0", atoi(e) != 0, "band-limited trailing updates when every sweep is symmetric; off: full updates") \
  X(trdf_nth, int, 0, "HELFEM_TRDF_NTH", false, "int", atoi(e), "512: k_trdf with 512 threads; anything else 1024 (A/B runs)") \
  X(acc_tile, int, 0, "HELFEM_ACC_TILE", false, "int", atoi(e), "128: 128 x 128 tiles for the accumulating updates (and full, not band-limited ones); anything else 64 x 64") \
  X(trdf_dbg, int, 0, "HELFEM_TRDF_DBG", false, "int", atoi(e), "measurement replay of k_trdf only: bits 0-2 go to the kernel's debug field, bit 2 also prints the per-wave stamps (tools/trdf_probe.py)") \
  X(trdf_c, int, -1, "HELFEM_TRDF_C", false, "int", atoi(e), "measurement replay of k_trdf only: column-in-panel index forced for every launch (negative: each launch's own)") \
  X(tridiag_ql, bool, false, "HELFEM_TRIDIAG", false, "=ql", !strcmp(e, "ql"), "one-lane implicit QL for the tridiagonal problem instead of divide and conquer (checker)") \
  X(dc_gemm_small, bool, false, "HELFEM_DC_GEMM", false, "=small", !strcmp(e, "small"), "Q U of the divide-and-conquer merges by the first 64 x 64 kernel instead of the tile engine (checker)") \
  X(dc_levels, bool, false, "HELFEM_DC", false, "=levels", !strcmp(e, "levels"), "divide-and-conquer merges with the gather, scatter and copy-back passes over Q and ten launches per level (checker of the column-mapped product)") \
  X(eigsel, EigSel, EigSel::crossover, "HELFEM_EIGSEL", false, "word", !strcmp(e, "stein") ? EigSel::stein : !strcmp(e, "dc") ? EigSel::dc : EigSel::crossover, "selected eigenpairs (hfg_eig_*_sel): stein = multisection and inverse iteration always; dc = the full divide and conquer, then the lowest columns (checker); unset or any other word = the crossover, which sends every wanted fraction to dc (measured: stein is slower down to 1/64 of the columns)") \
  X(dc_dbg, bool, false, "HELFEM_DC_DBG", false, "present", true, "merge statistics of divide and conquer on stderr") \
  X(bt_column, bool, false, "HELFEM_BT", false, "=column", !strcmp(e, "column"), "back-transformation reflector by reflector instead of compact WY (checker)") \
  X(bt_fold, bool, true, "HELFEM_BT_FOLD", false, "off if 0", atoi(e) != 0, "X Q formed on the side stream beside divide and conquer; off: Z <- Q Z on the main stream behind it") \
  X(bt_side, bool, false, "HELFEM_BT_SIDE", false, "=1", atoi(e) == 1, "without the fold: the compact-WY set-up on the side stream") \
  X(gemm_tile, int, 0, "HELFEM_GEMM_TILE", false, "int", atoi(e), "128: 128 x 128 tiles always; other non-zero: 64 x 64 always; 0: the large tiles where they fill whole rounds of the chip") \
  X(gemm_splitk, int, -1, "HELFEM_GEMM_SPLITK", false, "int", atoi(e), "eigensolve's products: 0 / other non-negative = large tiles without / with two half-K workgroups each; negative: chosen by tile count") \
  X(gemm_rect, bool, false, "HELFEM_GEMM_RECT", false, "on if not 0", atoi(e) != 0, "128 x 64 tiles for the eigensolve's large-tile products") \
  X(mfma_4x4x4, bool, false, "HELFEM_MFMA", false, "=4x4x4", !strcmp(e, "4x4x4"), "v_mfma_f64_4x4x4_4b_f64 in the tile engine instead of v_mfma_f64_16x16x4_f64 (A/B runs)") \
  X(num_threads, int, 0, "HELFEM_NUM_THREADS", true, "int", std::max(0, atoi(e)), "host threads of the set-up code (0: one per core, 64 at most)") \
  X(hdf5_lib, std::string, "", "HELFEM_HDF5_LIB", true, "path", e, "HDF5 library tried before the usual names")

struct Tuning {
#define X(field, type, def, ...) type field = def;
  HELFEM_TUNING(X)
#undef X
};
const Tuning &tuning();
Tuning tuning_live();
std::string tuning_table();
}
```

### include/helfem_gpu.h

```cpp
#ifndef HELFEM_GPU_H
#define HELFEM_GPU_H

#include <stddef.h>
#include <stdint.h>

#ifdef __cplusplus
extern "C" {
#endif

typedef struct hfg_ctx hfg_ctx;
typedef struct hfg_basis hfg_basis;

#define HFG_NULL_STREAM ((void *)(intptr_t)-1)
int hfg_ctx_create(hfg_ctx **ctx, int device, void *stream);
int hfg_ctx_destroy(hfg_ctx *ctx);
int hfg_ctx_synchronize(hfg_ctx *ctx);
const char *hfg_last_error(void);
const char *hfg_version(void);
int hfg_device_count(void);

int hfg_ctx_set_shard(hfg_ctx *ctx, int rank, int nranks);

int hfg_ctx_fix_sinvh(hfg_ctx *ctx, const double *dSinvh);

typedef struct {
  int Z1, Z2;
  double Rhalf;
  int primbas;
  int nnodes;
  int nquad;
  const double *bval;
  int nbval;
  const int *lval;
  const int *mval;
  int nang;
  int lpad;
} hfg_diatomic_desc;

int hfg_diatomic_basis_create(const hfg_diatomic_desc *desc, hfg_basis **basis);

typedef struct {
  int Z;
  int primbas;
  int nnodes;
  int nquad;
  const double *bval;
  int nbval;
  const int *lval;
  const int *mval;
  int nang;
} hfg_atomic_desc;
int hfg_atomic_basis_create(const hfg_atomic_desc *desc, hfg_basis **basis);
typedef struct {
  hfg_atomic_desc base;
  int finitenuc;
  double Rrms;
  int zeroder;
  int Zl, Zr;
  double Rmid;
} hfg_atomic_desc_ex;
int hfg_atomic_basis_create_ex(const hfg_atomic_desc_ex *desc, hfg_basis **basis);
int hfg_basis_confinement(const hfg_basis *basis, int iconf, int N, double R, double V, double shift, double *out);
int hfg_atomic_grid(int finitenuc, double Rrms, int nelem, double Rmax, int grid, double zexp, int nelem0, int grid0,
                    double zexp0, int Z, int Zl, int Zr, double Rmid, int add_conf, double shift_conf, double *bval, int *n);
int hfg_angular_basis(int lmax, int mmax, int *lval, int *mval, int *nang );
int hfg_basis_destroy(hfg_basis *basis);
int hfg_basis_dims(const hfg_basis *basis, int64_t *Nbf, int64_t *Ndummy, int64_t *Nrad, int64_t *Nang,
                   int64_t *Nel);
int hfg_basis_overlap(const hfg_basis *basis, double *S);
int hfg_basis_kinetic(const hfg_basis *basis, double *T);
int hfg_basis_nuclear(const hfg_basis *basis, double *V);
int hfg_basis_sym_blocks(const hfg_basis *basis, int symm, int *nblk, int64_t *blk_ptr, int64_t *blk_idx);
int hfg_compute_tei(hfg_basis *basis, int exchange);
int hfg_compute_rs_tei(hfg_basis *basis, int rs_kind, double omega);
int hfg_compute_rs_tei_dev(hfg_ctx *ctx, hfg_basis *basis, int rs_kind, double omega);
int hfg_compute_tei_dev(hfg_ctx *ctx, hfg_basis *basis, int exchange);
int hfg_diis_weights(int n, const double *B, const double *T, const double *E, double maxerr, double diiseps, double diisthr,
                     int mode, double *w, int *dropped);

typedef struct hfg_diis hfg_diis;
int hfg_diis_create(hfg_ctx *ctx, int64_t N, int nspin , int order, double diiseps, double diisthr,
                    int mode , hfg_diis **d);
int hfg_diis_destroy(hfg_diis *d);
int hfg_diis_set_metric_devptr(hfg_diis *d, const double *dS, const double *dSinvh, int64_t n);
int hfg_diis_set_blocks(hfg_diis *d, int nblk, const int64_t *blk_ptr, const int64_t *blk_idx);
int hfg_diis_update_devptr(hfg_diis *d, double E, const double *dFa, const double *dPa, const double *dCa, int64_t nocca,
                           const double *dFb, const double *dPb, const double *dCb, int64_t noccb, double *maxerr );
int hfg_diis_solve_devptr(hfg_diis *d, double *dFa, double *dFb, int *dropped);
int hfg_diis_size(const hfg_diis *d);
int hfg_diis_get(hfg_diis *d, int which, double *out, int64_t cap);

int hfg_basis_interbasis_overlap(const hfg_basis *a, const hfg_basis *b, double *S12);
int hfg_basis_lm_map(const hfg_basis *basis, int *L, int *M, int *n);
int hfg_basis_get_prim(hfg_ctx *ctx, const hfg_basis *basis, int which, int ilm, int iel, double *out, int64_t *rows,
                       int64_t *cols);
int hfg_radial_grid(double mumax, int nelem, int igrid, double zexp, double *bval );
int hfg_lm_list(const int *lmmax, int nlm, int *lval, int *mval, int *nang );

double hfg_gaunt_coefficient(int L, int M, int l, int m, int lp, int mp);
double hfg_modified_gaunt_coefficient(int lj, int mj, int L, int M, int li, int mi);
void hfg_legendre_PQ(int Lmax, int Mmax, double xi, double *P, double *Q);
double hfg_theta_lm(int l, int m, double cth);
double hfg_bessel_il(double x, int L);
double hfg_bessel_kl(double x, int L);
double hfg_erfc_phi(int n, double Xi, double xi);
void hfg_set_erfc_binomial_mode(int mode);
int hfg_rs_special_dev(hfg_ctx *ctx, int which, int L, const double *a, const double *b, int64_t n, double *out);
void hfg_chebyshev_rule(int n, double *x, double *w);
void hfg_lobatto_nodes(int n, double *x);

int hfg_basis_upload(hfg_ctx *ctx, hfg_basis *basis, int ldft, int mdft);

int hfg_coulomb(hfg_ctx *ctx, hfg_basis *basis, const double *P, double *J);
int hfg_coulomb_batch(hfg_ctx *ctx, hfg_basis *basis, int64_t nP, const double *P, double *J);
int hfg_coulomb_energy_matrix(hfg_ctx *ctx, hfg_basis *basis, int64_t nP, const double *P, double *W);
int hfg_exchange(hfg_ctx *ctx, hfg_basis *basis, const double *P, double *K);
int hfg_rs_exchange(hfg_ctx *ctx, hfg_basis *basis, const double *P, double *K);
int hfg_exchange_batch(hfg_ctx *ctx, hfg_basis *basis, int64_t nP, const double *P, double *K);
int hfg_rs_exchange_batch(hfg_ctx *ctx, hfg_basis *basis, int64_t nP, const double *P, double *K);
int hfg_xc_fock(hfg_ctx *ctx, hfg_basis *basis, int x_func, int c_func, const double *P, double *H, double *Exc,
                double *Nel, double *Ekin, double dens_thr);
int hfg_xc_fock_pol(hfg_ctx *ctx, hfg_basis *basis, int x_func, int c_func, const double *Pa, const double *Pb,
                    double *Ha, double *Hb, double *Exc, double *Nel, double *Ekin, double dens_thr);
int hfg_xc_fock_ext(hfg_ctx *ctx, hfg_basis *basis, int x_func, const double *x_pars, int n_x_pars, int c_func,
                    const double *c_pars, int n_c_pars, const double *P, double *H, double *Exc, double *Nel, double *Ekin,
                    double dens_thr);
int hfg_xc_fock_pol_ext(hfg_ctx *ctx, hfg_basis *basis, int x_func, const double *x_pars, int n_x_pars, int c_func,
                        const double *c_pars, int n_c_pars, const double *Pa, const double *Pb, double *Ha, double *Hb,
                        double *Exc, double *Nel, double *Ekin, double dens_thr);
int hfg_xc_eval(int func_id, int nspin, int64_t np, const double *rho, const double *sigma, const double *lapl, const double *tau,
                double *exc, double *vrho, double *vsigma, double *vlapl, double *vtau, double dens_thr);
int hfg_xc_eval_ext(int func_id, const double *pars, int n_pars, int nspin, int64_t np, const double *rho, const double *sigma,
                    const double *lapl, const double *tau, double *exc, double *vrho, double *vsigma, double *vlapl, double *vtau,
                    double dens_thr);
int hfg_xc_func_ids(const char *method, int *x_func, int *c_func);
const char *hfg_xc_func_name(int func_id);
int hfg_xc_exact_exchange(int x_func, double *omega, double *alpha, double *beta);
int hfg_xc_rs_kind(int x_func);
int hfg_xc_func_table(char *buf, size_t cap);
int hfg_basis_radial_table(const hfg_basis *basis, int which, int iel, double *out, int64_t *rows, int64_t *cols);
typedef struct {
  int kind;
  int Z;
  double d, H;
} hfg_model_pot;
int hfg_model_potential(hfg_ctx *ctx, hfg_basis *basis, const hfg_model_pot *p1, const hfg_model_pot *p2, double *H);
int hfg_scf_set_iguess(int iguess);
int hfg_eig_gsym(hfg_ctx *ctx, int64_t N, int64_t n, const double *F, const double *Sinvh, double *E, double *C);
int hfg_eig_gsym_sub(hfg_ctx *ctx, int64_t N, const double *F, const double *Sinvh, int nblk,
                     const int64_t *blk_ptr, const int64_t *blk_idx, double *E, double *C);
int hfg_eig_gsym_sub_pair(hfg_ctx *ctx, int64_t N, const double *Fa, const double *Fb, const double *Sinvh, int nblk,
                          const int64_t *blk_ptr, const int64_t *blk_idx, double *Ea, double *Ca, double *Eb, double *Cb);
int hfg_eig_sym(hfg_ctx *ctx, int64_t n, const double *A, double *E, double *C);
int64_t hfg_eig_sel_count(int nblk, const int64_t *blk_ptr, int64_t nev);
int hfg_eig_sym_sel(hfg_ctx *ctx, int64_t n, const double *A, int64_t nev, double *E, double *C);
int hfg_eig_gsym_sub_sel(hfg_ctx *ctx, int64_t N, const double *F, const double *Sinvh, int nblk, const int64_t *blk_ptr,
                         const int64_t *blk_idx, int64_t nev, double *E , double *C );
int hfg_form_sinvh(hfg_ctx *ctx, int64_t N, const double *S, int chol, int nblk, const int64_t *blk_ptr,
                   const int64_t *blk_idx, double *Sinvh);
int hfg_form_density(hfg_ctx *ctx, int64_t N, int64_t ncols, const double *C, int64_t nocc, double *P);
int hfg_gemm(hfg_ctx *ctx, int transA, int transB, int64_t m, int64_t n, int64_t k, const double *A, int64_t lda,
             const double *B, int64_t ldb, double *C, int64_t ldc);

int hfg_coulomb_dev(hfg_ctx *ctx, hfg_basis *basis, const double *dP, double *dJ);
int hfg_coulomb_batch_devptr(hfg_ctx *ctx, hfg_basis *basis, int64_t nP, const double *dP, double *dJ);
int hfg_exchange_dev(hfg_ctx *ctx, hfg_basis *basis, const double *dP, double *dK);
int hfg_rs_exchange_dev(hfg_ctx *ctx, hfg_basis *basis, const double *dP, double *dK);
int hfg_exchange_occ_dev(hfg_ctx *ctx, hfg_basis *basis, const double *dP, const double *dC, int64_t nocc, double *dK);
int hfg_exchange_batch_devptr(hfg_ctx *ctx, hfg_basis *basis, int64_t nP, const double *dP, double *dK);
int hfg_rs_exchange_batch_devptr(hfg_ctx *ctx, hfg_basis *basis, int64_t nP, const double *dP, double *dK);
int hfg_exchange_occ_batch_devptr(hfg_ctx *ctx, hfg_basis *basis, int64_t nP, const double *dP, const double *dC,
                                  const int64_t *nocc, int64_t ldc_cols, double *dK);
int hfg_mix_exchange_tables(hfg_ctx *ctx, hfg_basis *basis, double alpha, double beta);
int hfg_mix_exchange(hfg_ctx *ctx, hfg_basis *basis, const double *P, double *K);
int hfg_mix_exchange_devptr(hfg_ctx *ctx, hfg_basis *basis, const double *dP, double *dK);
int hfg_mix_exchange_occ_devptr(hfg_ctx *ctx, hfg_basis *basis, const double *dP, const double *dC, int64_t nocc, double *dK);
// ... 158 lines not shown
```

Measured before the change: 7.924 ms.

## Exploit radial-element band pattern of Fock in eigensolve F·X product

Adds a declared radial-element sparsity pattern for the Fock matrix, checked once against H0 on the GPU. Under that pattern, the symmetry-blocked eigensolve reorders F rows radial-major and computes F·X as 64-row tile tasks that only visit the k-steps touching each tile's non-zero columns, using a new k-list GEMM kernel. This is meant to skip the structurally zero parts of the dense product. It adds host planning and synchronisation on cache misses, plus a gather kernel. It also assumes the XC and J contributions respect the same element pattern as H0.

```diff
diff --git a/helfem_amd/__init__.py b/helfem_amd/__init__.py
--- a/helfem_amd/__init__.py
+++ b/helfem_amd/__init__.py
@@ -210,6 +210,22 @@
     def fix_sinvh(self, device_ptr):
         _check(lib().hfg_ctx_fix_sinvh(self.h, ctypes.c_void_p(device_ptr or 0)))
 
+    FOCK_BAND_STATES = ("none", "declared", "refused")
+
+    def declare_fock_band(self, basis, H0_ptr=None, blockid_ptr=None):
+        f = lib().hfg_ctx_declare_fock_band
+        f.argtypes = [ctypes.c_void_p, ctypes.c_void_p, ctypes.c_void_p, ctypes.c_void_p, c_int_p]
+        st = ctypes.c_int()
+        _check(f(self.h, basis.h, ctypes.c_void_p(H0_ptr or 0), ctypes.c_void_p(blockid_ptr or 0), ctypes.byref(st)))
+        return self.FOCK_BAND_STATES[st.value]
+
+    def fock_band_state(self):
+        f = lib().hfg_ctx_fock_band_state
+        f.argtypes = [ctypes.c_void_p, c_int_p]
+        st = ctypes.c_int()
+        _check(f(self.h, ctypes.byref(st)))
+        return self.FOCK_BAND_STATES[st.value]
+
     def profile(self, on=True):
         _check(lib().hfg_profile_enable(self.h, 1 if on else 0))
 
@@ -655,6 +671,21 @@
     n = ctypes.c_int(0)
     _check(lib().hfg_exchange_batch_plan(len(r), r.ctypes.data_as(c_int_p), int(max_members), out.ctypes.data_as(c_int_p), ctypes.byref(n)))
     return out.tolist(), n.value
+
+
+def eig_band_plan(node, pm, E):
+    nd = np.ascontiguousarray(node, dtype=np.int32)
+    n = len(nd)
+    nt = (n + 63) // 64
+    cap = nt * ((n + 15) // 16)
+    perm = np.zeros(n, dtype=np.int64)
+    toff, ks = np.zeros(nt + 1, dtype=np.int32), np.zeros(max(cap, 1), dtype=np.int32)
+    banded = ctypes.c_int(0)
+    f = lib().hfg_eig_band_plan
+    f.argtypes = [ctypes.c_int64, c_int_p, ctypes.c_int, ctypes.c_int, c_i64_p, c_int_p, c_int_p, ctypes.c_int64, c_int_p]
+    _check(f(n, nd.ctypes.data_as(c_int_p), int(pm), int(E), perm.ctypes.data_as(c_i64_p), toff.ctypes.data_as(c_int_p),
+             ks.ctypes.data_as(c_int_p), cap, ctypes.byref(banded)))
+    return perm, [ks[toff[t]:toff[t + 1]].copy() for t in range(nt)], bool(banded.value)
 
 
 class DFTGrid(object):
@@ -1272,6 +1303,8 @@
         self.ctx.fix_sinvh(None)
         self.Sinvh = t.from_numpy(np.asfortranarray(Sinvh).ravel(order="F").copy()).to(self.dev)
         self.ctx.fix_sinvh(self.Sinvh.data_ptr())
+        if not self.anyK and not self._applies_cuhf:
+            self.ctx.declare_fock_band(self.basis, self.H0.data_ptr(), self.blockid.data_ptr())
 
     def set_density(self, P, C=None):
         self.P.copy_(self.torch.from_numpy(np.asfortranarray(P).ravel(order="F").copy()))
diff --git a/helfem_amd/csrc/hip/capi.cpp b/helfem_amd/csrc/hip/capi.cpp
--- a/helfem_amd/csrc/hip/capi.cpp
+++ b/helfem_amd/csrc/hip/capi.cpp
@@ -3,6 +3,7 @@
 #include "../host/diis.h"
 #include "../host/dftfuncs.h"
 #include "../host/exchange_batch_plan.h"
+#include "../host/eig_band_plan.h"
 #include "../host/fock_need.h"
 #include <cstring>
 #include <memory>
@@ -191,6 +192,52 @@
 int hfg_ctx_fix_sinvh(hfg_ctx *c, const double *dSinvh) {
   HFG_TRY
   c->fix_sinvh(dSinvh);
+  HFG_CATCH
+}
+
+int hfg_ctx_declare_band(hfg_ctx *c, int64_t N, const int *node, int pm, int E, const double *dH0, const int *dBlockId, int *state) {
+  HFG_TRY
+  if (!c) throw std::logic_error("hfg_ctx_declare_band: null context\n");
+  const int st = eig_declare_band(c, (int)N, node, pm, E, dH0, dBlockId);
+  if (state) *state = st;
+  HFG_CATCH
+}
+
+int hfg_ctx_declare_fock_band(hfg_ctx *c, hfg_basis *b, const double *dH0, const int *dBlockId, int *state) {
+  HFG_TRY
+  if (!c || !b) throw std::logic_error("hfg_ctx_declare_fock_band: null context or basis\n");
+  const hfg_dev_tables *t = b->dev;
+  if (!t) throw std::logic_error("hfg_ctx_declare_fock_band: the basis tables are not uploaded\n");
+  std::vector<int> node;
+  node.reserve(t->N);
+  for (int s = 0; s < t->A; s++)
+    for (int n = (t->h_shell_skip[s] ? 1 : 0); n < t->R; n++) node.push_back(n);
+  if ((int)node.size() != t->N) throw std::logic_error("hfg_ctx_declare_fock_band: basis tables and basis size disagree\n");
+  const int st = eig_declare_band(c, t->N, node.data(), t->p - 1, t->E, dH0, dBlockId);
+  if (state) *state = st;
+  HFG_CATCH
+}
+
+int hfg_ctx_fock_band_state(hfg_ctx *c, int *state) {
+  HFG_TRY
+  if (!c || !state) throw std::logic_error("hfg_ctx_fock_band_state: null pointer\n");
+  *state = c->band_state;
+  HFG_CATCH
+}
+
+int hfg_eig_band_plan(int64_t n, const int *node, int pm, int E, int64_t *perm, int *toff, int *kstart, int64_t cap, int *banded) {
+  HFG_TRY
+  if (n < 1 || pm < 1 || E < 1) throw std::logic_error("hfg_eig_band_plan: empty block or basis\n");
+  if (!node || !perm || !toff || !kstart) throw std::logic_error("hfg_eig_band_plan: null pointer\n");
+  for (int64_t i = 0; i < n; i++)
+    if (node[i] < 0 || node[i] > pm * E) throw std::logic_error("hfg_eig_band_plan: radial node outside the elements\n");
+  helfem::eig_band_order(n, node, perm);
+  std::vector<int> ks, to;
+  const bool b = helfem::eig_band_plan(n, node, perm, pm, E, ks, to);
+  if ((int64_t)ks.size() > cap) throw std::logic_error("hfg_eig_band_plan: output capacity too small\n");
+  std::copy(to.begin(), to.end(), toff);
+  std::copy(ks.begin(), ks.end(), kstart);
+  if (banded) *banded = b ? 1 : 0;
   HFG_CATCH
 }
 
diff --git a/helfem_amd/csrc/hip/common.h b/helfem_amd/csrc/hip/common.h
--- a/helfem_amd/csrc/hip/common.h
+++ b/helfem_amd/csrc/hip/common.h
@@ -87,7 +87,12 @@
   void fix_sinvh(const double *p) {
     fixed_sinvh = p;
     fixed_gen++;
+    band_node.clear();
+    band_state = 0;
   }
+  std::vector<int> band_node;
+  int band_pm = 0, band_E = 0;
+  int band_state = 0;
   hfg::DevBuf<int> fock_need, fock_gneed;
   const hfg_dev_tables *fock_need_tables = nullptr;
   int fock_need_A = 0, fock_need_G = 0;
@@ -142,8 +147,11 @@
   int over = 0;
   const int *amap = nullptr, *cmap = nullptr;
   const int64_t *rmap = nullptr;
+  const int *kstart = nullptr;
+  int nk = 0;
+  int kpad = 0;
 };
-static_assert(sizeof(GemmTask) == 104, "GemmTask is compared bytewise: keep it free of padding");
+static_assert(sizeof(GemmTask) == 120, "GemmTask is compared bytewise: keep it free of padding");
 
 struct ProfScope {
   hfg_ctx *c;
diff --git a/helfem_amd/csrc/hip/eig.hip b/helfem_amd/csrc/hip/eig.hip
--- a/helfem_amd/csrc/hip/eig.hip
+++ b/helfem_amd/csrc/hip/eig.hip
@@ -1,6 +1,7 @@
 #include "internal.h"
 #include "wave.h"
 #include "../host/eigsel_count.h"
+#include "../host/eig_band_plan.h"
 #include <cstdlib>
 #include <cstring>
 #include <functional>
@@ -42,6 +43,14 @@
   int j = blockIdx.y;
   if (i >= n) return;
   Fb[(size_t)j * n + i] = F[(size_t)rows[j] * N + rows[i]];
+}
+
+__global__ void k_gather_f2(const double *__restrict__ F, int N, const int64_t *__restrict__ irows, const int64_t *__restrict__ jrows,
+                            int n, double *__restrict__ Fb) {
+  int i = blockIdx.x * blockDim.x + threadIdx.x;
+  int j = blockIdx.y;
+  if (i >= n) return;
+  Fb[(size_t)j * n + i] = F[(size_t)jrows[j] * N + irows[i]];
 }
 
 __global__ void k_col_support(const double *__restrict__ S, int N, const int64_t *__restrict__ rows, int n,
@@ -602,6 +611,13 @@
   std::vector<int64_t> sup_ptr, sup_idx;
   DevBuf<double> Xc;
   std::vector<char> xc_have;
+  std::vector<int64_t> band_rows, band_pos;
+  std::vector<int> band_ks, band_koff, band_toff;
+  bool band_any = false;
+  DevBuf<long long> band_rows_dev, band_pos_dev;
+  DevBuf<int> band_ks_dev, band_iota_dev;
+  DevBuf<GemmTask> fxtasks;
+  std::vector<GemmTask> h_fxtasks;
   int *h_status = nullptr;
   hipEvent_t status_ev = nullptr;
   ~EigWork() {
@@ -1152,13 +1168,54 @@
   int64_t *dcols = drows + N;
   for (int ib = 0; ib < nblk; ib++)
     if (blk_ptr[ib + 1] == blk_ptr[ib]) throw std::logic_error("eig_gsym_sub: empty symmetry block\n");
+  const bool want_band = ctx->fixed_sinvh && ctx->fixed_sinvh == dS && ctx->band_state == 1 && ctx->band_node.size() == (size_t)N &&
+                         helfem::tuning_live().eig_band;
   const bool cached = ctx->fixed_sinvh && ctx->fixed_sinvh == dS && w.sup_S == dS && w.sup_gen == ctx->fixed_gen &&
-                      w.sup_N == N &&
+                      w.sup_N == N && want_band == !w.band_rows.empty() &&
                       w.sup_ptr.size() == (size_t)nblk + 1 && std::equal(w.sup_ptr.begin(), w.sup_ptr.end(), blk_ptr) &&
                       w.sup_idx.size() == (size_t)N && std::equal(w.sup_idx.begin(), w.sup_idx.end(), blk_idx);
   if (!cached) {
     w.sup_S = nullptr;
     w.xc_have.clear();
+    HFG_HIP_CHECK(hipStreamSynchronize(s));
+    w.band_rows.clear();
+    w.band_pos.clear();
+    w.band_ks.clear();
+    w.band_koff.assign(1, 0);
+    w.band_toff.assign(1, 0);
+    w.band_any = false;
+    if (want_band) {
+      w.band_rows.resize(N);
+      w.band_pos.resize(N);
+      std::vector<int> nd, ks, toff;
+      int64_t nbig = 0;
+      for (int ib = 0; ib < nblk; ib++) {
+        const int64_t o = blk_ptr[ib], n = blk_ptr[ib + 1] - o;
+        nbig = std::max(nbig, n);
+        nd.resize(n);
+        for (int64_t i = 0; i < n; i++) {
+          if (blk_idx[o + i] < 0 || blk_idx[o + i] >= N) throw std::logic_error("eig_gsym_sub: block index out of range\n");
+          nd[i] = ctx->band_node[blk_idx[o + i]];
+        }
+        helfem::eig_band_order(n, nd.data(), w.band_pos.data() + o);
+        for (int64_t i = 0; i < n; i++) w.band_rows[o + i] = blk_idx[o + w.band_pos[o + i]];
+        if (helfem::eig_band_plan(n, nd.data(), w.band_pos.data() + o, ctx->band_pm, ctx->band_E, ks, toff)) w.band_any = true;
+        for (size_t t = 0; t + 1 < toff.size(); t++) w.band_koff.push_back((int)w.band_ks.size() + toff[t + 1]);
+        w.band_ks.insert(w.band_ks.end(), ks.begin(), ks.end());
+        w.band_toff.push_back((int)w.band_koff.size() - 1);
+      }
+      std::vector<int> iota(nbig);
+      for (int64_t i = 0; i < nbig; i++) iota[i] = (int)i;
+      w.band_rows_dev.resize(N);
+      w.band_pos_dev.resize(N);
+      w.band_ks_dev.resize(w.band_ks.size() + 1);
+      w.band_iota_dev.resize(nbig);
+      HFG_HIP_CHECK(hipMemcpyAsync(w.band_rows_dev.p, w.band_rows.data(), sizeof(int64_t) * N, hipMemcpyHostToDevice, s));
+      HFG_HIP_CHECK(hipMemcpyAsync(w.band_pos_dev.p, w.band_pos.data(), sizeof(int64_t) * N, hipMemcpyHostToDevice, s));
+      HFG_HIP_CHECK(hipMemcpyAsync(w.band_ks_dev.p, w.band_ks.data(), sizeof(int) * w.band_ks.size(), hipMemcpyHostToDevice, s));
+      HFG_HIP_CHECK(hipMemcpyAsync(w.band_iota_dev.p, iota.data(), sizeof(int) * nbig, hipMemcpyHostToDevice, s));
+      HFG_HIP_CHECK(hipStreamSynchronize(s));
+    }
     HFG_HIP_CHECK(hipMemcpyAsync(drows, blk_idx, sizeof(int64_t) * N, hipMemcpyHostToDevice, s));
     DevBuf<int> &flag = w.ibuf2;
     flag.resize((size_t)N * nblk + 8);
@@ -1280,25 +1337,50 @@
       gt[3 * nb + k] = g;
     }
     upload_cached(w.gtasks, w.h_gtasks, gt, s);
+    std::vector<GemmTask> fx;
+    if (w.band_any && !w.band_rows.empty()) {
+      for (int k = 0; k < nb; k++) {
+        const int ib = mine[c0 + k] % nblk;
+        const int n = ns[k], nt = w.band_toff[ib + 1] - w.band_toff[ib];
+        for (int t = 0; t < nt; t++) {
+          const int i0 = t * helfem::EIG_BAND_TILE, q = w.band_toff[ib] + t;
+          GemmTask g = gt[k];
+          g.A = gt[k].A + i0;
+          g.M = std::min(helfem::EIG_BAND_TILE, n - i0);
+          g.rmap = (const int64_t *)w.band_pos_dev.p + blk_ptr[ib] + i0;
+          g.cmap = w.band_iota_dev.p;
+          g.kstart = w.band_ks_dev.p + w.band_koff[q];
+          g.nk = w.band_koff[q + 1] - w.band_koff[q];
+          fx.push_back(g);
+        }
+      }
+      std::stable_sort(fx.begin(), fx.end(), [](const GemmTask &a, const GemmTask &b) { return a.nk > b.nk; });
+      upload_cached(w.fxtasks, w.h_fxtasks, fx, s);
+    }
     {
       ProfScope ps(ctx, "eig_reduce");
-      for (int k = 0; k < nb; k++) {
-        const int ib = mine[c0 + k] % nblk;
-        const double *dF = dFs[mine[c0 + k] / nblk];
-        int n = ns[k];
-        if (keep_x && w.xc_have[ib])
-          hipLaunchKernelGGL(k_gather_f, dim3((n + 255) / 256, n), dim3(256), 0, s, dF, N, drows + blk_ptr[ib], n, Fb.p + (size_t)k * nmax * nmax);
-        else
-          hipLaunchKernelGGL(k_gather_block, dim3((n + 255) / 256, n), dim3(256), 0, s, dF, dS, N, drows + blk_ptr[ib],
-                             dcols + blk_ptr[ib], n, Fb.p + (size_t)k * nmax * nmax, const_cast<double *>(Xptr[k]));
-        if (keep_x) w.xc_have[ib] = 1;
-      }
       const int force_split = tuning().gemm_splitk;
       long full_tiles = 0, low_tiles = 0;
       for (int k = 0; k < nb; k++) {
         const long t1 = (ns[k] + 127) / 128;
         full_tiles += t1 * t1;
         low_tiles += t1 * (t1 + 1) / 2;
+      }
+      const bool band_fx = !fx.empty() && force_split < 0 && !gemm_prefers_128(ctx, full_tiles) && !tuning().mfma_4x4x4;
+      for (int k = 0; k < nb; k++) {
+        const int ib = mine[c0 + k] % nblk;
+        const double *dF = dFs[mine[c0 + k] / nblk];
+        int n = ns[k];
+        double *Fk = Fb.p + (size_t)k * nmax * nmax;
+        if (!(keep_x && w.xc_have[ib]))
+          hipLaunchKernelGGL(k_gather_block, dim3((n + 255) / 256, n), dim3(256), 0, s, dF, dS, N, drows + blk_ptr[ib],
+                             dcols + blk_ptr[ib], n, Fk, const_cast<double *>(Xptr[k]));
+        else if (!band_fx)
+          hipLaunchKernelGGL(k_gather_f, dim3((n + 255) / 256, n), dim3(256), 0, s, dF, N, drows + blk_ptr[ib], n, Fk);
+        if (band_fx)
+          hipLaunchKernelGGL(k_gather_f2, dim3((n + 255) / 256, n), dim3(256), 0, s, dF, N, (const int64_t *)w.band_rows_dev.p + blk_ptr[ib],
+                             drows + blk_ptr[ib], n, Fk);
+        if (keep_x) w.xc_have[ib] = 1;
       }
       const int slots = 2 * eig_num_cus(ctx);
       const bool split_full = force_split >= 0 ? force_split != 0 : (full_tiles < slots && nm >= 256);
@@ -1315,7 +1397,13 @@
       w.full_how = full;
       if (full.split2)
         for (int k = 0; k < nb; k++) HFG_HIP_CHECK(hipMemsetAsync(T1.p + (size_t)k * nmax * nmax, 0, sizeof(double) * (size_t)ns[k] * ns[k], s));
-      gemm_tasklist_dev(ctx, w.gtasks.p, nb, nm, nm, full);
+      if (band_fx) {
+        GemmHow how;
+        how.tile = GemmTile::T64;
+        how.scatter = how.klist = true;
+        gemm_tasklist_dev(ctx, w.fxtasks.p, (int)fx.size(), helfem::EIG_BAND_TILE, nm, how);
+      } else
+        gemm_tasklist_dev(ctx, w.gtasks.p, nb, nm, nm, full);
       if (low.split2)
         for (int k = 0; k < nb; k++) HFG_HIP_CHECK(hipMemsetAsync(w.A[k].p, 0, sizeof(double) * (size_t)ns[k] * ns[k], s));
       gemm_tasklist_dev(ctx, w.gtasks.p + nb, nb, nm, nm, low);
@@ -1502,6 +1590,47 @@
   }
 }
 
+__global__ void k_band_outside(const double *__restrict__ H, int N, const int *__restrict__ node, const int *__restrict__ blockid,
+                               int pm, int E, int *__restrict__ flag) {
+  const int row = blockIdx.x * blockDim.x + threadIdx.x, col = blockIdx.y;
+  int bad = 0;
+  if (row < N && (!blockid || blockid[row] == blockid[col]) && !helfem::eig_band_share(node[row], node[col], pm, E))
+    bad = H[(size_t)col * N + row] != 0.0;
+  bad = __syncthreads_or(bad);
+  if (bad && threadIdx.x == 0) atomicOr(flag, 1);
+}
+
+int eig_declare_band(hfg_ctx *ctx, int N, const int *node, int pm, int E, const double *dH0, const int *dBlockId) {
+  if (!ctx->fixed_sinvh) throw std::logic_error("hfg_ctx_declare_fock_band: no Sinvh is declared fixed (hfg_ctx_fix_sinvh)\n");
+  if (N < 1 || pm < 1 || E < 1 || !node) throw std::logic_error("hfg_ctx_declare_fock_band: invalid pattern\n");
+  for (int i = 0; i < N; i++)
+    if (node[i] < 0 || node[i] > pm * E) throw std::logic_error("hfg_ctx_declare_fock_band: radial node outside the elements\n");
+  ctx->band_node.clear();
+  ctx->band_state = 0;
+  EigWork &w = work_for(ctx);
+  w.sup_S = nullptr;
+  if (dH0) {
+    hipStream_t s = ctx->stream;
+    DevBuf<int> &buf = w.ibuf2;
+    buf.resize((size_t)N + 8);
+    int flag = 0;
+    HFG_HIP_CHECK(hipMemcpyAsync(buf.p + 1, node, sizeof(int) * N, hipMemcpyHostToDevice, s));
+    HFG_HIP_CHECK(hipMemsetAsync(buf.p, 0, sizeof(int), s));
+    hipLaunchKernelGGL(k_band_outside, dim3((N + 255) / 256, N), dim3(256), 0, s, dH0, N, buf.p + 1, dBlockId, pm, E, buf.p);
+    HFG_HIP_CHECK(hipMemcpyAsync(&flag, buf.p, sizeof(int), hipMemcpyDeviceToHost, s));
+    HFG_HIP_CHECK(hipStreamSynchronize(s));
+    if (flag) {
+      ctx->band_state = 2;
+      return 2;
+    }
+  }
+  ctx->band_node.assign(node, node + N);
+  ctx->band_pm = pm;
+  ctx->band_E = E;
+  ctx->band_state = 1;
+  return 1;
+}
+
 void eig_gsym_sub_pair_dev(hfg_ctx *ctx, int N, const double *dFa, const double *dFb, const double *dS, int nblk, const int64_t *blk_ptr,
                            const int64_t *blk_idx, double *dEa, double *dCa, double *dEb, double *dCb) {
   const double *Fs[2] = {dFa, dFb};
diff --git a/helfem_amd/csrc/hip/gemm.hip b/helfem_amd/csrc/hip/gemm.hip
--- a/helfem_amd/csrc/hip/gemm.hip
+++ b/helfem_amd/csrc/hip/gemm.hip
@@ -9,13 +9,14 @@
 typedef double double4_t __attribute__((ext_vector_type(4)));
 typedef double d2_t __attribute__((ext_vector_type(2)));
 
-template <int BM, int BN, bool ACC = false, int MF = 1, bool MAP = false, bool RMAP = false>
+template <int BM, int BN, bool ACC = false, int MF = 1, bool MAP = false, bool RMAP = false, bool KLIST = false>
 __device__ __forceinline__ void dgemm_tile(int id, int transA, int transB, int M, int N, int K, double alpha,
                                            const double *__restrict__ A, int lda, const double *__restrict__ B, int ldb,
                                            double beta, double *__restrict__ C, int ldc, double (*As)[16][BM + 16],
                                            double (*Bs)[16][BN + 16], int sym = 0, int kbeg = 0, int kend = -1, int over = 0,
                                            const int *__restrict__ amap = nullptr, const int *__restrict__ cmap = nullptr,
-                                           const int64_t *__restrict__ rmap = nullptr) {
+                                           const int64_t *__restrict__ rmap = nullptr, const int *__restrict__ kstart = nullptr,
+                                           int nk = 0) {
   constexpr int BK = 16;
   constexpr int PAD = 16;
   constexpr int WM = BM / 2, WN = BN / 2;
@@ -191,6 +192,34 @@
 
   const bool splitk = kend >= 0;
   const int kstop = splitk ? min(kend, K) : K;
+  if constexpr (KLIST) {
+    static_assert(MF == 1 && !ACC && !MAP, "the k-step list goes with the plain 16x16x4 tile");
+    if (nk > 0) {
+      load_tiles(kstart[0]);
+      store_tiles(0);
+    }
+    __syncthreads();
+    int kbuf = 0;
+    for (int st = 0; st < nk; st++) {
+      const bool more = (st + 1 < nk);
+      if (more) load_tiles(kstart[st + 1]);
+#pragma unroll
+      for (int kk = 0; kk < BK; kk += 4) {
+        double fa[TM], fb[TN];
+#pragma unroll
+        for (int i = 0; i < TM; i++) fa[i] = As[kbuf][kk + l4][wm + i * 16 + l15];
+#pragma unroll
+        for (int j = 0; j < TN; j++) fb[j] = Bs[kbuf][kk + l4][wn + j * 16 + l15];
+#pragma unroll
+        for (int i = 0; i < TM; i++)
+#pragma unroll
+          for (int j = 0; j < TN; j++) accv[i][j] = __builtin_amdgcn_mfma_f64_16x16x4f64(fb[j], fa[i], accv[i][j], 0, 0, 0);
+      }
+      if (more) store_tiles(kbuf ^ 1);
+      __syncthreads();
+      kbuf ^= 1;
+    }
+  } else {
   load_tiles(kbeg);
   store_tiles(0);
   __syncthreads();
@@ -229,6 +258,7 @@
     if (more) store_tiles(buf ^ 1);
     __syncthreads();
     buf ^= 1;
+  }
   }
   if constexpr (PRE) {
 #pragma unroll
@@ -335,6 +365,17 @@
   if ((int)blockIdx.x >= nt) return;
   dgemm_tile<BM, BN, false, MF, false, true>(blockIdx.x, t.tA, t.tB, t.M, t.N, t.K, t.alpha, t.A, t.lda, t.B, t.ldb, 0.0, t.C, t.ldc,
                                              As, Bs, 0, 0, -1, t.over, nullptr, t.cmap, t.rmap);
+}
+
+__global__ __launch_bounds__(256, 2) void k_dgemm_tasklist_klist(const GemmTask *__restrict__ tasks) {
+  __shared__ __attribute__((aligned(16))) double As[2][16][64 + 16];
+  __shared__ __attribute__((aligned(16))) double Bs[2][16][64 + 16];
+  const GemmTask t = tasks[blockIdx.y];
+  if (t.M <= 0 || t.N <= 0) return;
+  const int nt = ((t.M + 63) / 64) * ((t.N + 63) / 64);
+  if ((int)blockIdx.x >= nt) return;
+  dgemm_tile<64, 64, false, 1, false, true, true>(blockIdx.x, 0, 0, t.M, t.N, t.K, t.alpha, t.A, t.lda, t.B, t.ldb, 0.0, t.C, t.ldc, As, Bs,
+                                                  0, 0, -1, t.over, nullptr, t.cmap, t.rmap, t.kstart, t.nk);
 }
 
 template <int BM, int BN, bool SPLIT = false>
@@ -441,11 +482,11 @@
 }
 
 typedef void (*TaskKernel)(const GemmTask *);
-constexpr int ACC = 1, SPLIT2 = 2, MAP = 4, SCATTER = 8;
-constexpr int variant(GemmTile tile, int flags) { return 16 * (int)tile + flags; }
+constexpr int ACC = 1, SPLIT2 = 2, MAP = 4, SCATTER = 8, KLIST = 16;
+constexpr int variant(GemmTile tile, int flags) { return 32 * (int)tile + flags; }
 TaskKernel tasklist_kernel(GemmTile tile, const GemmHow &how) {
   const bool m4 = mfma4();
-  switch (variant(tile, how.acc * ACC + how.split2 * SPLIT2 + how.map * MAP + how.scatter * SCATTER)) {
+  switch (variant(tile, how.acc * ACC + how.split2 * SPLIT2 + how.map * MAP + how.scatter * SCATTER + how.klist * KLIST)) {
     case variant(GemmTile::T64, 0): return m4 ? k_dgemm_tasklist<64, 64, false, 0> : k_dgemm_tasklist<64, 64>;
     case variant(GemmTile::T128, 0): return m4 ? k_dgemm_tasklist<128, 128, false, 0> : k_dgemm_tasklist<128, 128>;
     case variant(GemmTile::T128x64, 0): return k_dgemm_tasklist<128, 64>;
@@ -457,11 +498,12 @@
     case variant(GemmTile::T64, SCATTER): return m4 ? k_dgemm_tasklist_scatter<64, 64, 0> : k_dgemm_tasklist_scatter<64, 64>;
     case variant(GemmTile::T128, SCATTER): return m4 ? k_dgemm_tasklist_scatter<128, 128, 0> : k_dgemm_tasklist_scatter<128, 128>;
     case variant(GemmTile::T128x64, SCATTER): return k_dgemm_tasklist_scatter<128, 64>;
+    case variant(GemmTile::T64, SCATTER + KLIST): return k_dgemm_tasklist_klist;
     case variant(GemmTile::T128, SPLIT2 + SCATTER): return k_dgemm_tasklist_split2_scatter<128, 128>;
     case variant(GemmTile::T128x64, SPLIT2 + SCATTER): return k_dgemm_tasklist_split2_scatter<128, 64>;
     default:
       throw std::logic_error(std::string("gemm_tasklist_dev: no kernel for tile ") + tile_name(tile) + (how.acc ? " acc" : "") +
-                             (how.split2 ? " split2" : "") + (how.map ? " map" : "") + (how.scatter ? " scatter" : ""));
+                             (how.split2 ? " split2" : "") + (how.map ? " map" : "") + (how.scatter ? " scatter" : "") + (how.klist ? " klist" : ""));
   }
 }
 }
diff --git a/helfem_amd/csrc/hip/internal.h b/helfem_amd/csrc/hip/internal.h
--- a/helfem_amd/csrc/hip/internal.h
+++ b/helfem_amd/csrc/hip/internal.h
@@ -8,7 +8,7 @@
 enum class GemmTile { Auto, T64, T128, T128x64 };
 struct GemmHow {
   GemmTile tile = GemmTile::Auto;
-  bool acc = false, split2 = false, map = false, scatter = false;
+  bool acc = false, split2 = false, map = false, scatter = false, klist = false;
 };
 void gemm_tasklist_dev(hfg_ctx *ctx, const GemmTask *dtasks, int ntasks, int maxM, int maxN, GemmHow how = {});
 void gemm_worklist_dev(hfg_ctx *ctx, const GemmTask *dtasks, const int2 *dwl, int nwg, GemmTile tile, bool split2 = false);
@@ -80,6 +80,8 @@
 void eig_gsym_sub_sel_dev(hfg_ctx *ctx, int N, const double *dF, const double *dS, int nblk, const int64_t *blk_ptr,
                           const int64_t *blk_idx, int nev, double *dE, double *dC);
 
+int eig_declare_band(hfg_ctx *ctx, int N, const int *node, int pm, int E, const double *dH0, const int *dBlockId);
+
 void tridiag_dc_batch(hfg_ctx *ctx, int nblk, const int *ns, double *const *d, double *const *e, double *const *Z);
 int dc_status(hfg_ctx *ctx);
 int *dc_status_word(hfg_ctx *ctx);
diff --git a/helfem_amd/csrc/host/eig_band_plan.h b/helfem_amd/csrc/host/eig_band_plan.h
--- /dev/null
+++ b/helfem_amd/csrc/host/eig_band_plan.h
@@ -0,0 +1,71 @@
+#pragma once
+#include <algorithm>
+#include <cstdint>
+#include <numeric>
+#include <vector>
+
+namespace helfem {
+constexpr int EIG_BAND_TILE = 64;
+constexpr int EIG_BAND_K0_ALIGN = 4;
+constexpr int EIG_BAND_KSTEP = 16;
+constexpr double EIG_BAND_MAX_FRACTION = 0.9;
+
+#if defined(__HIPCC__)
+#define HELFEM_BAND_HD __host__ __device__
+#else
+#define HELFEM_BAND_HD
+#endif
+HELFEM_BAND_HD inline void eig_band_node_range(int n, int pm, int E, int &lo, int &hi) {
+  const int e1 = n / pm;
+  const int ehi = e1 < E - 1 ? e1 : E - 1;
+  const int el = (n % pm == 0 && e1 >= 1) ? e1 - 1 : e1;
+  const int elo = el < E - 1 ? el : E - 1;
+  lo = elo * pm;
+  hi = ehi * pm + pm;
+}
+HELFEM_BAND_HD inline bool eig_band_share(int n, int m, int pm, int E) {
+  int lo, hi;
+  eig_band_node_range(n, pm, E, lo, hi);
+  return m >= lo && m <= hi;
+}
+
+inline void eig_band_order(int64_t n, const int *node, int64_t *perm) {
+  std::iota(perm, perm + n, (int64_t)0);
+  std::stable_sort(perm, perm + n, [&](int64_t a, int64_t b) { return node[a] < node[b]; });
+}
+
+inline bool eig_band_plan(int64_t n, const int *node, const int64_t *perm, int pm, int E, std::vector<int> &kstart, std::vector<int> &toff) {
+  const int nt = (int)((n + EIG_BAND_TILE - 1) / EIG_BAND_TILE);
+  kstart.clear();
+  toff.assign(1, 0);
+  for (int t = 0; t < nt; t++) {
+    const int64_t i0 = (int64_t)t * EIG_BAND_TILE, i1 = std::min<int64_t>(n, i0 + EIG_BAND_TILE);
+    int lo = 0, hi = 0;
+    for (int64_t i = i0; i < i1; i++) {
+      int l, h;
+      eig_band_node_range(node[perm[i]], pm, E, l, h);
+      lo = (i == i0) ? l : std::min(lo, l);
+      hi = (i == i0) ? h : std::max(hi, h);
+    }
+    int64_t next = 0;
+    for (int64_t k = 0; k < n; k++) {
+      if (k < next || node[k] < lo || node[k] > hi) continue;
+      const int64_t st = k - k % EIG_BAND_K0_ALIGN;
+      kstart.push_back((int)st);
+      next = st + EIG_BAND_KSTEP;
+    }
+    toff.push_back((int)kstart.size());
+  }
+  const double dense_steps = (double)nt * (double)((n + EIG_BAND_KSTEP - 1) / EIG_BAND_KSTEP);
+  const bool banded = nt >= 2 && (double)kstart.size() <= EIG_BAND_MAX_FRACTION * dense_steps;
+  if (!banded) {
+    kstart.clear();
+    toff.assign(1, 0);
+    for (int t = 0; t < nt; t++) {
+      for (int64_t k = 0; k < n; k += EIG_BAND_KSTEP) kstart.push_back((int)k);
+      toff.push_back((int)kstart.size());
+    }
+  }
+  return banded;
+}
+}
diff --git a/helfem_amd/csrc/host/tuning.h b/helfem_amd/csrc/host/tuning.h
--- a/helfem_amd/csrc/host/tuning.h
+++ b/helfem_amd/csrc/host/tuning.h
@@ -32,6 +32,7 @@
   X(cuhf_lowrank, bool, true, "HELFEM_CUHF_LOWRANK", true, "off if 0", atoi(e) != 0, "hfg_cuhf_update_devptr: the constraint from the occupied orbitals (rank na + nb, up to 128 columns); off: the dense natural-orbital sequence always (checker)") \
   X(eig_pair, bool, true, "HELFEM_EIG_PAIR", false, "off if 0", atoi(e) != 0, "both spins' Fock matrices in one batched eigensolve; off: two calls") \
   X(eig_direct, bool, true, "HELFEM_EIG_DIRECT", true, "off if 0", atoi(e) != 0, "one-call blocked eigensolve (hfg_eig_gsym_sub_dev, _sel_dev, _pair_devptr) ranks before its last product and stores that product straight into C; off: block slots, then hfg_eig_assemble_dev (checker)") \
+  X(eig_band, bool, true, "HELFEM_EIG_BAND", true, "off if 0", atoi(e) != 0, "blocked eigensolve under a declared radial-element pattern of F (hfg_ctx_declare_fock_band): rows of F radial-major, F X as row-tile tasks over the k steps that meet their non-zero columns, bit for bit the dense product; off: the declaration is ignored (checker)") \
   X(trd_mode, TrdMode, TrdMode::persistent, "HELFEM_TRD", false, "word", !strcmp(e, "persistent") ? TrdMode::persistent : !strcmp(e, "twokernel") ? TrdMode::twokernel : !strcmp(e, "unblocked") ? TrdMode::unblocked : TrdMode::chain, "tridiagonalisation: persistent = k_trdp where the batch fits, else the chain; chain (and any unknown word) = one k_trdf launch per column always (checker); twokernel = k_trdb_gemv + k_trdb_w; unblocked = the first-generation kernels") \
   X(trdp_min, int, 256, "HELFEM_TRDP_MIN", false, "int", atoi(e), "smallest order the persistent kernel takes") \
   X(trdp_r, int, 0, "HELFEM_TRDP_R", false, "int", atoi(e), "rows per thread of the persistent kernel forced (0: the first that fits)") \
diff --git a/include/helfem_gpu.h b/include/helfem_gpu.h
--- a/include/helfem_gpu.h
+++ b/include/helfem_gpu.h
@@ -22,6 +22,11 @@
 int hfg_ctx_set_shard(hfg_ctx *ctx, int rank, int nranks);
 
 int hfg_ctx_fix_sinvh(hfg_ctx *ctx, const double *dSinvh);
+
+int hfg_ctx_declare_band(hfg_ctx *ctx, int64_t N, const int *node, int pm, int E, const double *dH0, const int *dBlockId, int *state);
+int hfg_ctx_declare_fock_band(hfg_ctx *ctx, hfg_basis *basis, const double *dH0, const int *dBlockId, int *state);
+int hfg_ctx_fock_band_state(hfg_ctx *ctx, int *state);
+int hfg_eig_band_plan(int64_t n, const int *node, int pm, int E, int64_t *perm, int *toff, int *kstart, int64_t cap, int *banded);
 
 typedef struct {
   int Z1, Z2;
```

Result: faster. 7.718 ms (median of 6 runs) (-2.6%).
